# hkapp/cniic

Measured on AMD Instinct MI355X. Metric: Mpixels/sec encode (cluster-colors K=256), higher is better.
Workload: dtype u8/u64; 1 GPU; configs[1]: cluster-colors(256) encode of one 4096x4096 photo-like synthetic RGB image per GPU (seed 0x636E696963+2+rank), to convergence; image and stream HBM-resident; pixels_per_gpu=16777216, parallelism=1 GPU

## Files before the change

cniic_amd/csrc/codec.cpp:

```cpp
#include "codec.hpp"

#include <algorithm>
#include <cctype>
#include <cstring>
#include <memory>

#include "huff_host.hpp"

namespace cniic {

HostTrace &host_trace() { static thread_local HostTrace t; return t; }

static bool match_fun_u32(const std::string &s, const char *const *names, uint32_t *arg) {
    for (size_t p = 0; p < s.size(); p++)
        for (int i = 0; names[i]; i++) {
            const size_t l = strlen(names[i]);
            if (s.compare(p, l, names[i]) != 0 || p + l >= s.size() || s[p + l] != '(') continue;
            size_t q = p + l + 1;
            if (q >= s.size() || !isdigit((unsigned char)s[q])) continue;
            unsigned long long v = 0;
            bool ok = true;
            while (q < s.size() && isdigit((unsigned char)s[q])) {
                v = v * 10 + (unsigned)(s[q] - '0');
                if (v > 0xffffffffull) { ok = false; break; }
// ... 421 lines not shown
    put_u32(header, w);
    put_u32(header, h);
    huff_serialize_tree(tree, CNIIC_SYM_RGB, skeys.data(), header);
    *nbits = 0;
    for (size_t i = 0; i < scounts.size(); i++) *nbits += scounts[i] * slen[i];
    for (uint32_t k = 0; k < K; k++) {
        const size_t si = std::lower_bound(skeys.begin(), skeys.end(), colour(k)) - skeys.begin();
        clen[k] = pixels[k] ? slen[si] : 0;
        ccode[k] = pixels[k] ? scode[si] : 0;
    }
    return true;
}

int cc_finish(CcSession *s, const uint8_t *rgb_d, uint32_t w, uint32_t h, const uint32_t *local_counts_d, uint8_t *out,
              uint64_t cap, uint64_t *len, cniic_kmeans_stats *stats) {
    Ctx *c = s->c;
    const uint32_t K = s->K;
    const uint64_t U = s->U, n = (uint64_t)w * h;
    KmRgbwState *km = s->km;
    std::vector<uint8_t> cent(3 * (size_t)K);
    std::vector<uint64_t> members(K), wsum(K);
    cniic_kmeans_stats st{};
    const bool wide = km_rgbw_is_wide(km);
    DevBuf lab_d, key2label, pixlab;
    CNIIC_HIP_TRY(c, pixlab.alloc(n * (wide ? 2 : 1) + 16));
    DevBuf lw;
    bool lw_early = false;
    for (int attempt = 0;; attempt++) {
    CNIIC_TRY(km_rgbw_result_begin(km));
    if (s->sp_mode) {
        uint32_t *cell_start, *ckeys, *cweight;
        km_rgbw_cell_arrays(km, &cell_start, &ckeys, &cweight);
        if (s->local_points && K <= kPuPaletteWeights.words) {
            CNIIC_HIP_TRY(c, ctx_pinned_u(c));
            CNIIC_HIP_TRY(c, lw.alloc((uint64_t)K * 8));
            CNIIC_HIP_TRY(c, hipMemsetAsync(lw.p, 0, (uint64_t)K * 8, c->stream));
            CNIIC_TRY(local_cluster_weights(c, ckeys, km_rgbw_labels_internal(km, nullptr), wide, U, nullptr, K, lw.as<uint64_t>(), cweight));
            CNIIC_HIP_TRY(c, hipMemcpyAsync(c->pinned_u + kPuPaletteWeights.at, lw.p, (size_t)K * 8, hipMemcpyDeviceToHost, c->stream));
            if (!c->u_ev) CNIIC_HIP_TRY(c, hipEventCreateWithFlags(&c->u_ev, hipEventDisableTiming));
            CNIIC_HIP_TRY(c, hipEventRecord(c->u_ev, c->stream));
            lw_early = true;
        }
        CNIIC_TRY(sp_pixel_labels(c, &s->sp, rgb_d, cell_start, ckeys, km_rgbw_labels_internal(km, nullptr), wide, pixlab.p));
    } else {
        CNIIC_HIP_TRY(c, lab_d.alloc(U * (wide ? 2 : 1)));
        CNIIC_TRY(km_rgbw_labels_canonical(km, lab_d.p));
        CNIIC_HIP_TRY(c, key2label.alloc((1ull << 24) * (wide ? 2 : 1)));
        CNIIC_TRY(scatter_labels_by_key(c, s->keys_d.as<uint32_t>(), lab_d.p, wide, U, key2label.p));
        CNIIC_TRY(pixel_labels(c, rgb_d, n, key2label.p, wide, pixlab.p));
    }
    host_trace().mark("labels + pixel labels enq");
    const int rc_res = km_rgbw_result_end(km, cent.data(), members.data(), wsum.data(), &st);
    if (rc_res == kKmRetry && attempt == 0) continue;
    CNIIC_TRY(rc_res);
    break;
    }
    host_trace().mark("km_result");
    if (stats) *stats = st;
    CNIIC_TRY(check_enough_active(c, K, U, st.active));
    if (lw_early) {
        CNIIC_HIP_TRY(c, hipEventSynchronize(c->u_ev));
        for (uint32_t k = 0; k < K; k++) wsum[k] = c->pinned_u[kPuPaletteWeights.at + k];
    } else if (local_counts_d || s->local_points) {
        CNIIC_HIP_TRY(c, lw.alloc((uint64_t)K * 8));
        CNIIC_HIP_TRY(c, hipMemsetAsync(lw.p, 0, (uint64_t)K * 8, c->stream));
        if (s->sp_mode) {
            uint32_t *cell_start, *ckeys, *cweight;
            km_rgbw_cell_arrays(km, &cell_start, &ckeys, &cweight);
            CNIIC_TRY(local_cluster_weights(c, ckeys, km_rgbw_labels_internal(km, nullptr), wide, U, nullptr, K, lw.as<uint64_t>(), cweight));
        } else {
            CNIIC_TRY(local_cluster_weights(c, s->keys_d.as<uint32_t>(), lab_d.p, wide, U, local_counts_d, K, lw.as<uint64_t>(),
                                            s->weight_d.as<uint32_t>()));
        }
        CNIIC_HIP_TRY(c, hipMemcpyAsync(wsum.data(), lw.p, (size_t)K * 8, hipMemcpyDeviceToHost, c->stream));
        CNIIC_HIP_TRY(c, hipStreamSynchronize(c->stream));
    }
    std::vector<uint8_t> header, clen(K);
    std::vector<uint64_t> ccode(K);
    uint64_t nbits = 0;
    if (!palette_code(cent.data(), wsum.data(), K, w, h, header, clen.data(), ccode.data(), &nbits))
        return c->fail(CNIIC_ERR_BAD_ARG, "huffman: cannot build code");
    host_trace().mark("tree+codes (host)");
    StreamOut so(c, out, cap, len);
    CNIIC_TRY(so.begin(header, (nbits + 7) / 8));
    host_trace().mark("so.begin");
    DevBuf clen_d, ccode_d;
    CNIIC_HIP_TRY(c, clen_d.alloc(K));
    CNIIC_HIP_TRY(c, ccode_d.alloc((uint64_t)K * 8));
    CNIIC_HIP_TRY(c, hipMemcpyAsync(clen_d.p, clen.data(), K, hipMemcpyHostToDevice, c->stream));
    CNIIC_HIP_TRY(c, hipMemcpyAsync(ccode_d.p, ccode.data(), (size_t)K * 8, hipMemcpyHostToDevice, c->stream));
    uint64_t packed_bits = 0;
    {
        ScopedKernelTimer t(c, "huff_pack");
        CNIIC_TRY(huff_pack_labels(c, pixlab.p, n, wide, K, clen_d.as<uint8_t>(), ccode_d.as<uint64_t>(), so.dev,
                                   (uint64_t)header.size() * 8, &packed_bits));
        t.stop(1);
    }
    host_trace().mark("pack (+sync)");
    if (packed_bits != nbits)
        return c->fail(CNIIC_ERR_HIP, "cluster-colors: packed %llu bits, histogram predicts %llu",
                       (unsigned long long)packed_bits, (unsigned long long)nbits);
    const int rc_fin = so.finish();
    host_trace().mark("so.finish");
    return rc_fin;
}

int cc_finish_frames(CcSession *s, const uint8_t *rgb_d, uint32_t w, uint32_t h, uint32_t F, uint8_t *out, uint64_t stride, uint64_t *lens,
                     cniic_kmeans_stats *stats) {
    Ctx *c = s->c;
    const uint32_t K = s->K;
    const uint64_t U = s->U, npf = (uint64_t)w * h, n = npf * F;
    KmRgbwState *km = s->km;
    host_trace().mark("frames: enter");
    if (!F || !npf) return c->fail(CNIIC_ERR_BAD_ARG, "cc_finish_frames: empty batch");
    if (stride & 3) return c->fail(CNIIC_ERR_BAD_ARG, "cc_finish_frames: the stride between streams must be a multiple of 4");
    if (s->sp_mode && s->sp.npx != n) return c->fail(CNIIC_ERR_BAD_ARG, "cc_finish_frames: the session was opened on %llu pixels, the batch has %llu",
                                                     (unsigned long long)s->sp.npx, (unsigned long long)n);
    std::vector<uint8_t> cent(3 * (size_t)K);
    std::vector<uint64_t> members(K), wsum(K);
    cniic_kmeans_stats st{};
    CNIIC_TRY(km_rgbw_result_begin(km));
    const bool wide = km_rgbw_is_wide(km);
    const uint64_t lb = wide ? 2 : 1;
    DevBuf lab_d, key2label, pixlab, pixlab_al, cnt_d;
    host_trace().mark("frames: result_begin");
    CNIIC_HIP_TRY(c, pixlab.alloc(n * lb + 16));
    host_trace().mark("frames: alloc pixel labels");
    if (s->sp_mode) {
        uint32_t *cell_start, *ckeys, *cweight;
        km_rgbw_cell_arrays(km, &cell_start, &ckeys, &cweight);
        CNIIC_TRY(sp_pixel_labels(c, &s->sp, rgb_d, cell_start, ckeys, km_rgbw_labels_internal(km, nullptr), wide, pixlab.p));
        host_trace().mark("frames: pixel labels enqueued");
    } else {
        CNIIC_HIP_TRY(c, lab_d.alloc(U * lb));
        CNIIC_TRY(km_rgbw_labels_canonical(km, lab_d.p));
        CNIIC_HIP_TRY(c, key2label.alloc((1ull << 24) * lb));
        CNIIC_TRY(scatter_labels_by_key(c, s->keys_d.as<uint32_t>(), lab_d.p, wide, U, key2label.p));
        CNIIC_TRY(pixel_labels(c, rgb_d, n, key2label.p, wide, pixlab.p));
    }
    const void *labs = pixlab.p;
    uint64_t lab_stride = npf;
    if ((npf * lb) & 15) {
        lab_stride = (npf + 15) & ~15ull;
        CNIIC_HIP_TRY(c, pixlab_al.alloc(lab_stride * lb * F + 16));
        CNIIC_HIP_TRY(c, hipMemcpy2DAsync(pixlab_al.p, lab_stride * lb, pixlab.p, npf * lb, npf * lb, F, hipMemcpyDeviceToDevice, c->stream));
        labs = pixlab_al.p;
    }
    CNIIC_HIP_TRY(c, cnt_d.alloc((uint64_t)F * K * 4));
    CNIIC_TRY(frame_label_hist(c, labs, npf, lab_stride, F, wide, K, cnt_d.as<uint32_t>()));
    const bool gpu_trees = !wide && K <= 256 && c->opt(CNIIC_OPT_FRAME_TREES_HOST, "CNIIC_FRAME_TREES_HOST", 0) == 0;
    std::vector<uint32_t> cnt(gpu_trees ? 0 : (size_t)F * K);
    if (!gpu_trees) CNIIC_HIP_TRY(c, hipMemcpyAsync(cnt.data(), cnt_d.p, cnt.size() * 4, hipMemcpyDeviceToHost, c->stream));
    host_trace().mark("frames: hist enqueued");
    CNIIC_TRY(km_rgbw_result_end(km, cent.data(), members.data(), wsum.data(), &st));
    if (stats) *stats = st;
    CNIIC_TRY(check_enough_active(c, K, U, st.active));
    host_trace().mark("frames: result_end (sync)");
    CNIIC_HIP_TRY(c, hipStreamSynchronize(c->stream));
    host_trace().mark("frames: wait for the histograms");
    FramesOut fo(c, out, stride, F);
    DevBuf clen_d, ccode_d;
    CNIIC_HIP_TRY(c, clen_d.alloc((size_t)F * K));
    CNIIC_HIP_TRY(c, ccode_d.alloc((size_t)F * K * 8));
    std::vector<uint64_t> totals(F, 0);
    if (gpu_trees) {
        CNIIC_TRY(fo.begin());
        DevBuf meta_d;
        CNIIC_HIP_TRY(c, meta_d.alloc((size_t)F * 24 + 8));
        uint64_t *bb_d = meta_d.as<uint64_t>(), *nb_d = bb_d + F, *ln_d = nb_d + F;
        uint32_t *err_d = reinterpret_cast<uint32_t *>(ln_d + F);
        CNIIC_HIP_TRY(c, hipMemsetAsync(err_d, 0, 8, c->stream));
        CNIIC_TRY(frame_trees(c, cnt_d.as<uint32_t>(), km_rgbw_centroids_dev(km), F, K, w, h, fo.dev, stride, clen_d.as<uint8_t>(), ccode_d.as<uint64_t>(), bb_d, nb_d, ln_d, err_d));
        std::vector<uint64_t> meta((size_t)F * 3 + 1);
        CNIIC_HIP_TRY(c, hipMemcpyAsync(meta.data(), meta_d.p, (size_t)F * 24 + 8, hipMemcpyDeviceToHost, c->stream));
        CNIIC_HIP_TRY(c, hipStreamSynchronize(c->stream));
        host_trace().mark("frames: trees, codes, headers (GPU) + lengths back");
        const uint32_t err = (uint32_t)meta[(size_t)F * 3];
        if (err & 3u) return c->fail(CNIIC_ERR_BAD_ARG, "huffman: cannot build code");
// ... 589 lines not shown
```

cniic_amd/csrc/common.hpp:

```cpp
#pragma once
#include <hip/hip_runtime.h>

#include <algorithm>
#include <cstdarg>
#include <cstdint>
#include <cstdio>
#include <cstring>
#include <atomic>
#include <chrono>
#include <map>
#include <memory>
#include <mutex>
#include <string>
#include <thread>
#include <vector>

#include "../../include/cniic_hip.h"

namespace cniic {

constexpr uint64_t kDefaultSeed = 0x636E696963ULL;

struct KernelTime {
    double   ms = 0.0;
// ... 90 lines not shown
    bool        own_stream = false;
    std::mutex  mu;
    std::string err;
    std::map<std::string, KernelTime> ktimes;
    hipEvent_t  ev0 = nullptr, ev1 = nullptr;
    bool    timers = getenv("CNIIC_KERNEL_TIMERS") != nullptr;
    uint64_t opt_val[CNIIC_OPT_COUNT] = {};
    uint32_t opt_set = 0;
    uint64_t opt(int id, const char *env, uint64_t dflt) const {
        if (id > 0 && id < CNIIC_OPT_COUNT && ((opt_set >> id) & 1u)) return opt_val[id];
        const char *e = env ? getenv(env) : nullptr;
        return e ? strtoull(e, nullptr, 10) : dflt;
    }
    DevPool pool;
    DevBuf dense;
    DevBuf dense27, dense27_pages;
    bool   dense27_clean = false;
    DevBuf hilbert_lut;
    void  *pinned = nullptr;
    void  *pinned_ps = nullptr;
    uint32_t ps_div = 1;
    uint32_t ps_backoff = 0, ps_backoff_left = 0;
    hipEvent_t poll_ev[2] = {nullptr, nullptr};
    void  *pinned_res = nullptr;
    uint64_t pinned_res_bytes = 0;
    hipEvent_t res_ev = nullptr;
    uint64_t *pinned_u = nullptr;
    hipEvent_t u_ev = nullptr;
    std::shared_ptr<void> trie_scratch;
    std::shared_ptr<void> huf_scratch;
    void  *pinned_huf = nullptr;
    uint64_t pinned_huf_bytes = 0;
    hipEvent_t huf_ev = nullptr;
    std::shared_ptr<void> scan_leaves;
    DevBuf scan_xy;
    uint32_t scan_w = 0, scan_h = 0;
    std::vector<void *> batch_workers;
    DevBuf batch_stage;
    const void *poll_owner = nullptr;

    int fail(int code, const char *fmt, ...) {
        char buf[512];
        va_list ap;
        va_start(ap, fmt);
        vsnprintf(buf, sizeof buf, fmt, ap);
        va_end(ap);
        err = buf;
        return code;
    }
};

#define CNIIC_HIP_TRY(ctx, expr)                                                          \
    do {                                                                                  \
        hipError_t _e = (expr);                                                           \
        if (_e != hipSuccess)                                                             \
            return (ctx)->fail(CNIIC_ERR_HIP, "%s:%d %s -> %s", __FILE__, __LINE__, #expr, \
                               hipGetErrorString(_e));                                    \
    } while (0)

inline hipError_t ctx_spin_sync(Ctx *c) {
    hipError_t e;
    while ((e = hipStreamQuery(c->stream)) == hipErrorNotReady) {}
    return e;
}

inline hipError_t ctx_pinned_huf(Ctx *c, uint64_t bytes) {
    if (c->pinned_huf_bytes >= bytes) return hipSuccess;
    if (c->pinned_huf) (void)hipHostFree(c->pinned_huf);
    c->pinned_huf = nullptr; c->pinned_huf_bytes = 0;
    const uint64_t want = bytes + bytes / 4 + 65536;
    const hipError_t e = hipHostMalloc(&c->pinned_huf, want, hipHostMallocDefault);
    if (e == hipSuccess) c->pinned_huf_bytes = want;
    return e;
}

struct PuSlot { uint32_t at, words; };
constexpr uint32_t kPinnedUWords = 64 * 1024 / 8;
constexpr PuSlot kPuSpCount{0, 1};
constexpr PuSlot kPuPointCount{1, 1};
constexpr PuSlot kPuImageCount{2, 1};
constexpr PuSlot kPuHufTotals{3, 2};
constexpr PuSlot kPuDeltaOverflow{5, 1};
constexpr PuSlot kPuDeltaPacked{6, 1};
constexpr PuSlot kPuPaletteWeights{8, 4096};
constexpr PuSlot kPuHdecode{4104, 3};
constexpr PuSlot kPuTrieTotals{4108, 6};
constexpr PuSlot kPuLeafRuns{4114, 3};
constexpr PuSlot kPuSlots[] = {kPuSpCount, kPuPointCount, kPuImageCount, kPuHufTotals, kPuDeltaOverflow, kPuDeltaPacked,
                               kPuPaletteWeights, kPuHdecode, kPuTrieTotals, kPuLeafRuns};
constexpr bool pu_slots_disjoint() {
    uint32_t end = 0;
    for (const PuSlot &s : kPuSlots) {
        if (s.at < end || s.words == 0) return false;
        end = s.at + s.words;
    }
    return end <= kPinnedUWords;
}
static_assert(pu_slots_disjoint(), "Ctx::pinned_u: two slots overlap, or the last one ends behind the 64 KiB block");
static_assert(kPuPaletteWeights.words >= 4096, "Ctx::pinned_u: the shared-palette weights need room for K = 4096");

inline hipError_t ctx_pinned_u(Ctx *c) {
    if (c->pinned_u) return hipSuccess;
    return hipHostMalloc(reinterpret_cast<void **>(&c->pinned_u), kPinnedUWords * 8, hipHostMallocDefault);
}

#define CNIIC_TRY(expr)              \
    do {                             \
        int _rc = (expr);            \
        if (_rc != CNIIC_OK) return _rc; \
    } while (0)

inline bool is_device_ptr(const void *p) {
    if (!p) return false;
    hipPointerAttribute_t a;
    hipError_t e = hipPointerGetAttributes(&a, p);
    if (e != hipSuccess) { (void)hipGetLastError(); return false; }
    return a.type == hipMemoryTypeDevice || a.type == hipMemoryTypeManaged;
}

template <class T> struct In {
    const T *d = nullptr;
    DevBuf   own;
    int bind(Ctx *c, const T *p, uint64_t n) {
        if (n == 0 || !p) { d = nullptr; return CNIIC_OK; }
        if (is_device_ptr(p)) { d = p; return CNIIC_OK; }
        CNIIC_HIP_TRY(c, own.alloc(n * sizeof(T)));
        CNIIC_HIP_TRY(c, hipMemcpyAsync(own.p, p, n * sizeof(T), hipMemcpyHostToDevice, c->stream));
        d = own.as<T>();
        return CNIIC_OK;
    }
};

template <class T> struct Out {
    T       *d = nullptr;
    T       *host = nullptr;
    uint64_t n = 0;
    DevBuf   own;
    int bind(Ctx *c, T *p, uint64_t count) {
        n = count;
        if (!p || count == 0) { d = nullptr; host = nullptr; return CNIIC_OK; }
        if (is_device_ptr(p)) { d = p; host = nullptr; return CNIIC_OK; }
        CNIIC_HIP_TRY(c, own.alloc(count * sizeof(T)));
        d = own.as<T>();
        host = p;
        return CNIIC_OK;
    }
    int finish(Ctx *c, uint64_t count) {
        if (host && count) CNIIC_HIP_TRY(c, hipMemcpyAsync(host, d, count * sizeof(T), hipMemcpyDeviceToHost, c->stream));
        return CNIIC_OK;
    }
    int finish(Ctx *c) { return finish(c, n); }
};

inline uint64_t ceil_div(uint64_t a, uint64_t b) { return (a + b - 1) / b; }

inline int check_enough_active(Ctx *c, uint32_t K, uint64_t npoints, uint64_t active) {
    const uint64_t min_cc = std::min<uint64_t>((uint64_t)(0.99 * (double)K), npoints);
    if (active < min_cc)
        return c->fail(CNIIC_ERR_FEW_ACTIVE, "Not enough active clusters: requested %u, got %llu (min allowed: %llu)", K,
                       (unsigned long long)active, (unsigned long long)min_cc);
    return CNIIC_OK;
}

template <class Body> void parallel_for(uint32_t count, uint32_t threads, Body body) {
    std::atomic<uint32_t> next{0};
    auto work = [&](uint32_t t) { for (uint32_t i; (i = next.fetch_add(1)) < count;) body(i, t); };
    std::vector<std::thread> pool;
    for (uint32_t t = 1; t < threads; t++) pool.emplace_back(work, t);
    work(0);
    for (auto &th : pool) th.join();
}

// ... 82 lines not shown
                                       (unsigned long long)limit_ms);
                    std::this_thread::sleep_for(std::chrono::microseconds(20));
                }
            }
            CNIIC_HIP_TRY(c, hipEventSynchronize(c->poll_ev[slot ^ 1]));
            if (ring) {
                const volatile PollRec *r = reinterpret_cast<const volatile PollRec *>(static_cast<uint8_t *>(c->pinned) + ring_offset()) + last_prev % kPollRing;
                if (r->seq != last_prev) return c->fail(CNIIC_ERR_HIP, "kmeans: launch %u left no state record (found %u)", last_prev, r->seq);
                KmDevState t{};
                t.done = r->done; t.iter = r->iter; t.moved_last = r->moved_last; t.reseeds = r->reseeds; t.active = r->active; t.pair_evals = r->pair_evals;
                *h = t;
            } else if (mapped) {
                volatile KmDevState *m = &slots[2];
                KmDevState t{};
                t.done = m->done;
                std::atomic_thread_fence(std::memory_order_acquire);
                t.iter = m->iter; t.moved_last = m->moved_last; t.reseeds = m->reseeds; t.active = m->active; t.pair_evals = m->pair_evals;
                *h = t;
            } else {
                *h = slots[slot ^ 1];
            }
        }
        slot ^= 1;
        pending = 1;
        last_prev = last_launch;
        return CNIIC_OK;
    }
    int drain(KmDevState *h) {
        KmDevState *slots = static_cast<KmDevState *>(c->pinned);
        CNIIC_HIP_TRY(c, hipEventSynchronize(c->poll_ev[slot ^ 1]));
        *h = slots[slot ^ 1];
        return CNIIC_OK;
    }
};

struct HostTrace {
    bool on;
    std::vector<std::pair<const char *, double>> marks;
    HostTrace() : on(test_env("CNIIC_TRACE_HOST") != nullptr) {}
    static double now() { return std::chrono::duration<double, std::micro>(std::chrono::steady_clock::now().time_since_epoch()).count(); }
    void mark(const char *what) { if (on) marks.emplace_back(what, now()); }
    void dump() {
        if (!on || marks.empty()) return;
        for (size_t i = 1; i < marks.size(); i++) fprintf(stderr, "[host] %-28s %8.1f us\n", marks[i].first, marks[i].second - marks[i - 1].second);
        fprintf(stderr, "[host] %-28s %8.1f us\n", "total", marks.back().second - marks.front().second);
        marks.clear();
    }
};
HostTrace &host_trace();

struct ScopedKernelTimer {
    Ctx        *c;
    const char *name;
    bool        on;
    ScopedKernelTimer(Ctx *ctx, const char *nm) : ScopedKernelTimer(ctx, nm, ctx->timers) {}
    ScopedKernelTimer(Ctx *ctx, const char *nm, bool enable) : c(ctx), name(nm), on(enable) {
        if (on) (void)hipEventRecord(c->ev0, c->stream);
    }
    void stop(uint64_t launches = 1) {
        if (!on) return;
        (void)hipEventRecord(c->ev1, c->stream);
        (void)hipEventSynchronize(c->ev1);
        float ms = 0.f;
        (void)hipEventElapsedTime(&ms, c->ev0, c->ev1);
        KernelTime &kt = c->ktimes[name];
        kt.ms += ms;
        kt.launches += launches;
        on = false;
    }
};


int hist_rgb_dense(Ctx *c, const uint8_t *rgb_d, uint64_t npx, uint32_t *table_d);
int hist_syms_dense(Ctx *c, const uint32_t *syms_d, uint64_t n, uint32_t *table_d, uint32_t bits);
struct CompactPlan {
    DevBuf   blockoff, blockmax;
    uint64_t n_unique = 0;
    uint64_t max_count = 0;
    uint32_t bits = 0;
    const uint8_t *pages = nullptr;
};
int occupancy_pack(Ctx *c, const uint32_t *table_d, uint32_t *occ_d);
int gidx_build(Ctx *c, const uint32_t *occ_d, DevBuf &bits, DevBuf &wprefix, uint64_t *U_h, DevBuf *total_keep = nullptr);
int gidx_finish(Ctx *c, uint32_t *wprefix_d, const uint32_t *blocktot_d, uint64_t *total_d);

struct SpPlan {
    uint64_t npx = 0, U = 0;
    uint32_t nchunks = 0;
    DevBuf cnt, pre, bstart;
    DevBuf part, prank;
    DevBuf cell_count;
    DevBuf sstart, sbin, scnt;
    DevBuf bits, wprefix;
    DevBuf total;
};
int sp_build(Ctx *c, const uint8_t *rgb_d, uint64_t npx, SpPlan *plan);
int sp_wait_count(Ctx *c, SpPlan *plan);
int sp_emit(Ctx *c, const SpPlan *plan, const uint32_t *cell_start_d, uint32_t *ckeys_d, uint32_t *cweight_d, void *labels_d, bool wide,
            uint32_t K, const void *gbits_d, const uint32_t *gprefix_d, uint64_t Ug, const uint64_t *Ug_dev );
int sp_occupancy(Ctx *c, const SpPlan *plan, uint32_t *occ_d);
int sp_pixel_labels(Ctx *c, const SpPlan *plan, const uint8_t *rgb_d, const uint32_t *cell_start_d, const uint32_t *ckeys_d,
                    const void *labels_d, bool wide, void *pixlab_d);
int hist_compact_count(Ctx *c, const uint32_t *table_d, uint32_t bits, CompactPlan *plan, uint32_t *cell_count_d = nullptr,
                       const uint8_t *pages_d = nullptr);
int hist_compact_write(Ctx *c, uint32_t *table_d, const CompactPlan *plan, uint32_t *keys_d, uint64_t *counts_d,
                       uint32_t *weights_d);
int dense_table(Ctx *c, uint32_t bits, uint32_t **table_d);

struct KmRgbwState;
int km_rgbw_create(Ctx *c, const uint32_t *keys_d, const uint32_t *weight_d, uint64_t U, uint32_t shard,
                   uint32_t nshards, uint32_t K, const cniic_kmeans_opts *opts, void *partials_dev,
                   const uint32_t *rank_table_d , KmRgbwState **out,
                   const uint32_t *cell_count_d = nullptr ,
                   const void *gbits_d = nullptr, const uint32_t *gprefix_d = nullptr, uint64_t Ug = 0
                   ,
                   bool points_follow = false ,
                   const uint64_t *points_dev = nullptr );
int km_rgbw_set_points(KmRgbwState *s, uint64_t U, uint64_t Ulist = 0 );
void km_rgbw_cell_arrays(KmRgbwState *s, uint32_t **cell_start_d, uint32_t **ckeys_d, uint32_t **cweight_d);
void km_rgbw_destroy(KmRgbwState *s);
int km_rgbw_set_state(KmRgbwState *s, const uint8_t *centroids_h, const uint32_t *labels_d_u32);
int km_rgbw_assign(KmRgbwState *s);
int km_rgbw_update(KmRgbwState *s);
struct Comm;
int comm_unique_id(uint8_t *id128);
int comm_create(Ctx *c, const uint8_t *id128, uint32_t rank, uint32_t nranks, Comm **out);
int comm_create_host(Ctx *c, uint32_t rank, uint32_t nranks, int32_t (*fn)(void *, void *, uint64_t, int32_t), void *user, Comm **out);
void comm_destroy(Comm *cm);
Ctx *comm_ctx(Comm *cm);
uint32_t comm_size(const Comm *cm);
int comm_all_reduce(Comm *cm, void *buf_d, uint64_t count, int kind);
void comm_abort(Comm *cm);
int comm_async_error(Comm *cm);
uint64_t comm_timeout_ms(const Comm *cm);
void comm_set_timeout_ms(Comm *cm, uint64_t ms);
int comm_create_mailbox(Ctx *c, uint32_t rank, uint32_t nranks, uint64_t max_bytes, uint8_t *handle64, Comm **out);
int comm_connect_mailbox(Comm *cm, const uint8_t *handles);

struct Mailbox;
int mailbox_create(Ctx *c, uint32_t rank, uint32_t nranks, uint64_t cap_bytes, uint8_t *handle64, Mailbox **out);
int mailbox_connect(Mailbox *m, const uint8_t *handles);
int mailbox_all_reduce(Mailbox *m, void *buf_d, uint64_t count, int kind, uint64_t timeout_ms);
int mailbox_status(const Mailbox *m);
void mailbox_abort(Mailbox *m);
void mailbox_destroy(Mailbox *m);

constexpr int kKmRetry = 1000;
int km_rgbw_run(KmRgbwState *s, Comm *cm = nullptr, bool may_defer = false);
int km_rgbw_poll_changed(KmRgbwState *s, uint64_t *changed);
int km_rgbw_poll(KmRgbwState *s, cniic_kmeans_stats *st, uint32_t *done);
bool km_rgbw_run_stats(KmRgbwState *s, cniic_kmeans_stats *st);
int km_rgbw_poll_lagged(KmRgbwState *s, cniic_kmeans_stats *st, uint32_t *done, uint32_t *have);
int km_rgbw_result(KmRgbwState *s, uint8_t *centroids_h, uint32_t *labels_d_u32, uint64_t *members_h,
                   uint64_t *wsum_h, cniic_kmeans_stats *stats);
int km_rgbw_result_begin(KmRgbwState *s);
int km_rgbw_result_end(KmRgbwState *s, uint8_t *centroids_h, uint64_t *members_h, uint64_t *wsum_h, cniic_kmeans_stats *stats);
int km_rgbw_time_assign(KmRgbwState *s, int reps, double *ms_per_launch);
int km_rgbw_partials(KmRgbwState *s, uint64_t *sums_h, uint64_t *wsum_h, uint64_t *members_h, uint64_t *changed_h);
void *km_rgbw_partials_dev(KmRgbwState *s);
const uint32_t *km_rgbw_centroids_dev(KmRgbwState *s);
bool km_rgbw_is_wide(KmRgbwState *s);
int km_rgbw_labels_canonical(KmRgbwState *s, void *dst_d);
void *km_rgbw_labels_internal(KmRgbwState *s, uint64_t *elem_bytes);
int km_rgbw_fold_initial(KmRgbwState *s);
int km_rgbw_export_labels(KmRgbwState *s, void *dst_d);
int km_rgbw_import_labels(KmRgbwState *s, const void *src_d);
uint64_t km_rgbw_points(KmRgbwState *s);
// ... 2 lines not shown
                 const cniic_kmeans_opts *opts, cniic_colorpos *centroids_h, uint32_t *labels_d_u32,
                 uint64_t *members_h, cniic_kmeans_stats *stats);
int km_xyrgb_run_wide(Ctx *c, const uint8_t *rgb_d, uint32_t w, uint32_t h, uint32_t K, const cniic_kmeans_opts *opts, cniic_colorpos *centroids_h,
                      uint32_t *labels_d_u32, uint64_t *members_h, cniic_kmeans_stats *stats);
int km_xyrgb_step(Ctx *c, const uint8_t *rgb_d, uint32_t w, uint32_t h, uint32_t K,
                  const cniic_colorpos *centroids_h, uint32_t *labels_d_u32, uint64_t *sums_h,
                  uint64_t *wsum_h, uint64_t *members_h, uint64_t *changed_h, const cniic_kmeans_opts *opts);

int remap_rgb(Ctx *c, const uint8_t *rgb_d, uint64_t npx, const uint32_t *rank_table_d,
              const uint32_t *lut_rgb_d , uint8_t *out_d);
int expand_codes_by_label(Ctx *c, const uint8_t *labels8_d, const uint16_t *labels16_d, uint64_t U, const uint8_t *clen_d,
                          const uint64_t *ccode_d, uint8_t *len_d, uint64_t *code_d);
int local_cluster_weights(Ctx *c, const uint32_t *keys_d, const void *labels_d, bool wide, uint64_t U,
                          const uint32_t *local_counts_d, uint32_t K, uint64_t *out_d, const uint32_t *weights_d = nullptr);
int label_lut(Ctx *c, const uint32_t *labels_d, uint64_t U, const uint32_t *cent_d, uint32_t *lut_d);
int rank_from_keys(Ctx *c, const uint32_t *keys_d, uint64_t U, uint32_t *table_d);
int voronoi_paint(Ctx *c, const cniic_colorpos *cent_d, uint32_t K, uint32_t w, uint32_t h, uint8_t *out_d, bool small_coords = false);
int mse_rgb(Ctx *c, const uint8_t *a_d, const uint8_t *b_d, uint64_t npx, double *mse_h);
int mse_rgb_batch(Ctx *c, const uint8_t *a_d, const uint8_t *b_d, uint64_t npx, uint32_t frames, double *mse_h);
int mse_rgb_batch_var(Ctx *c, const uint8_t *a_d, const uint8_t *b_d, const uint64_t *a_off, const uint64_t *b_off, const uint64_t *npx,
                      uint32_t frames, double *mse_h);
int synth_image(Ctx *c, int kind, uint64_t seed, uint32_t w, uint32_t h, uint8_t *out_d);
int rgb_to_keys(Ctx *c, const uint8_t *rgb_d, uint64_t npx, uint32_t *keys_d);

constexpr int kCellShift = 3;
constexpr uint32_t kCellsPerDim = 256 >> kCellShift;
constexpr uint32_t kNumCells = kCellsPerDim * kCellsPerDim * kCellsPerDim;

struct LeafTable;
struct UdSums { DevBuf buf; bool filled = false; };
int huff_decode_dev(Ctx *c, const LeafTable &lt, const uint8_t *payload, bool payload_dev, uint64_t payload_bytes, uint64_t nsyms,
                    int mode, void *out_d, int *status, UdSums *sums = nullptr);
struct HdBatchFrame {
    const LeafTable *lt = nullptr;
    const uint8_t *payload = nullptr;
    uint64_t payload_bytes = 0, nsyms = 0;
    uint8_t *out_d = nullptr;
    int status = 0;
};
int huff_decode_batch_dev(Ctx *c, std::vector<HdBatchFrame> &frames);
int huff_decode_tables_dev(Ctx *c, const uint8_t *tab_d, uint64_t n, uint64_t off_key, uint64_t off_len, uint32_t max_len, uint32_t first_key,
                           const uint8_t *payload, bool payload_dev, uint64_t payload_bytes, uint64_t nsyms, int mode, void *out_d, int *status, UdSums *sums = nullptr);
int huff_parse_leaves_dev(Ctx *c, int sym_kind, const uint8_t *stream_d, uint64_t nbytes, uint64_t pos0, DevBuf *tab, uint64_t *n_leaves,
                          uint64_t *off_key, uint64_t *off_len, uint32_t *max_len, uint64_t *payload_pos, int *status);
int keys_to_rgb(Ctx *c, const uint32_t *keys_d, uint64_t n, uint8_t *rgb_d);
int delta_undiff_dev(Ctx *c, const uint32_t *keys_d, uint64_t n, uint8_t *lin_d, uint32_t *bad_h);
int delta_undiff_scatter_dev(Ctx *c, const uint32_t *keys_d, uint32_t w, uint32_t h, uint8_t *rgb_out_d, uint32_t *bad_h, UdSums *sums = nullptr);

struct RlePlan { uint64_t n = 0, nruns = 0; uint32_t nchunks = 0; DevBuf flags, run_off; };
int rle_plan(Ctx *c, const uint8_t *lin_d, uint64_t n, RlePlan *plan);
int rle_emit(Ctx *c, const uint8_t *lin_d, const RlePlan *plan, uint32_t *out_words_d);
int rle_expand_dev(Ctx *c, const uint8_t *rec_d, uint64_t R, uint64_t tail_bytes, uint64_t n, uint8_t *lin_d, int *status);
int rle_offsets(Ctx *c, const uint32_t *chunk_runs_d, uint32_t nchunks, uint64_t *run_off_d, uint64_t *total_d);
double rla_threshold(double d);
int rle_approx_plan(Ctx *c, const uint8_t *lin_d, uint64_t n, double d, RlePlan *plan);
int rle_approx_emit(Ctx *c, const uint8_t *lin_d, const RlePlan *plan, uint32_t *out_words_d);

int hilbert_xy(Ctx *c, uint32_t w, uint32_t h, uint32_t *xy_d);
int hilbert_linearize(Ctx *c, const uint8_t *rgb_d, uint32_t w, uint32_t h, uint8_t *out_d);
int hilbert_delta(Ctx *c, const uint8_t *rgb_d, uint32_t w, uint32_t h, uint32_t *syms_d, uint32_t *table_d);
int hilbert_scatter(Ctx *c, const uint8_t *lin_d, uint32_t w, uint32_t h, uint8_t *rgb_out_d);
int scan_inject(Ctx *c, uint32_t w, uint32_t h, const uint32_t *xy, bool xy_dev);
int hilbert_undiff_scatter(Ctx *c, const uint32_t *keys_d, const int32_t *chunk_off_d, uint32_t w, uint32_t h, uint8_t *rgb_out_d, uint32_t *bad_d, bool *fused);

constexpr uint32_t kPageShift = 12;
int delta_table(Ctx *c, uint32_t **table_d, uint8_t **pages_d);
int delta_table_clean(Ctx *c);
uint64_t delta_stream_len(uint64_t n);
int delta_gather_hist(Ctx *c, const uint8_t *rgb_d, uint32_t w, uint32_t h, uint16_t *hot16_d, uint32_t *table_d, uint8_t *pages_d,
                      uint32_t *coldkeys_d, uint8_t *chunk_cold_d, uint32_t *overflow_d);
struct DeltaPackScratch { DevBuf cb, co, edge, hot, hotlen; };
int delta_pack16_count(Ctx *c, const uint16_t *hot16_d, uint64_t n, uint32_t *coldkeys_d, const uint8_t *chunk_cold_d, uint32_t *dense_d,
                       const uint32_t *keys_d, const uint8_t *len_d, const uint64_t *code_d, uint64_t U, uint64_t *total_d, DeltaPackScratch *keep);
int delta_pack16_write(Ctx *c, const uint16_t *hot16_d, uint64_t n, const uint32_t *coldkeys_d, const uint8_t *len_d, const uint64_t *code_d, uint8_t *out_d,
                       uint64_t bit_base, DeltaPackScratch *keep);

int huff_sort_leaves_dev(Ctx *c, const uint64_t *counts_d, uint32_t n, uint64_t max_count, uint64_t *buf_a, uint64_t *buf_b, uint64_t **out_d);
int huff_sort_u64(Ctx *c, uint64_t *buf_a, uint64_t *buf_b, uint32_t n, uint32_t lo_bit, uint64_t **out_d);
int huff_tree_from_runs(Ctx *c, const uint64_t *sorted_d, const uint64_t *counts_d, uint32_t n, int sym_kind, uint8_t *len_d, uint64_t *code_d,
                        uint64_t *off_d, uint64_t *nbits_h, bool *built);
int huff_tree_codes(Ctx *c, const uint32_t *left_d, const uint32_t *right_d, const uint32_t *nleaves_d, const uint64_t *counts_d, uint32_t n,
                    uint32_t root, int sym_kind, uint8_t *len_d, uint64_t *code_d, uint64_t *off_d, uint64_t *totals_d);
int huff_tree_serialize_dev(Ctx *c, const uint32_t *keys_d, const uint64_t *off_d, uint32_t n, int sym_kind, uint8_t *trie_d, uint64_t trie_bytes);
int pack_scan(Ctx *c, const uint32_t *chunk_bits_d, uint32_t nchunks, uint64_t *chunk_off_d, uint64_t *total_d);
uint32_t pack_img_cap();
int huff_pack_keys(Ctx *c, const uint32_t *keys_or_null_d, const uint8_t *rgb_or_null_d, uint64_t n,
                   const uint32_t *rank_table_d, const uint8_t *len_d, const uint64_t *code_d,
                   uint8_t *out_d, uint64_t bit_base, uint64_t *nbits_h);
int huff_rank_stream(Ctx *c, const uint32_t *keys_or_null_d, const uint8_t *rgb_or_null_d, uint64_t n, const uint32_t *rank_table_d,
                     uint32_t *ranks_d, bool one_based);
int huff_pack_ranks(Ctx *c, const uint32_t *ranks_d, uint64_t n, const uint8_t *len_d, const uint64_t *code_d, uint8_t *out_d,
                    uint64_t bit_base, uint64_t *nbits_h);
int huff_pack_code32(Ctx *c, const uint32_t *syms_or_null_d, const uint8_t *rgb_or_null_d, uint64_t n, uint32_t *table_d,
                     const uint32_t *keys_d, const uint8_t *len_d, const uint64_t *code_d, uint64_t U, uint32_t *packed_d,
                     uint8_t *out_d, uint64_t bit_base, uint64_t *nbits_h);
int huff_pack_code32_hot(Ctx *c, const uint32_t *syms_d, uint64_t n, uint32_t *dense_d, const uint32_t *keys_d, const uint8_t *len_d,
                         const uint64_t *code_d, uint64_t U, uint32_t *packed_d, uint8_t *out_d, uint64_t bit_base, uint64_t *nbits_h);
int pixel_labels(Ctx *c, const uint8_t *rgb_d, uint64_t n, const void *key2label_d, bool wide, void *pixlab_d);
int huff_pack_labels(Ctx *c, const void *pixlab_d, uint64_t n, bool wide, uint32_t K, const uint8_t *clen_d,
                     const uint64_t *ccode_d, uint8_t *out_d, uint64_t bit_base, uint64_t *nbits_h);
int scatter_labels_by_key(Ctx *c, const uint32_t *keys_d, const void *labels_d, bool wide, uint64_t U, void *key2label_d);
int frame_label_hist(Ctx *c, const void *pixlab_d, uint64_t npf, uint64_t lab_stride, uint32_t frames, bool wide, uint32_t K, uint32_t *out_d );
int huff_pack_labels_frames(Ctx *c, const void *pixlab_d, uint64_t npf, uint64_t lab_stride, uint32_t frames, bool wide, uint32_t K, const uint8_t *clen_d,
                            const uint64_t *ccode_d, uint8_t *out_d, uint64_t stride, const uint64_t *bit_base_h, uint64_t *totals_h, const uint64_t *bit_base_d = nullptr);
int frame_trees(Ctx *c, const uint32_t *cnt_d, const uint32_t *cent_d, uint32_t frames, uint32_t K, uint32_t w, uint32_t h, uint8_t *out_d, uint64_t stride,
                uint8_t *clen_d, uint64_t *ccode_d, uint64_t *bit_base_d, uint64_t *nbits_d, uint64_t *lens_d, uint32_t *err_d);

}
```

cniic_amd/csrc/k_hist.hip:

```cpp
#include <cstdlib>

#include "common.hpp"
#include "device_utils.hpp"

namespace cniic {

__global__ __launch_bounds__(256) void k_hist_rgb(const uint8_t *__restrict__ rgb, uint64_t npx,
                                                  uint32_t *__restrict__ table) {
    const uint64_t ngroups = npx / 16;
    const uint64_t stride = (uint64_t)gridDim.x * blockDim.x;
    const uint4 *v = reinterpret_cast<const uint4 *>(rgb);
    for (uint64_t g = (uint64_t)blockIdx.x * blockDim.x + threadIdx.x; g < ngroups; g += stride) {
        uint32_t key[16];
        load16px_keys(v + 3 * g, key);
#pragma unroll
        for (int i = 0; i < 16; i++) atomic_count(table, key[i]);
    }
    if (blockIdx.x == 0) {
        uint64_t i = ngroups * 16 + threadIdx.x;
        if (i < npx) atomic_count(table, rgb_key(rgb + 3 * i));
    }
}

constexpr int kPartBits = 12;
// ... 256 lines not shown
            val[i] = rank + 1;
            rank++;
            dirty = true;
        }
    }
    if (dirty) {
#pragma unroll
        for (int j = 0; j < kScanPerThread / 4; j++)
            v[j] = make_uint4(val[4 * j], val[4 * j + 1], val[4 * j + 2], val[4 * j + 3]);
    }
}

int hist_compact_count(Ctx *c, const uint32_t *table_d, uint32_t bits, CompactPlan *plan, uint32_t *cell_count_d, const uint8_t *pages_d) {
    static_assert(kScanChunk == (1 << kPageShift), "a page flag per block of the compaction");
    plan->pages = pages_d;
    const uint64_t entries = 1ull << bits;
    const uint32_t nblocks = (uint32_t)(entries / kScanChunk);
    DevBuf tot;
    CNIIC_HIP_TRY(c, plan->blockoff.alloc((uint64_t)nblocks * 4));
    CNIIC_HIP_TRY(c, plan->blockmax.alloc((uint64_t)nblocks * 4));
    CNIIC_HIP_TRY(c, tot.alloc(16));
    hipLaunchKernelGGL(k_compact_count, dim3(nblocks), dim3(kScanThreads), 0, c->stream, table_d, plan->blockoff.as<uint32_t>(), plan->blockmax.as<uint32_t>(),
                       bits == 24 ? cell_count_d : nullptr, pages_d, tot.as<uint64_t>());
    {
        const uint32_t nparts = (nblocks + 1023) / 1024;
        DevBuf parttot;
        CNIIC_HIP_TRY(c, parttot.alloc((uint64_t)nparts * 4));
        hipLaunchKernelGGL(k_compact_scan_local, dim3(nparts), dim3(1024), 0, c->stream, plan->blockoff.as<uint32_t>(), (const uint32_t *)plan->blockmax.as<uint32_t>(), nblocks,
                           parttot.as<uint32_t>(), tot.as<uint64_t>());
        if (nparts > 1)
            hipLaunchKernelGGL(k_compact_scan_add, dim3(nparts), dim3(1024), 0, c->stream, plan->blockoff.as<uint32_t>(), nblocks,
                               (const uint32_t *)parttot.as<uint32_t>(), tot.as<uint64_t>());
    }
    CNIIC_HIP_TRY(c, hipGetLastError());
    uint64_t total[2] = {0, 0};
    CNIIC_HIP_TRY(c, hipMemcpyAsync(total, tot.p, 16, hipMemcpyDeviceToHost, c->stream));
    CNIIC_HIP_TRY(c, pages_d ? ctx_spin_sync(c) : hipStreamSynchronize(c->stream));
    plan->n_unique = total[0];
    plan->max_count = total[1];
    plan->bits = bits;
    return CNIIC_OK;
}

int hist_compact_write(Ctx *c, uint32_t *table_d, const CompactPlan *plan, uint32_t *keys_d, uint64_t *counts_d,
                       uint32_t *weights_d) {
    const uint32_t nblocks = (uint32_t)((1ull << plan->bits) / kScanChunk);
    hipLaunchKernelGGL(k_compact_write, dim3(nblocks), dim3(kScanThreads), 0, c->stream, table_d,
                       plan->blockoff.as<uint32_t>(), keys_d, counts_d, weights_d, plan->pages);
    CNIIC_HIP_TRY(c, hipGetLastError());
    return CNIIC_OK;
}

__global__ __launch_bounds__(256) void k_occ_pack(const uint32_t *__restrict__ table, uint32_t *__restrict__ occ) {
    const uint32_t wd = blockIdx.x * 256 + threadIdx.x;
    const uint4 a = reinterpret_cast<const uint4 *>(table)[2 * (size_t)wd], b = reinterpret_cast<const uint4 *>(table)[2 * (size_t)wd + 1];
    occ[wd] = (a.x != 0) | ((a.y != 0) << 4) | ((a.z != 0) << 8) | ((a.w != 0) << 12) | ((b.x != 0) << 16) | ((b.y != 0) << 20) |
              ((b.z != 0) << 24) | ((uint32_t)(b.w != 0) << 28);
}
__global__ __launch_bounds__(256) void k_gidx_words(const uint32_t *__restrict__ occ, unsigned long long *__restrict__ bits,
                                                    uint32_t *__restrict__ wprefix, uint32_t *__restrict__ blocktot) {
    __shared__ uint32_t wsum[256 / 64];
    const uint32_t w0 = (blockIdx.x * 256 + threadIdx.x) * 4;
    uint32_t cnt[4], mine = 0;
#pragma unroll
    for (int q = 0; q < 4; q++) {
        unsigned long long m = 0;
#pragma unroll
        for (int j = 0; j < 8; j++) {
            const uint32_t v = occ[8 * (size_t)(w0 + q) + j];
#pragma unroll
            for (int i = 0; i < 8; i++)
                if ((v >> (4 * i)) & 15u) m |= 1ull << (8 * j + i);
        }
        bits[w0 + q] = m;
        cnt[q] = (uint32_t)__popcll(m);
        mine += cnt[q];
    }
    uint32_t run = block_exclusive_scan<256>(mine, wsum);
#pragma unroll
    for (int q = 0; q < 4; q++) { wprefix[w0 + q] = run; run += cnt[q]; }
    if (threadIdx.x == 255) blocktot[blockIdx.x] = run;
}
__global__ __launch_bounds__(256) void k_gidx_finish(uint32_t *__restrict__ wprefix, const uint32_t *__restrict__ blocktot,
                                                     uint64_t *__restrict__ total) {
    __shared__ uint32_t wsum[256 / 64];
    __shared__ uint32_t boff[256];
    const uint32_t t = blocktot[threadIdx.x];
    const uint32_t ex = block_exclusive_scan<256>(t, wsum);
    boff[threadIdx.x] = ex;
    if (blockIdx.x == 0 && threadIdx.x == 255) *total = (uint64_t)ex + t;
    __syncthreads();
    const uint32_t add = boff[blockIdx.x];
    for (uint32_t i = threadIdx.x; i < 1024; i += 256) wprefix[blockIdx.x * 1024 + i] += add;
}

int gidx_finish(Ctx *c, uint32_t *wprefix_d, const uint32_t *blocktot_d, uint64_t *total_d) {
    hipLaunchKernelGGL(k_gidx_finish, dim3(256), dim3(256), 0, c->stream, wprefix_d, blocktot_d, total_d);
    CNIIC_HIP_TRY(c, hipGetLastError());
    return CNIIC_OK;
}

int occupancy_pack(Ctx *c, const uint32_t *table_d, uint32_t *occ_d) {
    hipLaunchKernelGGL(k_occ_pack, dim3((1u << 21) / 256), dim3(256), 0, c->stream, table_d, occ_d);
    CNIIC_HIP_TRY(c, hipGetLastError());
    return CNIIC_OK;
}

int gidx_build(Ctx *c, const uint32_t *occ_d, DevBuf &bits, DevBuf &wprefix, uint64_t *U_h, DevBuf *total_keep) {
    DevBuf tot_own;
    DevBuf &tot = total_keep ? *total_keep : tot_own;
    CNIIC_HIP_TRY(c, bits.alloc((1ull << 18) * 8));
    CNIIC_HIP_TRY(c, wprefix.alloc((1ull << 18) * 4));
    CNIIC_HIP_TRY(c, tot.alloc(8));
    DevBuf blocktot;
    CNIIC_HIP_TRY(c, blocktot.alloc(256 * 4));
    hipLaunchKernelGGL(k_gidx_words, dim3(256), dim3(256), 0, c->stream, occ_d, bits.as<unsigned long long>(), wprefix.as<uint32_t>(),
                       blocktot.as<uint32_t>());
    hipLaunchKernelGGL(k_gidx_finish, dim3(256), dim3(256), 0, c->stream, wprefix.as<uint32_t>(), (const uint32_t *)blocktot.as<uint32_t>(),
                       tot.as<uint64_t>());
    CNIIC_HIP_TRY(c, hipGetLastError());
    CNIIC_HIP_TRY(c, hipMemcpyAsync(U_h, tot.p, 8, hipMemcpyDeviceToHost, c->stream));
    if (!total_keep) CNIIC_HIP_TRY(c, hipStreamSynchronize(c->stream));
    return CNIIC_OK;
}

int dense_table(Ctx *c, uint32_t bits, uint32_t **table_d) {
    const uint64_t bytes = (1ull << bits) * 4;
    if (c->dense.bytes < bytes) CNIIC_HIP_TRY(c, c->dense.alloc(bytes));
    CNIIC_HIP_TRY(c, hipMemsetAsync(c->dense.p, 0, bytes, c->stream));
    *table_d = c->dense.as<uint32_t>();
    return CNIIC_OK;
}

}
```

cniic_amd/csrc/k_huff.hip:

```cpp
#include <mutex>

#include <algorithm>
#include <vector>

#include "common.hpp"
#include "device_utils.hpp"

namespace cniic {

constexpr int kPackThreads = 256;
constexpr int kPackPer = 16;
constexpr int kPackChunk = kPackThreads * kPackPer;

enum { SRC_RGB = 0, SRC_KEYS = 1, SRC_SYM16 = 2, SRC_RANKS = 3 };

template <int SRC>
__device__ __forceinline__ void fetch_ranks(const void *__restrict__ src, uint64_t n, uint64_t first,
                                            const uint32_t *__restrict__ rank_table, uint32_t rank[kPackPer]) {
    if (SRC == SRC_RGB) {
        const uint8_t *rgb = reinterpret_cast<const uint8_t *>(src);
        if (first + kPackPer <= n && ((reinterpret_cast<uintptr_t>(rgb) & 15) == 0)) {
            uint32_t key[16];
            load16px_keys(reinterpret_cast<const uint4 *>(rgb + 3 * first), key);
#pragma unroll
            for (int i = 0; i < kPackPer; i++) rank[i] = rank_table[key[i]] - 1;
        } else {
#pragma unroll
            for (int i = 0; i < kPackPer; i++)
                rank[i] = (first + i < n) ? rank_table[rgb_key(rgb + 3 * (first + i))] - 1 : 0xffffffffu;
        }
    } else if (SRC == SRC_KEYS) {
        const uint32_t *keys = reinterpret_cast<const uint32_t *>(src);
#pragma unroll
        for (int i = 0; i < kPackPer; i++) rank[i] = (first + i < n) ? rank_table[keys[first + i]] - 1 : 0xffffffffu;
    } else if (SRC == SRC_RANKS) {
        const uint32_t *rk = reinterpret_cast<const uint32_t *>(src);
        if (first + kPackPer <= n && ((reinterpret_cast<uintptr_t>(rk) & 15) == 0)) {
            const uint4 *v = reinterpret_cast<const uint4 *>(rk + first);
#pragma unroll
            for (int j = 0; j < 4; j++) { const uint4 q = v[j]; rank[4 * j] = q.x - 1; rank[4 * j + 1] = q.y - 1; rank[4 * j + 2] = q.z - 1; rank[4 * j + 3] = q.w - 1; }
        } else {
#pragma unroll
            for (int i = 0; i < kPackPer; i++) rank[i] = (first + i < n) ? rk[first + i] - 1 : 0xffffffffu;
        }
    } else {
        const uint16_t *sym = reinterpret_cast<const uint16_t *>(src);
#pragma unroll
        for (int i = 0; i < kPackPer; i++) rank[i] = (first + i < n) ? (uint32_t)sym[first + i] : 0xffffffffu;
    }
}

template <int SRC>
__global__ __launch_bounds__(kPackThreads) void k_rank_stream(const void *__restrict__ src, uint64_t n,
                                                              const uint32_t *__restrict__ rank_table, uint32_t *__restrict__ out,
                                                              uint32_t plus) {
    const uint64_t first = (uint64_t)blockIdx.x * kPackChunk + (uint64_t)threadIdx.x * kPackPer;
    uint32_t rank[kPackPer];
    fetch_ranks<SRC>(src, n, first, rank_table, rank);
    if (first + kPackPer <= n && ((reinterpret_cast<uintptr_t>(out) & 15) == 0)) {
        uint4 *o = reinterpret_cast<uint4 *>(out + first);
#pragma unroll
        for (int j = 0; j < 4; j++) o[j] = make_uint4(rank[4 * j] + plus, rank[4 * j + 1] + plus, rank[4 * j + 2] + plus, rank[4 * j + 3] + plus);
    } else {
        for (int i = 0; i < kPackPer; i++)
            if (first + i < n) out[first + i] = rank[i] + plus;
    }
}

template <int SRC>
__global__ __launch_bounds__(kPackThreads) void k_pack_count(const void *__restrict__ src, uint64_t n,
                                                             const uint32_t *__restrict__ rank_table,
                                                             const uint8_t *__restrict__ len,
                                                             uint32_t *__restrict__ chunk_bits) {
    const uint64_t first = (uint64_t)blockIdx.x * kPackChunk + (uint64_t)threadIdx.x * kPackPer;
    uint32_t rank[kPackPer];
    fetch_ranks<SRC>(src, n, first, rank_table, rank);
    uint32_t bits = 0;
#pragma unroll
    for (int i = 0; i < kPackPer; i++)
        if (rank[i] != 0xffffffffu) bits += len[rank[i]];
    bits = block_reduce_sum<kPackThreads>(bits);
    if (threadIdx.x == 0) chunk_bits[blockIdx.x] = bits;
}

__global__ __launch_bounds__(1024) void k_pack_scan_local(const uint32_t *__restrict__ chunk_bits, uint32_t nchunks,
                                                          uint64_t *__restrict__ chunk_off, uint64_t *__restrict__ blocktot,
                                                          uint64_t *__restrict__ total_bits) {
    __shared__ uint32_t wsum[1024 / 64];
    const uint32_t i = blockIdx.x * 1024 + threadIdx.x;
    const uint32_t v = i < nchunks ? chunk_bits[i] : 0u;
    const uint32_t ex = block_exclusive_scan<1024>(v, wsum);
    if (i < nchunks) chunk_off[i] = ex;
    if (threadIdx.x == 1023) {
        blocktot[blockIdx.x] = (uint64_t)ex + v;
        if (gridDim.x == 1) *total_bits = (uint64_t)ex + v;
    }
}
__global__ __launch_bounds__(1024) void k_pack_scan_add(uint32_t nchunks, uint64_t *__restrict__ chunk_off,
                                                        const uint64_t *__restrict__ blocktot, uint64_t *__restrict__ total_bits) {
    __shared__ unsigned long long s_before;
    unsigned long long mine = 0;
    for (uint32_t b = threadIdx.x; b < blockIdx.x; b += 1024) mine += blocktot[b];
    if (threadIdx.x == 0) s_before = 0;
    __syncthreads();
    mine = wave_reduce_sum64(mine);
    if ((threadIdx.x & 63) == 0 && mine) atomicAdd(&s_before, mine);
    __syncthreads();
    const unsigned long long before = s_before;
    const uint32_t i = blockIdx.x * 1024 + threadIdx.x;
    if (i < nchunks) chunk_off[i] += before;
    if (blockIdx.x == gridDim.x - 1 && threadIdx.x == 0) *total_bits = before + blocktot[blockIdx.x];
}
__global__ __launch_bounds__(1024) void k_pack_scan_small(const uint32_t *__restrict__ chunk_bits, uint32_t nchunks,
                                                          uint64_t *__restrict__ chunk_off, uint64_t *__restrict__ total_bits) {
    __shared__ uint32_t wsum[1024 / 64];
    const uint32_t i0 = threadIdx.x * 8;
    uint32_t v[8], sum = 0;
#pragma unroll
    for (int j = 0; j < 8; j++) { v[j] = i0 + j < nchunks ? chunk_bits[i0 + j] : 0u; sum += v[j]; }
    uint32_t run = block_exclusive_scan<1024>(sum, wsum);
#pragma unroll
    for (int j = 0; j < 8; j++) {
        if (i0 + j < nchunks) chunk_off[i0 + j] = run;
        run += v[j];
    }
    if (threadIdx.x == 1023) *total_bits = run;
}
static int pack_scan_counts(Ctx *c, const uint32_t *counts_d, uint32_t n, uint64_t *off_d, uint64_t *total_d) {
    if (n > 1024 && n <= 8192) {
        hipLaunchKernelGGL(k_pack_scan_small, dim3(1), dim3(1024), 0, c->stream, counts_d, n, off_d, total_d);
        CNIIC_HIP_TRY(c, hipGetLastError());
        return CNIIC_OK;
    }
    return pack_scan(c, counts_d, n, off_d, total_d);
}
int pack_scan(Ctx *c, const uint32_t *chunk_bits_d, uint32_t nchunks, uint64_t *chunk_off_d, uint64_t *total_d) {
    const uint32_t nb = (nchunks + 1023) / 1024;
    DevBuf blocktot;
    CNIIC_HIP_TRY(c, blocktot.alloc((uint64_t)nb * 8));
    hipLaunchKernelGGL(k_pack_scan_local, dim3(nb), dim3(1024), 0, c->stream, chunk_bits_d, nchunks, chunk_off_d, blocktot.as<uint64_t>(), total_d);
    if (nb > 1)
        hipLaunchKernelGGL(k_pack_scan_add, dim3(nb), dim3(1024), 0, c->stream, nchunks, chunk_off_d, (const uint64_t *)blocktot.as<uint64_t>(), total_d);
    CNIIC_HIP_TRY(c, hipGetLastError());
    return CNIIC_OK;
}

uint32_t pack_img_cap() {
    const char *e = test_env("CNIIC_TEST_PACK_IMG_WORDS");
    return e ? (uint32_t)atoi(e) : 0xffffffffu;
}

template <int SRC>
__global__ __launch_bounds__(kPackThreads) void k_pack_write(const void *__restrict__ src, uint64_t n,
                                                             const uint32_t *__restrict__ rank_table,
                                                             const uint8_t *__restrict__ len,
                                                             const uint64_t *__restrict__ code,
                                                             const uint64_t *__restrict__ chunk_off,
                                                             uint32_t *__restrict__ out_words, uint64_t bit_base, uint32_t img_cap) {
    constexpr uint32_t kImgWords = kPackChunk + 2;
    __shared__ uint32_t img[kImgWords];
    __shared__ uint32_t wsum[kPackThreads / 64];
    __shared__ uint32_t s_total;
    const uint64_t first = (uint64_t)blockIdx.x * kPackChunk + (uint64_t)threadIdx.x * kPackPer;
    uint32_t rank[kPackPer];
    fetch_ranks<SRC>(src, n, first, rank_table, rank);
    uint32_t l[kPackPer];
    uint32_t bits = 0;
#pragma unroll
    for (int i = 0; i < kPackPer; i++) {
        l[i] = rank[i] != 0xffffffffu ? len[rank[i]] : 0;
        bits += l[i];
    }
    uint32_t excl = block_exclusive_scan<kPackThreads>(bits, wsum);
    const uint64_t g0 = bit_base + chunk_off[blockIdx.x];
    const uint32_t skew = (uint32_t)(g0 & 31);
    uint32_t pos = skew + excl;
    if (threadIdx.x == kPackThreads - 1) s_total = excl + bits;
    __syncthreads();
    const uint32_t total = s_total;
    if (total == 0) return;
    const uint32_t nwords = (skew + total + 31) >> 5;
    const uint64_t w0 = g0 >> 5;
    if (nwords + 2 > min(kImgWords, img_cap)) {
#pragma unroll 1
        for (int i = 0; i < kPackPer; i++) {
            if (l[i]) pack_put<true>(out_words + w0, pos, l[i], code[rank[i]]);
            pos += l[i];
        }
        return;
    }
    for (uint32_t i = threadIdx.x; i < nwords + 2; i += kPackThreads) img[i] = 0;
    __syncthreads();
#pragma unroll
    for (int i = 0; i < kPackPer; i++) {
        if (l[i]) pack_put<false>(img, pos, l[i], code[rank[i]]);
        pos += l[i];
    }
    __syncthreads();
    for (uint32_t i = threadIdx.x; i < nwords; i += kPackThreads) {
        uint32_t v = __builtin_bswap32(img[i]);
        if (v == 0) continue;
        if (i == 0 || i == nwords - 1) atomicOr(&out_words[w0 + i], v);
        else out_words[w0 + i] = v;
    }
}

template <typename LabelT>
__global__ __launch_bounds__(kPackThreads) void k_pixel_labels(const uint8_t *__restrict__ rgb, uint64_t n,
                                                               const LabelT *__restrict__ key2label, LabelT *__restrict__ pixlab) {
    const uint64_t first = (uint64_t)blockIdx.x * kPackChunk + (uint64_t)threadIdx.x * kPackPer;
    if (first + kPackPer <= n && ((reinterpret_cast<uintptr_t>(rgb) & 15) == 0)) {
        uint32_t key[16];
        load16px_keys(reinterpret_cast<const uint4 *>(rgb + 3 * first), key);
        LabelT lab[16];
#pragma unroll
        for (int i = 0; i < 16; i++) lab[i] = key2label[key[i]];
        if (sizeof(LabelT) == 1) {
            uint32_t w[4];
#pragma unroll
            for (int j = 0; j < 4; j++) w[j] = (uint32_t)lab[4 * j] | ((uint32_t)lab[4 * j + 1] << 8) | ((uint32_t)lab[4 * j + 2] << 16) | ((uint32_t)lab[4 * j + 3] << 24);
            *reinterpret_cast<uint4 *>(pixlab + first) = make_uint4(w[0], w[1], w[2], w[3]);
        } else {
#pragma unroll
            for (int i = 0; i < 16; i++) pixlab[first + i] = lab[i];
        }
    } else {
        for (int i = 0; i < kPackPer; i++)
            if (first + i < n) pixlab[first + i] = key2label[rgb_key(rgb + 3 * (first + i))];
    }
}

template <typename LabelT>
__global__ __launch_bounds__(kPackThreads) void k_pack_count_lab(const LabelT *__restrict__ pixlab, uint64_t n, uint32_t K,
                                                                 const uint8_t *__restrict__ clen,
                                                                 uint32_t *__restrict__ chunk_bits, uint64_t lab_stride = 0) {
    extern __shared__ uint8_t s_len[];
    pixlab += (size_t)blockIdx.y * lab_stride;
    clen += (size_t)blockIdx.y * K;
    chunk_bits += (size_t)blockIdx.y * gridDim.x;
    for (uint32_t i = threadIdx.x; i < K; i += kPackThreads) s_len[i] = clen[i];
    __syncthreads();
    const uint64_t first = (uint64_t)blockIdx.x * kPackChunk + (uint64_t)threadIdx.x * kPackPer;
    uint32_t bits = 0;
    if (sizeof(LabelT) == 1 && first + kPackPer <= n) {
        const uint4 v = *reinterpret_cast<const uint4 *>(pixlab + first);
        const uint32_t w[4] = {v.x, v.y, v.z, v.w};
#pragma unroll
        for (int i = 0; i < 16; i++) bits += s_len[(w[i >> 2] >> (8 * (i & 3))) & 255];
    } else {
        for (int i = 0; i < kPackPer; i++)
            if (first + i < n) bits += s_len[pixlab[first + i]];
    }
    bits = block_reduce_sum<kPackThreads>(bits);
    if (threadIdx.x == 0) chunk_bits[blockIdx.x] = bits;
}

template <typename LabelT>
__global__ __launch_bounds__(kPackThreads) void k_pack_write_lab(const LabelT *__restrict__ pixlab, uint64_t n, uint32_t K,
                                                                 const uint8_t *__restrict__ clen,
                                                                 const uint64_t *__restrict__ ccode,
                                                                 const uint64_t *__restrict__ chunk_off,
                                                                 uint32_t *__restrict__ out_words, uint64_t bit_base, uint64_t lab_stride = 0,
                                                                 uint64_t out_stride_words = 0, const uint64_t *__restrict__ bit_base_frames = nullptr,
                                                                 uint32_t img_cap = 0xffffffffu ) {
    extern __shared__ __align__(8) unsigned long long s_tab[];
    pixlab += (size_t)blockIdx.y * lab_stride;
    clen += (size_t)blockIdx.y * K;
    ccode += (size_t)blockIdx.y * K;
    chunk_off += (size_t)blockIdx.y * gridDim.x;
    out_words += (size_t)blockIdx.y * out_stride_words;
    if (bit_base_frames) bit_base = bit_base_frames[blockIdx.y];
    constexpr uint32_t kImgWords = kPackChunk / 2 + 2;
    __shared__ uint32_t img[kImgWords];
    __shared__ uint32_t wsum[kPackThreads / 64];
    __shared__ uint32_t s_total;
    uint8_t *s_len = reinterpret_cast<uint8_t *>(s_tab + K);
    for (uint32_t i = threadIdx.x; i < K; i += kPackThreads) { s_tab[i] = ccode[i]; s_len[i] = clen[i]; }
    __syncthreads();
    const uint64_t first = (uint64_t)blockIdx.x * kPackChunk + (uint64_t)threadIdx.x * kPackPer;
    uint32_t lab[kPackPer], l[kPackPer];
    uint32_t bits = 0;
    if (sizeof(LabelT) == 1 && first + kPackPer <= n) {
        const uint4 v = *reinterpret_cast<const uint4 *>(pixlab + first);
        const uint32_t w[4] = {v.x, v.y, v.z, v.w};
#pragma unroll
        for (int i = 0; i < 16; i++) lab[i] = (w[i >> 2] >> (8 * (i & 3))) & 255;
    } else {
#pragma unroll
        for (int i = 0; i < kPackPer; i++) lab[i] = first + i < n ? (uint32_t)pixlab[first + i] : 0xffffffffu;
    }
#pragma unroll
    for (int i = 0; i < kPackPer; i++) { l[i] = lab[i] != 0xffffffffu ? s_len[lab[i]] : 0; bits += l[i]; }
    uint32_t excl = block_exclusive_scan<kPackThreads>(bits, wsum);
    const uint64_t g0 = bit_base + chunk_off[blockIdx.x];
    const uint32_t skew = (uint32_t)(g0 & 31);
    uint32_t pos = skew + excl;
    if (threadIdx.x == kPackThreads - 1) s_total = excl + bits;
    __syncthreads();
    const uint32_t nw_all = (skew + s_total + 31) >> 5;
    if (nw_all + 2 > min(kImgWords, img_cap)) {
        const uint64_t w0 = g0 >> 5;
#pragma unroll 1
        for (int i = 0; i < kPackPer; i++) {
            const uint32_t L = l[i];
            if (L == 0) continue;
            const uint64_t cd = s_tab[lab[i]];
            const uint32_t w = pos >> 5, b = pos & 31, room = 32 - b;
            if (L <= room) {
                atomicOr(&out_words[w0 + w], __builtin_bswap32((uint32_t)(cd << (room - L))));
            } else {
                const uint32_t rem = L - room;
                atomicOr(&out_words[w0 + w], __builtin_bswap32((uint32_t)(cd >> rem)));
                if (rem <= 32) atomicOr(&out_words[w0 + w + 1], __builtin_bswap32((uint32_t)(cd << (32 - rem))));
                else { atomicOr(&out_words[w0 + w + 1], __builtin_bswap32((uint32_t)(cd >> (rem - 32)))); atomicOr(&out_words[w0 + w + 2], __builtin_bswap32((uint32_t)(cd << (64 - rem)))); }
            }
            pos += L;
        }
        return;
    }
    for (uint32_t i = threadIdx.x; i < nw_all + 2; i += kPackThreads) img[i] = 0;
    __syncthreads();
#pragma unroll
    for (int i = 0; i < kPackPer; i++) {
        const uint32_t L = l[i];
        if (L == 0) continue;
        const uint64_t cd = s_tab[lab[i]];
        const uint32_t w = pos >> 5, b = pos & 31, room = 32 - b;
        if (L <= room) {
            atomicOr(&img[w], (uint32_t)(cd << (room - L)));
        } else {
            const uint32_t rem = L - room;
            atomicOr(&img[w], (uint32_t)(cd >> rem));
            if (rem <= 32) atomicOr(&img[w + 1], (uint32_t)(cd << (32 - rem)));
            else { atomicOr(&img[w + 1], (uint32_t)(cd >> (rem - 32))); atomicOr(&img[w + 2], (uint32_t)(cd << (64 - rem))); }
        }
        pos += L;
    }
    __syncthreads();
    const uint32_t total = s_total;
    if (total == 0) return;
    const uint32_t nwords = (skew + total + 31) >> 5;
    const uint64_t w0 = g0 >> 5;
    for (uint32_t i = threadIdx.x; i < nwords; i += kPackThreads) {
        const uint32_t v = __builtin_bswap32(img[i]);
        if (v == 0) continue;
        if (i == 0 || i == nwords - 1) atomicOr(&out_words[w0 + i], v);
        else out_words[w0 + i] = v;
    }
}

int pixel_labels(Ctx *c, const uint8_t *rgb_d, uint64_t n, const void *key2label_d, bool wide, void *pixlab_d) {
    if (n == 0) return CNIIC_OK;
    const uint32_t nchunks = (uint32_t)ceil_div(n, kPackChunk);
    if (wide)
        hipLaunchKernelGGL(k_pixel_labels<uint16_t>, dim3(nchunks), dim3(kPackThreads), 0, c->stream, rgb_d, n,
                           reinterpret_cast<const uint16_t *>(key2label_d), reinterpret_cast<uint16_t *>(pixlab_d));
    else
        hipLaunchKernelGGL(k_pixel_labels<uint8_t>, dim3(nchunks), dim3(kPackThreads), 0, c->stream, rgb_d, n,
                           reinterpret_cast<const uint8_t *>(key2label_d), reinterpret_cast<uint8_t *>(pixlab_d));
    CNIIC_HIP_TRY(c, hipGetLastError());
    return CNIIC_OK;
}

int huff_pack_labels(Ctx *c, const void *pixlab_d, uint64_t n, bool wide, uint32_t K,
                     const uint8_t *clen_d, const uint64_t *ccode_d, uint8_t *out_d, uint64_t bit_base, uint64_t *nbits_h) {
    *nbits_h = 0;
    if (n == 0) return CNIIC_OK;
    if (reinterpret_cast<uintptr_t>(out_d) & 3) return c->fail(CNIIC_ERR_BAD_ARG, "huff_pack: output must be 4-byte aligned");
    const uint32_t nchunks = (uint32_t)ceil_div(n, kPackChunk);
    DevBuf cb, co, tot;
    CNIIC_HIP_TRY(c, cb.alloc((uint64_t)nchunks * 4));
    CNIIC_HIP_TRY(c, co.alloc((uint64_t)nchunks * 8));
    CNIIC_HIP_TRY(c, tot.alloc(8));
    if (wide)
        hipLaunchKernelGGL(k_pack_count_lab<uint16_t>, dim3(nchunks), dim3(kPackThreads), K, c->stream,
                           reinterpret_cast<const uint16_t *>(pixlab_d), n, K, clen_d, cb.as<uint32_t>());
    else
        hipLaunchKernelGGL(k_pack_count_lab<uint8_t>, dim3(nchunks), dim3(kPackThreads), K, c->stream,
                           reinterpret_cast<const uint8_t *>(pixlab_d), n, K, clen_d, cb.as<uint32_t>());
    CNIIC_TRY(pack_scan(c, cb.as<uint32_t>(), nchunks, co.as<uint64_t>(), tot.as<uint64_t>()));
    if (wide)
        hipLaunchKernelGGL(k_pack_write_lab<uint16_t>, dim3(nchunks), dim3(kPackThreads), (size_t)K * 9 + 8, c->stream,
                           reinterpret_cast<const uint16_t *>(pixlab_d), n, K, clen_d, ccode_d, co.as<uint64_t>(),
                           reinterpret_cast<uint32_t *>(out_d), bit_base, (uint64_t)0, (uint64_t)0, (const uint64_t *)nullptr, pack_img_cap());
    else
        hipLaunchKernelGGL(k_pack_write_lab<uint8_t>, dim3(nchunks), dim3(kPackThreads), (size_t)K * 9 + 8, c->stream,
                           reinterpret_cast<const uint8_t *>(pixlab_d), n, K, clen_d, ccode_d, co.as<uint64_t>(),
                           reinterpret_cast<uint32_t *>(out_d), bit_base, (uint64_t)0, (uint64_t)0, (const uint64_t *)nullptr, pack_img_cap());
    CNIIC_HIP_TRY(c, hipGetLastError());
    uint64_t total = 0;
    CNIIC_HIP_TRY(c, hipMemcpyAsync(&total, tot.p, 8, hipMemcpyDeviceToHost, c->stream));
    CNIIC_HIP_TRY(c, hipStreamSynchronize(c->stream));
    *nbits_h = total;
    return CNIIC_OK;
}

template <typename LabelT>
__global__ __launch_bounds__(256) void k_frame_label_hist(const LabelT *__restrict__ pixlab, uint64_t npf, uint64_t lab_stride, uint32_t K,
                                                          uint32_t *__restrict__ out ) {
    extern __shared__ uint32_t s_hist[];
    for (uint32_t i = threadIdx.x; i < 4 * K; i += 256) s_hist[i] = 0;
    __syncthreads();
    const LabelT *base = pixlab + (size_t)blockIdx.y * lab_stride;
    uint32_t *hw = s_hist + (threadIdx.x >> 6) * K;
    const uint64_t per = ((npf + gridDim.x - 1) / gridDim.x + 15) & ~15ull;
    const uint64_t lo = (uint64_t)blockIdx.x * per, hi = lo + per < npf ? lo + per : npf;
    if (sizeof(LabelT) == 1 && (reinterpret_cast<uintptr_t>(base) & 15) == 0) {
        for (uint64_t i = lo + (uint64_t)threadIdx.x * 16; i < hi; i += 256 * 16) {
            if (i + 16 <= hi) {
                const uint4 v = *reinterpret_cast<const uint4 *>(base + i);
                const uint32_t w[4] = {v.x, v.y, v.z, v.w};
#pragma unroll
                for (int j = 0; j < 16; j++) atomicAdd(&hw[(w[j >> 2] >> (8 * (j & 3))) & 255], 1u);
            } else {
                for (uint64_t q = i; q < hi; q++) atomicAdd(&hw[base[q]], 1u);
            }
        }
    } else {
        for (uint64_t i = lo + threadIdx.x; i < hi; i += 256) atomicAdd(&hw[base[i]], 1u);
    }
    __syncthreads();
    for (uint32_t i = threadIdx.x; i < K; i += 256) {
        const uint32_t v = s_hist[i] + s_hist[K + i] + s_hist[2 * K + i] + s_hist[3 * K + i];
        if (v) atomicAdd(&out[(size_t)blockIdx.y * K + i], v);
    }
}

int frame_label_hist(Ctx *c, const void *pixlab_d, uint64_t npf, uint64_t lab_stride, uint32_t frames, bool wide, uint32_t K, uint32_t *out_d) {
    if (!frames || !npf) return CNIIC_OK;
    CNIIC_HIP_TRY(c, hipMemsetAsync(out_d, 0, (uint64_t)frames * K * 4, c->stream));
    const uint32_t bx = (uint32_t)std::min<uint64_t>(std::max<uint64_t>(ceil_div(npf, 1u << 16), 1), 64);
    if (wide)
        hipLaunchKernelGGL(k_frame_label_hist<uint16_t>, dim3(bx, frames), dim3(256), (size_t)K * 16, c->stream,
                           reinterpret_cast<const uint16_t *>(pixlab_d), npf, lab_stride, K, out_d);
    else
        hipLaunchKernelGGL(k_frame_label_hist<uint8_t>, dim3(bx, frames), dim3(256), (size_t)K * 16, c->stream,
                           reinterpret_cast<const uint8_t *>(pixlab_d), npf, lab_stride, K, out_d);
    CNIIC_HIP_TRY(c, hipGetLastError());
    return CNIIC_OK;
}

__device__ __forceinline__ void bitonic_sort_256(unsigned long long *a, uint32_t tid) {
    for (uint32_t k = 2; k <= 256; k <<= 1)
        for (uint32_t j = k >> 1; j > 0; j >>= 1) {
            __syncthreads();
            const uint32_t x = tid ^ j;
            if (x > tid) {
                const unsigned long long u = a[tid], v = a[x];
                const bool up = (tid & k) == 0;
                if ((u > v) == up) { a[tid] = v; a[x] = u; }
            }
        }
    __syncthreads();
}

__global__ __launch_bounds__(256) void k_frame_trees(const uint32_t *__restrict__ cnt , const uint32_t *__restrict__ cent ,
                                                     uint32_t K, uint32_t w, uint32_t h, uint8_t *__restrict__ out, uint64_t stride,
                                                     uint8_t *__restrict__ clen , unsigned long long *__restrict__ ccode ,
                                                     unsigned long long *__restrict__ bit_base , unsigned long long *__restrict__ nbits ,
                                                     unsigned long long *__restrict__ lens , uint32_t *__restrict__ err) {
    __shared__ unsigned long long s_sort[256];
    __shared__ uint32_t s_key[256], s_cnt[256], s_bfreq[256];
    __shared__ unsigned short s_symk[256], s_left[256], s_right[256], s_parent[512], s_size[512];
    __shared__ unsigned char s_side[512], s_len[256];
    __shared__ unsigned long long s_code[256], s_bits;
    __shared__ uint32_t s_wsum[4], s_n;
    const uint32_t tid = threadIdx.x, f = blockIdx.x;
    const uint32_t *fc = cnt + (size_t)f * K;
    const uint32_t myc = tid < K ? fc[tid] : 0u;
    s_sort[tid] = myc ? (((unsigned long long)(cent[tid] & 0xffffffu) << 32) | tid) : ~0ull;
    s_cnt[tid] = 0;
    if (tid == 0) s_bits = 0;
    bitonic_sort_256(s_sort, tid);
    const unsigned long long me = s_sort[tid];
    const bool valid = me != ~0ull;
    const uint32_t key = (uint32_t)(me >> 32), k = (uint32_t)me & 0xffffu;
// ... 813 lines not shown
```

cniic_amd/csrc/k_kmeans_persist.hip:

```cpp
#include <atomic>

#include <hip/hip_ext.h>

#include "kmeans_rgbw.hpp"

namespace cniic {

constexpr int kPsThreads = 1024, kPsWaves = kPsThreads / 64;
constexpr uint32_t kPsAccWords = 5 * 256;
constexpr uint32_t kPsOffTab = kPsAccWords * 8, kPsOffS = kPsOffTab + 256 * 8;
static_assert(kPsOffCell == kPsOffS + kPsSlotsMax * kPsScap * 4, "ps_cell_bytes / kPsOffCell (kmeans_rgbw.hpp) describe this layout");

__device__ __forceinline__ uint32_t ps_xcc_id() {
    uint32_t v;
    asm volatile("s_getreg_b32 %0, hwreg(HW_REG_XCC_ID)" : "=s"(v));
    return v & 7u;
}
__device__ __forceinline__ unsigned long long ps_aread(unsigned long long *p) {
    return __hip_atomic_fetch_add(p, 0ull, __ATOMIC_RELAXED, __HIP_MEMORY_SCOPE_AGENT);
}
__device__ __forceinline__ uint32_t ps_ld(const uint32_t *p) { return __hip_atomic_load(p, __ATOMIC_RELAXED, __HIP_MEMORY_SCOPE_AGENT); }
__device__ __forceinline__ void ps_st(uint32_t *p, uint32_t v) { __hip_atomic_store(p, v, __ATOMIC_RELAXED, __HIP_MEMORY_SCOPE_AGENT); }

__device__ __forceinline__ bool ps_spin(uint32_t *word, uint32_t old, PsBar *b, unsigned long long ticks) {
// ... 809 lines not shown
                atomicOr(&s_mm[(k >> 6) & 3], 1ull << (k & 63));
            }
        } else if (tid == kPsThreads - 1) {
            s_changed = ps_aread(&Pcur[5 * (size_t)K]);
            s_pev = ps_aread(&Pcur[5 * (size_t)K + 1]);
        }
        __syncthreads();
        const unsigned long long changed = s_changed;
        nS = s_nmoved;
        reseeds_total += s_reseed;
        evals_total += s_pev;
        const bool fin = changed == 0 || (a.max_iters && j >= a.max_iters);
        if (blockIdx.x == 0 && tid == 0) {
            KmDevState *sw = a.st_rw;
            sw->changed_ring[(j - 1) % kHistRing] = changed;
            sw->nmoved_ring[(j - 1) % kHistRing] = nS;
            if (fin) {
                sw->moved_last = changed; sw->reseeds = reseeds_total; sw->active = s_active; sw->pair_evals = evals_total; sw->iter = j; sw->done = 1;
                PsExit *x = &a.cold->exit;
                x->iter = j; x->moved_last = changed; x->reseeds = reseeds_total; x->active = s_active; x->pair_evals = evals_total;
            }
        }
        if (fin) break;
    }
    if (blockIdx.x == 0 && tid < K) {
        const PsCold *cd = a.cold;
        const uint2 cc = tab[tid];
        cd->cent_g[tid] = cc.x;
        cd->cconst_g[tid] = cc;
        cd->members_out[tid] = run[4];
        cd->wsum_out[tid] = run[3];
    }
    for (uint32_t i = wid; i < C; i += kPsWaves) {
        const uint32_t s = cstart[i], n = cstart[i + 1] - s, gs = gstart[i];
        if (i < Cres) { for (uint32_t t = lane; t < n; t += 64) a.labels[gs + t] = (uint8_t)(255u - (pts[s + t] >> 24)); }
        else { for (uint32_t t = lane; t < n; t += 64) a.labels[gs + t] = (uint8_t)(255u - (a.pk[gs + t] >> 24)); }
    }
    if (blockIdx.x == 0) {
        __syncthreads();
        if (tid == 0) { __threadfence_system(); a.cold->exit.status = kPsStatusDone; __threadfence_system(); }
    }
}

static std::atomic<int> g_ps_cus_in_use[16];

static int ps_cu_count(int device) {
    static std::atomic<int> cached[16];
    const int d = device >= 0 && device < 16 ? device : 0;
    int n = cached[d].load();
    if (n) return n;
    hipDeviceProp_t prop;
    if (hipGetDeviceProperties(&prop, device) != hipSuccess) { (void)hipGetLastError(); return 0; }
    cached[d].store(prop.multiProcessorCount);
    return prop.multiProcessorCount;
}

uint32_t ps_grid_for(Ctx *c, uint64_t Umax) {
    uint32_t G = (uint32_t)ps_cu_count(c->device);
    if (!G) return 0;
    G = std::max(1u, G / std::max(1u, c->ps_div));
    if (const uint64_t mb = c->opt(CNIIC_OPT_KM_MAX_BLOCKS, "CNIIC_KM_MAX_BLOCKS", 0)) G = std::max<uint32_t>(1u, (uint32_t)((uint64_t)G * std::min<uint64_t>(mb, 768) / 768));
    if (const char *e = test_env("CNIIC_KM_PS_BLOCKS")) G = std::max(1, atoi(e));
    G = (uint32_t)std::min<uint64_t>(G, std::max<uint64_t>(1, ceil_div(Umax, 512)));
    return std::min<uint32_t>(G, 1024u);
}

static void ps_learn(Ctx *c, uint32_t status, bool injected) {
    if (status == kPsStatusDone) { c->ps_backoff = 0; c->ps_backoff_left = 0; return; }
    if (status != kPsStatusAborted || injected) return;
    c->ps_backoff = std::min<uint32_t>(256u, std::max<uint32_t>(4u, 2u * c->ps_backoff));
    c->ps_backoff_left = c->ps_backoff;
}

int ps_prepare(KmRgbwState *s) {
    Ctx *c = s->c;
    if (c->ps_backoff_left && !test_env("CNIIC_KM_PS_REQUIRE")) { c->ps_backoff_left--; return CNIIC_OK; }
    const uint32_t G = ps_grid_for(c, s->U);
    if (!G) return CNIIC_OK;
    static bool attr_set[16] = {};
    if (c->device >= 0 && c->device < 16 && !attr_set[c->device]) {
        CNIIC_HIP_TRY(c, hipFuncSetAttribute(reinterpret_cast<const void *>(k_rgbw_persist), hipFuncAttributeMaxDynamicSharedMemorySize, (int)kPsDynBytes));
        attr_set[c->device] = true;
    }
    const uint64_t o_bar = 0, o_part = (sizeof(PsBar) + 255) & ~255ull, o_fail = o_part + ((3 * (uint64_t)kPsPartWords * 8 + 255) & ~255ull);
    const uint64_t o_rng = o_fail + 256, total = o_rng + ((uint64_t)G * kPsChunks + 1) * 4;
    CNIIC_HIP_TRY(c, s->ps_arena.alloc(total));
    CNIIC_HIP_TRY(c, hipMemsetAsync(s->ps_arena.p, 0, o_rng, c->stream));
    CNIIC_HIP_TRY(c, s->ps_pk.alloc(std::max<uint64_t>(s->U, 1) * 4));
    s->ps_blocks = G;
    s->ps_o_part = o_part; s->ps_o_fail = o_fail; s->ps_o_rng = o_rng;
    (void)o_bar;
    uint8_t *a = s->ps_arena.as<uint8_t>();
    uint32_t budget = kPsDynBytes;
    if (const char *e = test_env("CNIIC_TEST_PS_LDS_BYTES")) budget = std::min<uint32_t>(kPsDynBytes, (uint32_t)atoi(e));
    s->ps_budget = budget;
    hipLaunchKernelGGL(k_ps_ranges, dim3(1), dim3(1024), 0, c->stream, (const uint32_t *)s->ne_cost.as<uint32_t>(), (const uint32_t *)s->ne_count.as<uint32_t>(), G, budget,
                       reinterpret_cast<uint32_t *>(a + o_rng), reinterpret_cast<uint32_t *>(a + o_fail));
    CNIIC_HIP_TRY(c, hipGetLastError());
    s->ps = true;
    return CNIIC_OK;
}

int km_rgbw_run_persistent(KmRgbwState *s, bool *ran, bool may_defer) {
    Ctx *c = s->c;
    *ran = false;
    if (!s->ps || s->ps_tried) return CNIIC_OK;
    s->ps_tried = true;
    const int dev = c->device >= 0 && c->device < 16 ? c->device : 0, G = (int)s->ps_blocks;
    if (g_ps_cus_in_use[dev].fetch_add(G) + G > ps_cu_count(c->device)) { g_ps_cus_in_use[dev].fetch_sub(G); return CNIIC_OK; }
    std::shared_ptr<void> release(nullptr, [dev, G](void *) { g_ps_cus_in_use[dev].fetch_sub(G); });
    if (!c->pinned_ps) CNIIC_HIP_TRY(c, hipHostMalloc(&c->pinned_ps, 1024, hipHostMallocDefault));
    static_assert(sizeof(PsCold) <= 1024, "the pinned block holds a PsCold");
    PsCold *cold = static_cast<PsCold *>(c->pinned_ps);
    memset(cold, 0, sizeof *cold);
    PsExit *xh = &cold->exit;
    uint8_t *ar = s->ps_arena.as<uint8_t>();
    PsArgs a{};
    a.ckeys = s->ckeys.as<uint32_t>(); a.cweight = s->cweight.as<uint32_t>(); a.labels = s->labels.as<uint8_t>();
    a.ne_cell = s->ne_cell.as<uint32_t>(); a.ne_start = s->ne_start.as<uint32_t>();
    a.cb = reinterpret_cast<const uint32_t *>(ar + s->ps_o_rng); a.ranges_fail = reinterpret_cast<const uint32_t *>(ar + s->ps_o_fail);
    a.lds_budget = s->ps_budget;
    a.pk = s->ps_pk.as<uint32_t>(); a.cconst0 = s->cconst.as<uint2>();
    a.partials = reinterpret_cast<unsigned long long *>(ar + s->ps_o_part); a.bar = reinterpret_cast<PsBar *>(ar);
    cold->cconst_g = s->cconst.as<uint2>(); cold->cent_g = s->cent.as<uint32_t>(); cold->members_out = s->members_last.as<uint64_t>(); cold->wsum_out = s->wsum_last.as<uint64_t>();
    cold->keys = s->keys; cold->gx = s->gidx; cold->seed = s->seed; cold->U = s->gidx.bits ? s->gidx.U : s->U;
    a.st_rw = s->dstate.as<KmDevState>(); a.cold = cold; a.max_iters = s->max_iters;
    a.K = s->K; a.max_skip = s->no_skip ? 0u : s->max_skip; a.agg_iters = kAggLaunches;
    a.test_abort_at = 0;
    if (const char *e = test_env("CNIIC_TEST_PS_ABORT_AT")) a.test_abort_at = (uint32_t)atoi(e);
    a.clean_skip = 1;
    if (const char *e = test_env("CNIIC_KM_PS_CLEANSKIP")) a.clean_skip = atoi(e) ? 1u : 0u;
    uint64_t tmo_ms = 2000;
    if (const char *e = test_env("CNIIC_KM_PS_TIMEOUT_MS")) tmo_ms = (uint64_t)atoll(e);
    a.timeout_ticks = tmo_ms * 100000ull;
    hipEvent_t e0 = nullptr, e1 = nullptr;
    if (s->profile) { CNIIC_HIP_TRY(c, hipEventCreate(&e0)); CNIIC_HIP_TRY(c, hipEventCreate(&e1)); }
    hipExtLaunchKernelGGL(k_rgbw_persist, dim3((uint32_t)G), dim3(kPsThreads), kPsDynBytes, c->stream, e0, e1, 0, a);
    CNIIC_HIP_TRY(c, hipGetLastError());
    if (may_defer && !s->profile) {
        s->ps_pending = true;
        s->ps_hold = release;
        *ran = true;
        return CNIIC_OK;
    }
    CNIIC_HIP_TRY(c, ctx_spin_sync(c));
    const uint32_t status = xh->status;
    ps_learn(c, status, a.test_abort_at != 0);
    if (status != kPsStatusDone) {
        if (e0) { (void)hipEventDestroy(e0); (void)hipEventDestroy(e1); }
        if (test_env("CNIIC_KM_PS_REQUIRE")) return c->fail(CNIIC_ERR_HIP, "kmeans_rgbw: the persistent launch ended with status %u (CNIIC_KM_PS_REQUIRE)", status);
        return CNIIC_OK;
    }
    s->run_stats.iterations = xh->iter; s->run_stats.moved_last = xh->moved_last; s->run_stats.empty_reseeds = xh->reseeds;
    s->run_stats.active = xh->active; s->run_stats.pair_evals = xh->pair_evals;
    s->run_stats_valid = true;
    if (s->profile) {
        float ms = 0.f;
        (void)hipEventElapsedTime(&ms, e0, e1);
        (void)hipEventDestroy(e0); (void)hipEventDestroy(e1);
        KernelTime &kt = c->ktimes["kmeans_rgbw_persist"];
        kt.ms += ms; kt.launches += 1;
        KernelTime &ki = c->ktimes["kmeans_rgbw_persist_iters"];
        ki.ms += ms; ki.launches += xh->iter;
    }
    *ran = true;
    return CNIIC_OK;
}

int km_rgbw_persistent_verdict(KmRgbwState *s, bool *retry) {
    Ctx *c = s->c;
    *retry = false;
    s->ps_pending = false;
    s->ps_hold.reset();
    const PsExit *xh = &static_cast<const PsCold *>(c->pinned_ps)->exit;
    ps_learn(c, xh->status, test_env("CNIIC_TEST_PS_ABORT_AT") != nullptr);
    if (xh->status == kPsStatusDone) {
        s->run_stats.iterations = xh->iter; s->run_stats.moved_last = xh->moved_last; s->run_stats.empty_reseeds = xh->reseeds;
        s->run_stats.active = xh->active; s->run_stats.pair_evals = xh->pair_evals;
        s->run_stats_valid = true;
        return CNIIC_OK;
    }
    if (test_env("CNIIC_KM_PS_REQUIRE")) return c->fail(CNIIC_ERR_HIP, "kmeans_rgbw: the persistent launch ended with status %u (CNIIC_KM_PS_REQUIRE)", xh->status);
    CNIIC_TRY(km_rgbw_run(s, nullptr, false));
    *retry = true;
    return CNIIC_OK;
}

}
```

cniic_amd/csrc/k_kmeans_rgbw.hip:

```cpp
#include <cstdlib>
#include <memory>
#include <vector>


#include <hip/hip_ext.h>

#include "kmeans_rgbw.hpp"

namespace cniic {


__global__ void k_rgbw_init_cent(const uint32_t *__restrict__ keys, uint64_t U, uint32_t K, uint32_t Kpad, uint32_t idbits,
                                 uint2 *__restrict__ cconst, uint32_t *__restrict__ cent, GIdx gx, uint32_t *__restrict__ cent_copy,
                                 uint32_t *__restrict__ moved_list, const uint64_t *__restrict__ U_dev) {
    uint32_t k = blockIdx.x * blockDim.x + threadIdx.x;
    if (U_dev) U = max(*U_dev, (uint64_t)K);
    if (k == 0 && moved_list) moved_list[0] = K;
    if (k < K) {
        uint64_t ppc = U / K;
        uint64_t first = (k < K - 1) ? U - ((uint64_t)k + 1) * ppc : 0;
        uint32_t ck = gx.bits ? gidx_select(gx, first) : keys[first];
        cent[k] = ck;
        if (cent_copy) cent_copy[k] = ck;
        cconst[k] = make_cconst(ck, k, idbits);
// ... 40 lines not shown
#pragma unroll 4
        for (uint32_t k = 0; k < Kpad; k++) {
            const uint2 cc = cconst[k];
#pragma unroll
            for (int j = 0; j < kPPT; j++) {
                uint32_t key = (dot4u8(p[j], cc.x, 0) << (IDBITS + 1)) + cc.y;
                best[j] = max(best[j], key);
            }
        }
#pragma unroll
        for (int j = 0; j < kPPT; j++) {
            if (!valid[j]) continue;
            uint64_t i = base + (uint64_t)j * kAssignThreads + threadIdx.x;
            uint32_t cur = labels[i];
            uint2 cc = tab[cur];
            uint32_t kcur = (dot4u8(p[j], cc.x, 0) << (IDBITS + 1)) + cc.y;
            uint32_t nl = cur;
            if ((best[j] >> IDBITS) > (kcur >> IDBITS)) {
                nl = IDMASK - (best[j] & IDMASK);
                labels[i] = (LabelT)nl;
                moved++;
            }
            uint64_t w = weight[lo + i];
            uint32_t r = (p[j] >> 16) & 255, g = (p[j] >> 8) & 255, b = p[j] & 255;
            atomicAdd(&acc[3 * nl + 0], (unsigned long long)(r * w));
            atomicAdd(&acc[3 * nl + 1], (unsigned long long)(g * w));
            atomicAdd(&acc[3 * nl + 2], (unsigned long long)(b * w));
            atomicAdd(&acc[3 * K + nl], (unsigned long long)w);
            atomicAdd(&acc[4 * K + nl], 1ull);
        }
    }
    moved = block_reduce_sum<kAssignThreads>(moved);
    __syncthreads();
    uint64_t *row = slabs + (size_t)blockIdx.x * (5 * (size_t)K + 2);
    for (uint32_t i = threadIdx.x; i < 5 * K; i += kAssignThreads) row[i] = acc[i];
    if (threadIdx.x == 0) {
        row[5 * (size_t)K] = moved;
        uint64_t per_block = 0;
        for (uint64_t base = (uint64_t)blockIdx.x * kAssignThreads * kPPT; base < n; base += sweep)
            per_block += min((uint64_t)kAssignThreads * kPPT, n - base);
        row[5 * (size_t)K + 1] = per_block * K;
    }
}

__global__ __launch_bounds__(256) void k_slab_reduce(const uint64_t *__restrict__ slabs, uint32_t nrows, uint32_t W,
                                                     uint64_t *__restrict__ partials,
                                                     const KmDevState *__restrict__ st) {
    if (st->done) return;
    __shared__ unsigned long long sh[4][64];
    const uint32_t col = blockIdx.x * 64 + (threadIdx.x & 63);
    const uint32_t rl = threadIdx.x >> 6;
    unsigned long long s = 0;
    if (col < W)
        for (uint32_t r = blockIdx.y * 4 + rl; r < nrows; r += gridDim.y * 4) s += slabs[(size_t)r * W + col];
    sh[rl][threadIdx.x & 63] = s;
    __syncthreads();
    if (rl == 0 && col < W) {
        s = sh[0][threadIdx.x] + sh[1][threadIdx.x] + sh[2][threadIdx.x] + sh[3][threadIdx.x];
        if (s) atomicAdd(reinterpret_cast<unsigned long long *>(partials) + col, s);
    }
}

__global__ __launch_bounds__(256) void k_cell_count(const uint32_t *__restrict__ keys, uint64_t U,
                                                    uint32_t *__restrict__ cell_count) {
    const uint64_t stride = (uint64_t)gridDim.x * blockDim.x;
    const int lane = threadIdx.x & 63;
    for (uint64_t base = (uint64_t)blockIdx.x * blockDim.x; base < U; base += stride) {
        const uint64_t i = base + threadIdx.x;
        bool active = i < U;
        const uint32_t cell = active ? cell_of(keys[i]) : 0;
        for (;;) {
            unsigned long long m = __ballot(active);
            if (!m) break;
            const int leader = __ffsll((long long)m) - 1;
            const uint32_t lc = (uint32_t)__builtin_amdgcn_readlane((int)cell, leader);
            const bool same = active && cell == lc;
            const unsigned long long ms = __ballot(same);
            if (lane == leader) atomicAdd(&cell_count[lc], (uint32_t)__popcll(ms));
            active = active && !same;
        }
    }
}

constexpr uint32_t kCellGroups = kNumCells / 64;
__global__ __launch_bounds__(64) void k_cell_totals(const uint32_t *__restrict__ cell_count, uint2 *__restrict__ tot) {
    const uint32_t v = cell_count[blockIdx.x * 64 + threadIdx.x];
    const uint32_t sum = wave_reduce_sum(v), sweeps = wave_reduce_sum((v + 64 * kSweep - 1) / (64 * kSweep));
    const uint32_t ne = (uint32_t)__popcll(__ballot(v != 0));
    if (threadIdx.x == 0) { tot[blockIdx.x] = make_uint2(sum, ne); tot[kCellGroups + blockIdx.x] = make_uint2(sweeps, 0u); }
}
__global__ __launch_bounds__(64) void k_cell_scan(const uint32_t *__restrict__ cell_count, const uint2 *__restrict__ tot,
                                                  uint32_t *__restrict__ cell_start, uint32_t *__restrict__ cursor,
                                                  uint32_t *__restrict__ ne_cell, uint32_t *__restrict__ ne_start,
                                                  uint32_t *__restrict__ ne_cost, uint32_t *__restrict__ ne_count, uint32_t fixed_cost,
                                                  uint32_t sweep_cost) {
    const uint32_t lane = threadIdx.x, grp = blockIdx.x;
    uint32_t ps = 0, pn = 0, pw = 0;
    for (uint32_t g = lane; g < grp; g += 64) { const uint2 t = tot[g]; ps += t.x; pn += t.y; pw += tot[kCellGroups + g].x; }
    const uint32_t base = wave_reduce_sum(ps), nbase = wave_reduce_sum(pn), wbase = wave_reduce_sum(pw);
    const uint32_t cell = grp * 64 + lane, v = cell_count[cell], sw = (v + 64 * kSweep - 1) / (64 * kSweep);
    const uint32_t start = base + wave_inclusive_scan(v) - v, swb = wbase + wave_inclusive_scan(sw) - sw;
    cell_start[cell] = start;
    if (cursor) cursor[cell] = start;
    const unsigned long long nzm = __ballot(v != 0);
    if (v) {
        const uint32_t m = nbase + (uint32_t)__popcll(nzm & ((1ull << lane) - 1ull));
        ne_cell[m] = cell; ne_start[m] = start; ne_cost[m] = (sweep_cost ? swb * sweep_cost : start) + m * fixed_cost;
    }
    if (grp == kCellGroups - 1 && lane == 63) {
        const uint32_t U = start + v, M = nbase + (uint32_t)__popcll(nzm);
        cell_start[kNumCells] = U;
        ne_start[M] = U;
        ne_cost[M] = (sweep_cost ? (swb + sw) * sweep_cost : U) + M * fixed_cost;
        *ne_count = M;
    }
}

constexpr uint32_t kCellColours = 1u << (3 * kCellShift);
__device__ __forceinline__ uint32_t cell_key(uint32_t cell, uint32_t t) {
    constexpr uint32_t lm = (1u << kCellShift) - 1;
    const CellBox bx = cell_box(cell);
    const uint32_t r = (uint32_t)bx.r0 | (t >> (2 * kCellShift));
    const uint32_t g = (uint32_t)bx.g0 | ((t >> kCellShift) & lm);
    const uint32_t b = (uint32_t)bx.b0 | (t & lm);
    return (r << 16) | (g << 8) | b;
}
__global__ __launch_bounds__(512) void k_cells_count_tbl(const uint32_t *__restrict__ table, uint32_t *__restrict__ cell_count) {
    uint32_t mine = 0;
    for (uint32_t t = threadIdx.x; t < kCellColours; t += 512) mine += table[cell_key(blockIdx.x, t)] != 0;
    const uint32_t n = block_reduce_sum<512>(mine);
    if (threadIdx.x == 0) cell_count[blockIdx.x] = n;
}
template <typename LabelT>
__global__ __launch_bounds__(512) void k_cells_write_tbl(const uint32_t *__restrict__ table, const uint32_t *__restrict__ weight,
                                                         const uint32_t *__restrict__ cell_start, uint64_t U, uint32_t K,
                                                         uint32_t *__restrict__ ckeys, uint32_t *__restrict__ cweight,
                                                         uint32_t *__restrict__ crank, LabelT *__restrict__ labels, GIdx gx) {
    __shared__ uint32_t wsum[512 / 64];
    __shared__ uint32_t s_run;
    const uint32_t s = cell_start[blockIdx.x], e = cell_start[blockIdx.x + 1];
    if (s == e) return;
    if (threadIdx.x == 0) s_run = s;
    __syncthreads();
    for (uint32_t t0 = 0; t0 < kCellColours; t0 += 512) {
        const uint32_t key = cell_key(blockIdx.x, t0 + threadIdx.x);
        const uint32_t v = table[key];
        const uint32_t run = s_run;
        const uint32_t pos = run + block_exclusive_scan<512>(v != 0, wsum);
        if (v) {
            const uint32_t rank = v - 1;
            ckeys[pos] = key;
            cweight[pos] = weight[rank];
            crank[pos] = rank;
            labels[pos] = (LabelT)init_label(gx.bits ? gidx_rank(gx, key) : rank, U, K);
        }
        if (threadIdx.x == 511) s_run = pos + (v != 0);
        __syncthreads();
    }
}

__global__ __launch_bounds__(256) void k_cell_scatter(const uint32_t *__restrict__ keys, const uint32_t *__restrict__ weight,
                                                      uint64_t U, uint32_t *__restrict__ cursor,
                                                      uint32_t *__restrict__ ckeys, uint32_t *__restrict__ cweight,
                                                      uint32_t *__restrict__ crank) {
    const uint64_t stride = (uint64_t)gridDim.x * blockDim.x;
    const int lane = threadIdx.x & 63;
    for (uint64_t base = (uint64_t)blockIdx.x * blockDim.x; base < U; base += stride) {
        const uint64_t i = base + threadIdx.x;
        bool active = i < U;
        const uint32_t key = active ? keys[i] : 0;
        const uint32_t cell = cell_of(key);
        uint32_t pos = 0;
        for (;;) {
            unsigned long long m = __ballot(active);
            if (!m) break;
            const int leader = __ffsll((long long)m) - 1;
            const uint32_t lc = (uint32_t)__builtin_amdgcn_readlane((int)cell, leader);
            const bool same = active && cell == lc;
            const unsigned long long ms = __ballot(same);
            uint32_t b = 0;
            if (lane == leader) b = atomicAdd(&cursor[lc], (uint32_t)__popcll(ms));
            b = (uint32_t)__builtin_amdgcn_readlane((int)b, leader);
            if (same) pos = b + (uint32_t)__popcll(ms & ((1ull << lane) - 1));
            active = active && !same;
        }
        if (i < U) {
            ckeys[pos] = key;
            cweight[pos] = weight[i];
            crank[pos] = (uint32_t)i;
        }
    }
}

// ... 789 lines not shown
__global__ void k_widen_labels(const LabelT *__restrict__ in, const uint32_t *__restrict__ rank, uint32_t *__restrict__ out,
                               uint64_t lo, uint64_t hi) {
    const uint64_t stride = (uint64_t)gridDim.x * blockDim.x;
    for (uint64_t i = lo + (uint64_t)blockIdx.x * blockDim.x + threadIdx.x; i < hi; i += stride) {
        if (rank) out[rank[i]] = in[i];
        else out[i - lo] = in[i - lo];
    }
}
template <typename LabelT>
__global__ void k_narrow_labels(const uint32_t *__restrict__ in, LabelT *__restrict__ out, uint64_t n) {
    const uint64_t stride = (uint64_t)gridDim.x * blockDim.x;
    for (uint64_t i = (uint64_t)blockIdx.x * blockDim.x + threadIdx.x; i < n; i += stride) out[i] = (LabelT)in[i];
}
template <typename LabelT>
__global__ void k_labels_to_canonical(const LabelT *__restrict__ in, const uint32_t *__restrict__ rank, LabelT *__restrict__ out,
                                      uint64_t U) {
    const uint64_t stride = (uint64_t)gridDim.x * blockDim.x;
    for (uint64_t i = (uint64_t)blockIdx.x * blockDim.x + threadIdx.x; i < U; i += stride) out[rank[i]] = in[i];
}
__global__ void k_set_cconst(const uint32_t *__restrict__ cent, uint32_t K, uint32_t Kpad, uint32_t idbits,
                             uint2 *__restrict__ cconst) {
    uint32_t k = blockIdx.x * blockDim.x + threadIdx.x;
    if (k < K) cconst[k] = make_cconst(cent[k], k, idbits);
    else if (k < Kpad) cconst[k] = make_uint2(0u, 0u);
}

static inline uint32_t grid_1d(uint64_t n, uint32_t cap = 2048) {
    return (uint32_t)std::min<uint64_t>(std::max<uint64_t>(ceil_div(n, 256), 1), cap);
}

#define KM_ALLOC(buf, bytes)                                                                       \
    do {                                                                                           \
        hipError_t _e = (buf).alloc(bytes);                                                        \
        if (_e != hipSuccess) { delete s; return c->fail(CNIIC_ERR_HIP, "kmeans_rgbw: hipMalloc(%llu) failed: %s", \
                                                        (unsigned long long)(bytes), hipGetErrorString(_e)); } \
    } while (0)

int km_rgbw_create(Ctx *c, const uint32_t *keys_d, const uint32_t *weight_d, uint64_t U, uint32_t shard,
                   uint32_t nshards, uint32_t K, const cniic_kmeans_opts *opts, void *partials_dev,
                   const uint32_t *rank_table_d, KmRgbwState **out, const uint32_t *cell_count_d, const void *gbits_d,
                   const uint32_t *gprefix_d, uint64_t Ug, bool points_follow, const uint64_t *points_dev) {
    if (K == 0 || U == 0 || nshards == 0 || shard >= nshards) return c->fail(CNIIC_ERR_BAD_ARG, "kmeans_rgbw: bad sizes");
    if (points_follow && (!gbits_d || !cell_count_d || nshards != 1 || (opts && (opts->flags & CNIIC_KM_BRUTE_FORCE))))
        return c->fail(CNIIC_ERR_BAD_ARG, "kmeans_rgbw: points written by the caller need the cell counts and the colour index");
    if (!points_follow && gbits_d && (!rank_table_d || nshards != 1 || (opts && (opts->flags & CNIIC_KM_BRUTE_FORCE))))
        return c->fail(CNIIC_ERR_BAD_ARG, "kmeans_rgbw: a share of a larger point list needs the table-driven cells path, unsharded");
    const uint64_t lo = U * shard / nshards, hi = U * (shard + 1) / nshards;
    const uint64_t Ulist = gbits_d ? Ug : U;
    if (points_dev && !points_follow) return c->fail(CNIIC_ERR_BAD_ARG, "kmeans_rgbw: a device-side point count needs points_follow");
    if (!points_dev && Ulist / K == 0) return c->fail(CNIIC_ERR_TOO_FEW_POINTS, "kmeans: %llu points for %u clusters (src/kmeans.rs:68)",
                                       (unsigned long long)Ulist, K);
    if (K > 65535) return c->fail(CNIIC_ERR_UNSUPPORTED, "kmeans_rgbw: K=%u > 65535 not supported", K);
    if (K > 2048 && (nshards != 1 || (opts && (opts->flags & CNIIC_KM_BRUTE_FORCE))))
        return c->fail(CNIIC_ERR_UNSUPPORTED, "kmeans_rgbw: K=%u > 2048 runs unsharded on the cell-major arrays only", K);
    if (U >= (1ull << 32)) return c->fail(CNIIC_ERR_BAD_ARG, "kmeans_rgbw: too many points");
    auto *s = new KmRgbwState();
    s->c = c; s->U = U; s->lo = lo; s->hi = hi; s->K = K; s->shard = shard; s->nshards = nshards;
    s->Kpad = (K + 3) & ~3u;
    s->wide = K > 256;
    s->big = K > 2048;
    s->idbits = s->wide ? 12 : 8;
    s->seed = (opts && opts->seed) ? opts->seed : kDefaultSeed;
    s->max_iters = opts ? opts->max_iters : 0;
    s->cells = !(opts && (opts->flags & CNIIC_KM_BRUTE_FORCE));
    s->profile = opts && (opts->flags & CNIIC_KM_PROFILE);
    s->no_skip = opts && (opts->flags & CNIIC_KM_NO_SKIP);
    if (const char *ms = test_env("CNIIC_KM_MAXSKIP")) s->max_skip = std::min<uint32_t>((uint32_t)atoi(ms), kMaxMovedSkip);
    if (const char *fa = test_env("CNIIC_TEST_FAIL_AT_LAUNCH")) s->fail_at = atol(fa);
    s->keys = keys_d; s->weight = weight_d;
    s->gidx = GIdx{static_cast<const unsigned long long *>(gbits_d), gprefix_d, Ug};
    const uint64_t n = hi - lo;
    const uint64_t W = 5 * (uint64_t)K + 2;
    const uint64_t lab_bytes = s->wide ? 2 : 1;
    KM_ALLOC(s->cconst, (uint64_t)s->Kpad * 8);
    s->res_cent = (sizeof(KmDevState) + 255) & ~255ull;
    s->res_members = s->res_cent + (((uint64_t)K * 4 + 7) & ~7ull);
    s->res_wsum = s->res_members + (uint64_t)K * 8;
    s->res_bytes = s->res_wsum + (uint64_t)K * 8;
    s->fused = s->cells && !s->wide && !(test_env("CNIIC_KM_UNFUSED") && atoi(test_env("CNIIC_KM_UNFUSED")));
    {
        auto up = [](uint64_t x) { return (x + 255) & ~255ull; };
        const uint64_t o_part = up(s->res_bytes), o_run = o_part + up(partials_dev ? 0 : W * 8), o_fp = o_run + up(s->cells ? W * 8 : 0);
        const uint64_t o_fr = o_fp + up(s->fused ? 3 * W * 8 : 0), o_fc = o_fr + up(s->fused ? 2 * W * 8 : 0);
        const uint64_t o_mv = o_fc + up(s->fused ? 2 * (uint64_t)K * 4 : 0), total = o_mv + up(s->cells ? ((uint64_t)K + 1) * 4 : 0);
        KM_ALLOC(s->arena, total);
        (void)hipMemsetAsync(s->arena.p, 0, total, c->stream);
        uint8_t *a = s->arena.as<uint8_t>();
        s->resblk.view(a, s->res_bytes);
        if (partials_dev) {
            s->partials = reinterpret_cast<uint64_t *>(partials_dev);
            (void)hipMemsetAsync(s->partials, 0, W * 8, c->stream);
        } else {
            s->partials_own.view(a + o_part, W * 8);
            s->partials = s->partials_own.as<uint64_t>();
        }
        if (s->cells) {
            s->running.view(a + o_run, W * 8);
            s->moved_list.view(a + o_mv, ((uint64_t)K + 1) * 4);
        }
        if (s->fused) {
            s->fused_partials.view(a + o_fp, 3 * W * 8);
            s->fused_running.view(a + o_fr, 2 * W * 8);
            s->fused_cent.view(a + o_fc, 2 * (uint64_t)K * 4);
        }
    }
    s->dstate.view(s->resblk.p, sizeof(KmDevState));
    s->cent.view(static_cast<uint8_t *>(s->resblk.p) + s->res_cent, (uint64_t)K * 4);
    s->members_last.view(static_cast<uint8_t *>(s->resblk.p) + s->res_members, (uint64_t)K * 8);
    s->wsum_last.view(static_cast<uint8_t *>(s->resblk.p) + s->res_wsum, (uint64_t)K * 8);
    hipLaunchKernelGGL(k_rgbw_init_cent, dim3(ceil_div(s->Kpad, 256)), dim3(256), 0, c->stream, keys_d, Ulist, K, s->Kpad, s->idbits,
                       s->cconst.as<uint2>(), s->cent.as<uint32_t>(), s->gidx, s->fused ? s->fused_cent.as<uint32_t>() : (uint32_t *)nullptr,
                       s->cells ? s->moved_list.as<uint32_t>() : (uint32_t *)nullptr, points_dev);
    if (s->cells) {
        s->nblocks = (uint32_t)std::min<uint64_t>(std::max<uint64_t>(ceil_div(U / nshards, s->wide ? 1024 : 64), 1), s->wide ? 4096u : kCellBlocks);
        if (const uint64_t mb = c->opt(CNIIC_OPT_KM_MAX_BLOCKS, "CNIIC_KM_MAX_BLOCKS", 0)) {
            const uint32_t cap = std::max(3u, (uint32_t)std::min<uint64_t>(mb, kCellBlocks) / 3 * 3);
            if (!s->wide && nshards == 1 && s->nblocks > cap) s->nblocks = cap;
        }
        if (s->wide) s->nblocks = (s->nblocks + 7) & ~7u;
        KM_ALLOC(s->labels, std::max<uint64_t>(U, 1) * lab_bytes);
        KM_ALLOC(s->ckeys, U * 4);
        KM_ALLOC(s->cweight, U * 4);
        if (!points_follow) KM_ALLOC(s->crank, U * 4);
        KM_ALLOC(s->cell_start, ((uint64_t)kNumCells + 1) * 4);
        KM_ALLOC(s->ne_cell, (uint64_t)kNumCells * 4);
        KM_ALLOC(s->ne_start, ((uint64_t)kNumCells + 1) * 4);
        KM_ALLOC(s->ne_cost, ((uint64_t)kNumCells + 1) * 4);
        KM_ALLOC(s->ne_count, 4);
        const uint32_t G = s->nblocks * (s->wide ? 1u : (uint32_t)kCellWaves) * nshards;
        KM_ALLOC(s->wfirst, ((uint64_t)G + 1) * 4);
        if (!s->big) KM_ALLOC(s->cell_rec, (uint64_t)kNumCells * cell_rec_words((K + 63) / 64) * 4);
        DevBuf count, cursor, cell_tot;
        KM_ALLOC(count, (uint64_t)kNumCells * 4);
        KM_ALLOC(cell_tot, (uint64_t)kCellGroups * 8 * 2);
        if (points_follow) {
            hipLaunchKernelGGL(k_cell_totals, dim3(kCellGroups), dim3(64), 0, c->stream, cell_count_d, cell_tot.as<uint2>());
            hipLaunchKernelGGL(k_cell_scan, dim3(kCellGroups), dim3(64), 0, c->stream, cell_count_d, (const uint2 *)cell_tot.as<uint2>(), s->cell_start.as<uint32_t>(),
                               (uint32_t *)nullptr, s->ne_cell.as<uint32_t>(), s->ne_start.as<uint32_t>(), s->ne_cost.as<uint32_t>(),
                               s->ne_count.as<uint32_t>(), kCellFixedCost, kCellSweepCost);
        } else if (rank_table_d) {
            const uint32_t *cnt = cell_count_d;
            if (!cnt) {
                hipLaunchKernelGGL(k_cells_count_tbl, dim3(kNumCells), dim3(512), 0, c->stream, rank_table_d, count.as<uint32_t>());
                cnt = count.as<uint32_t>();
            }
            hipLaunchKernelGGL(k_cell_totals, dim3(kCellGroups), dim3(64), 0, c->stream, cnt, cell_tot.as<uint2>());
            hipLaunchKernelGGL(k_cell_scan, dim3(kCellGroups), dim3(64), 0, c->stream, cnt, (const uint2 *)cell_tot.as<uint2>(), s->cell_start.as<uint32_t>(),
                               (uint32_t *)nullptr, s->ne_cell.as<uint32_t>(), s->ne_start.as<uint32_t>(), s->ne_cost.as<uint32_t>(),
                               s->ne_count.as<uint32_t>(), kCellFixedCost, kCellSweepCost);
            if (s->wide)
                hipLaunchKernelGGL(k_cells_write_tbl<uint16_t>, dim3(kNumCells), dim3(512), 0, c->stream, rank_table_d, weight_d,
                                   s->cell_start.as<uint32_t>(), Ulist, K, s->ckeys.as<uint32_t>(), s->cweight.as<uint32_t>(),
                                   s->crank.as<uint32_t>(), s->labels.as<uint16_t>(), s->gidx);
            else
                hipLaunchKernelGGL(k_cells_write_tbl<uint8_t>, dim3(kNumCells), dim3(512), 0, c->stream, rank_table_d, weight_d,
                                   s->cell_start.as<uint32_t>(), Ulist, K, s->ckeys.as<uint32_t>(), s->cweight.as<uint32_t>(),
                                   s->crank.as<uint32_t>(), s->labels.as<uint8_t>(), s->gidx);
        } else {
            KM_ALLOC(cursor, (uint64_t)kNumCells * 4);
            (void)hipMemsetAsync(count.p, 0, (uint64_t)kNumCells * 4, c->stream);
            const uint32_t g = grid_1d(U);
            hipLaunchKernelGGL(k_cell_count, dim3(g), dim3(256), 0, c->stream, keys_d, U, count.as<uint32_t>());
            hipLaunchKernelGGL(k_cell_totals, dim3(kCellGroups), dim3(64), 0, c->stream, count.as<uint32_t>(), cell_tot.as<uint2>());
            hipLaunchKernelGGL(k_cell_scan, dim3(kCellGroups), dim3(64), 0, c->stream, count.as<uint32_t>(), (const uint2 *)cell_tot.as<uint2>(), s->cell_start.as<uint32_t>(),
                               cursor.as<uint32_t>(), s->ne_cell.as<uint32_t>(), s->ne_start.as<uint32_t>(), s->ne_cost.as<uint32_t>(),
                               s->ne_count.as<uint32_t>(), kCellFixedCost, kCellSweepCost);
            hipLaunchKernelGGL(k_cell_scatter, dim3(g), dim3(256), 0, c->stream, keys_d, weight_d, U, cursor.as<uint32_t>(),
                               s->ckeys.as<uint32_t>(), s->cweight.as<uint32_t>(), s->crank.as<uint32_t>());
            if (s->wide)
                hipLaunchKernelGGL(k_rgbw_init_labels<uint16_t>, dim3(grid_1d(U)), dim3(256), 0, c->stream, s->crank.as<uint32_t>(), U,
                                   (uint64_t)0, U, K, s->labels.as<uint16_t>());
            else
                hipLaunchKernelGGL(k_rgbw_init_labels<uint8_t>, dim3(grid_1d(U)), dim3(256), 0, c->stream, s->crank.as<uint32_t>(), U,
                                   (uint64_t)0, U, K, s->labels.as<uint8_t>());
        }
        s->wfirst_waves = G;
        if (s->fused && nshards == 1 && c->ps_div <= 1 && c->opt(CNIIC_OPT_KM_LOOP, "CNIIC_KM_LOOP", 0) == 0) {
            const int rc_ps = ps_prepare(s);
            if (rc_ps != CNIIC_OK) { delete s; return rc_ps; }
        }
        hipError_t e = hipGetLastError();
        if (e != hipSuccess) { delete s; return c->fail(CNIIC_ERR_HIP, "kmeans_rgbw setup: %s", hipGetErrorString(e)); }
    } else {
        s->nblocks = (uint32_t)std::min<uint64_t>(std::max<uint64_t>(ceil_div(n, (uint64_t)kAssignThreads * kPPT), 1), kMaxBlocks);
        KM_ALLOC(s->labels, std::max<uint64_t>(n, 1) * lab_bytes);
        KM_ALLOC(s->slabs, (uint64_t)s->nblocks * W * 8);
        if (s->wide)
            hipLaunchKernelGGL(k_rgbw_init_labels<uint16_t>, dim3(grid_1d(n)), dim3(256), 0, c->stream, (const uint32_t *)nullptr, U, lo,
                               hi, K, s->labels.as<uint16_t>());
        else
            hipLaunchKernelGGL(k_rgbw_init_labels<uint8_t>, dim3(grid_1d(n)), dim3(256), 0, c->stream, (const uint32_t *)nullptr, U, lo,
                               hi, K, s->labels.as<uint8_t>());
    }
    hipError_t e = hipGetLastError();
    if (e != hipSuccess) { delete s; return c->fail(CNIIC_ERR_HIP, "kmeans_rgbw init launch: %s", hipGetErrorString(e)); }
    *out = s;
    return CNIIC_OK;
}

void km_rgbw_destroy(KmRgbwState *s) { delete s; }

static int launch_update(KmRgbwState *s, int mode) {
    Ctx *c = s->c;
    hipLaunchKernelGGL(k_rgbw_update, dim3(1), dim3(256), 0, c->stream, s->partials, s->running.as<uint64_t>(), mode, s->keys,
                       s->gidx.bits ? s->gidx.U : s->U,
                       s->K, s->idbits, s->seed, s->max_iters, s->cconst.as<uint2>(), s->cent.as<uint32_t>(),
                       s->members_last.as<uint64_t>(), s->wsum_last.as<uint64_t>(), s->cells ? s->moved_list.as<uint32_t>() : nullptr,
                       s->dstate.as<KmDevState>(), s->gidx);
    CNIIC_HIP_TRY(c, hipGetLastError());
    return CNIIC_OK;
}

int km_rgbw_fold_initial(KmRgbwState *) { return CNIIC_OK; }

int km_rgbw_set_state(KmRgbwState *s, const uint8_t *centroids_h, const uint32_t *labels_d_u32) {
    Ctx *c = s->c;
    if (s->cells) return c->fail(CNIIC_ERR_BAD_ARG, "km_rgbw_set_state needs the brute-force state");
    std::vector<uint32_t> ck(s->K);
    for (uint32_t k = 0; k < s->K; k++)
        ck[k] = ((uint32_t)centroids_h[3 * k] << 16) | ((uint32_t)centroids_h[3 * k + 1] << 8) | centroids_h[3 * k + 2];
    CNIIC_HIP_TRY(c, hipMemcpyAsync(s->cent.p, ck.data(), (size_t)s->K * 4, hipMemcpyHostToDevice, c->stream));
    hipLaunchKernelGGL(k_set_cconst, dim3(ceil_div(s->Kpad, 256)), dim3(256), 0, c->stream, s->cent.as<uint32_t>(), s->K,
                       s->Kpad, s->idbits, s->cconst.as<uint2>());
    const uint64_t n = s->hi - s->lo;
    if (n) {
        if (s->wide)
            hipLaunchKernelGGL(k_narrow_labels<uint16_t>, dim3(grid_1d(n)), dim3(256), 0, c->stream, labels_d_u32, s->labels.as<uint16_t>(), n);
        else
            hipLaunchKernelGGL(k_narrow_labels<uint8_t>, dim3(grid_1d(n)), dim3(256), 0, c->stream, labels_d_u32, s->labels.as<uint8_t>(), n);
    }
    CNIIC_HIP_TRY(c, hipGetLastError());
    CNIIC_HIP_TRY(c, hipStreamSynchronize(c->stream));
    return CNIIC_OK;
}

static void ensure_wave_ranges(KmRgbwState *s) {
    if (!s->wfirst_waves) return;
    hipLaunchKernelGGL(k_wave_ranges, dim3(ceil_div((uint64_t)s->wfirst_waves + 1, 256)), dim3(256), 0, s->c->stream, s->ne_cost.as<uint32_t>(),
                       s->ne_count.as<uint32_t>(), s->wfirst_waves, s->wfirst.as<uint32_t>());
    s->wfirst_waves = 0;
}

static void launch_assign(KmRgbwState *s, hipEvent_t ev_start = nullptr, hipEvent_t ev_stop = nullptr, const FusedUpdate *fused = nullptr,
                          unsigned long long *part_fused = nullptr) {
    Ctx *c = s->c;
    if (s->cells) ensure_wave_ranges(s);
    FusedUpdate fz{};
// ... 412 lines not shown
```

cniic_amd/csrc/k_points.hip:

```cpp
#include "common.hpp"
#include "device_utils.hpp"

namespace cniic {

constexpr uint32_t kSpBuckets = 512;
constexpr uint32_t kSpBins = 1u << 15;
constexpr uint32_t kSpChunk = 1u << 16;
constexpr int kSpThreads = 1024;
constexpr uint32_t kSpSliceMin = 1u << 17;
constexpr uint32_t kSpSlices = 8;
constexpr uint32_t kSpWaves = kSpThreads / 64;

__device__ __forceinline__ uint32_t sp_bucket(uint32_t key) {
    return (((key >> 21) & 7u) << 6) | (((key >> 13) & 7u) << 3) | ((key >> 5) & 7u);
}
__device__ __forceinline__ uint32_t sp_bin(uint32_t key) {
    const uint32_t r = (key >> 16) & 31u, g = (key >> 8) & 31u, b = key & 31u;
    return ((r >> 3) << 13) | ((g >> 3) << 11) | ((b >> 3) << 9) | ((r & 7u) << 6) | ((g & 7u) << 3) | (b & 7u);
}
__device__ __forceinline__ uint32_t sp_key(uint32_t bucket, uint32_t bin) {
    const uint32_t r = (((bucket >> 6) & 7u) << 5) | (((bin >> 13) & 3u) << 3) | ((bin >> 6) & 7u);
    const uint32_t g = (((bucket >> 3) & 7u) << 5) | (((bin >> 11) & 3u) << 3) | ((bin >> 3) & 7u);
    const uint32_t b = ((bucket & 7u) << 5) | (((bin >> 9) & 3u) << 3) | (bin & 7u);
    return (r << 16) | (g << 8) | b;
}

__device__ __forceinline__ uint32_t scan512(uint32_t v, uint32_t *wsum) { return block_exclusive_scan<kSpThreads>(v, wsum); }

template <typename F> __device__ __forceinline__ void sp_for_pixels(const uint8_t *__restrict__ rgb, uint64_t npx, F &&f) {
    const uint64_t p0 = (uint64_t)blockIdx.x * kSpChunk, p1 = min(npx, p0 + kSpChunk);
    const uint4 *v = reinterpret_cast<const uint4 *>(rgb);
    for (uint64_t g = p0 / 16 + threadIdx.x; g * 16 < p1; g += kSpThreads) {
        uint32_t key[16];
        if (g * 16 + 16 <= p1) {
            load16px_keys(v + 3 * g, key);
            f(g * 16, key, 16u);
        } else {
            const uint32_t m = (uint32_t)(p1 - g * 16);
            for (uint32_t i = 0; i < 16; i++) key[i] = i < m ? rgb_key(rgb + 3 * (g * 16 + i)) : 0u;
            f(g * 16, key, m);
        }
    }
}

__global__ __launch_bounds__(kSpThreads) void k_sp_count(const uint8_t *__restrict__ rgb, uint64_t npx, uint32_t *__restrict__ cnt) {
    __shared__ uint32_t h[kSpBuckets];
    if (threadIdx.x < kSpBuckets) h[threadIdx.x] = 0;
    __syncthreads();
    sp_for_pixels(rgb, npx, [&](uint64_t, const uint32_t (&key)[16], uint32_t m) {
#pragma unroll
        for (uint32_t i = 0; i < 16; i++)
            if (i < m) atomicAdd(&h[sp_bucket(key[i])], 1u);
    });
    __syncthreads();
    if (threadIdx.x < kSpBuckets) cnt[(size_t)blockIdx.x * kSpBuckets + threadIdx.x] = h[threadIdx.x];
}

__global__ __launch_bounds__(256) void k_sp_colscan(const uint32_t *__restrict__ cnt, uint32_t nchunks, uint32_t *__restrict__ pre,
                                                    uint32_t *__restrict__ total) {
    __shared__ uint32_t wsum[256 / 64];
    const uint32_t b = blockIdx.x, per = (nchunks + 255) / 256;
    const uint32_t c0 = threadIdx.x * per, c1 = min(c0 + per, nchunks);
    uint32_t s = 0;
    for (uint32_t c = c0; c < c1; c++) s += cnt[(size_t)c * kSpBuckets + b];
    uint32_t run = block_exclusive_scan<256>(s, wsum);
    for (uint32_t c = c0; c < c1; c++) {
        pre[(size_t)c * kSpBuckets + b] = run;
        run += cnt[(size_t)c * kSpBuckets + b];
    }
    if (threadIdx.x == 255) total[b] = run;
}

__global__ __launch_bounds__(kSpBuckets) void k_sp_bstart(const uint32_t *__restrict__ total, uint32_t *__restrict__ bstart,
                                                          uint32_t *__restrict__ sstart) {
    __shared__ uint32_t wsum[kSpBuckets / 64];
    const uint32_t t = total[threadIdx.x];
    const uint32_t ex = block_exclusive_scan<kSpBuckets>(t, wsum);
    bstart[threadIdx.x] = ex;
    if (threadIdx.x == kSpBuckets - 1) bstart[kSpBuckets] = ex + t;
    sstart[threadIdx.x] = block_exclusive_scan<kSpBuckets>(min(t, kSpBins), wsum);
}

template <int STEPS, typename F> __device__ __forceinline__ void sp_walk_sorted(const uint32_t *off, uint32_t n, F &&f) {
    const uint32_t lane = threadIdx.x & 63, wv = threadIdx.x >> 6;
    const uint32_t per = (n + kSpThreads - 1) / kSpThreads * 64;
    const uint32_t j0 = wv * per, j1 = min(n, j0 + per);
    if (j0 >= j1) return;
    const uint32_t jj = min(j0 + lane, j1 - 1);
    uint32_t lo = 0, hi = kSpBuckets;
    while (hi - lo > 1) {
        const uint32_t mid = (lo + hi) >> 1;
        if (off[mid] <= jj) lo = mid; else hi = mid;
    }
    uint32_t b = lo, end = off[b + 1];
    for (uint32_t j = j0 + lane; j < j1; j += 64 * STEPS) {
        uint32_t jb[STEPS];
#pragma unroll
        for (int t = 0; t < STEPS; t++) {
            const uint32_t q = j + 64 * t;
            jb[t] = 0xffffffffu;
            if (q < j1) {
                while (q >= end) { b++; end = off[b + 1]; }
                jb[t] = b;
            }
        }
        f(j, jb);
    }
}

__global__ __launch_bounds__(kSpThreads) void k_sp_scatter(const uint8_t *__restrict__ rgb, uint64_t npx, const uint32_t *__restrict__ cnt,
                                                           const uint32_t *__restrict__ pre, const uint32_t *__restrict__ bstart,
                                                           uint16_t *__restrict__ part, uint16_t *__restrict__ prank) {
    extern __shared__ __align__(16) uint8_t sp_lds[];
    uint16_t *stage = reinterpret_cast<uint16_t *>(sp_lds);
    uint32_t *off = reinterpret_cast<uint32_t *>(sp_lds + (size_t)kSpChunk * 2);
    uint32_t *cur = off + kSpBuckets + 1;
    __shared__ uint32_t wsum[kSpWaves];
    const uint32_t *mycnt = cnt + (size_t)blockIdx.x * kSpBuckets;
    const uint32_t n_b = threadIdx.x < kSpBuckets ? mycnt[threadIdx.x] : 0u;
    const uint32_t ex = scan512(n_b, wsum);
    if (threadIdx.x < kSpBuckets) { off[threadIdx.x] = ex; cur[threadIdx.x] = 0; }
    if (threadIdx.x == kSpBuckets - 1) off[kSpBuckets] = ex + n_b;
    __syncthreads();
    sp_for_pixels(rgb, npx, [&](uint64_t first, const uint32_t (&key)[16], uint32_t m) {
        uint32_t rk[16];
#pragma unroll
        for (uint32_t i = 0; i < 16; i++) {
            rk[i] = 0;
            if (i < m) {
                const uint32_t b = sp_bucket(key[i]);
                rk[i] = off[b] + atomicAdd(&cur[b], 1u);
                stage[rk[i]] = (uint16_t)sp_bin(key[i]);
            }
        }
        if (m == 16) {
            uint4 *d = reinterpret_cast<uint4 *>(prank + first);
            d[0] = make_uint4(rk[0] | (rk[1] << 16), rk[2] | (rk[3] << 16), rk[4] | (rk[5] << 16), rk[6] | (rk[7] << 16));
            d[1] = make_uint4(rk[8] | (rk[9] << 16), rk[10] | (rk[11] << 16), rk[12] | (rk[13] << 16), rk[14] | (rk[15] << 16));
        } else {
            for (uint32_t i = 0; i < m; i++) prank[first + i] = (uint16_t)rk[i];
        }
    });
    __syncthreads();
    const uint32_t lane = threadIdx.x & 63, wv = threadIdx.x >> 6;
    const uint32_t *mypre = pre + (size_t)blockIdx.x * kSpBuckets;
    const uint32_t mb = wv + kSpWaves * (lane & 31);
    const uint32_t m_n = mycnt[mb], m_dst = bstart[mb] + mypre[mb], m_off = off[mb];
    for (uint32_t k = 0; k < kSpBuckets / kSpWaves; k++) {
        const uint32_t n = __shfl(m_n, k, 64), d0 = __shfl(m_dst, k, 64), o = __shfl(m_off, k, 64);
        for (uint32_t i = lane; i < n; i += 64) part[(size_t)d0 + i] = stage[o + i];
    }
}

template <typename F> __device__ __forceinline__ void sp_for_entries(const uint16_t *__restrict__ part, uint64_t s, uint64_t e, F &&f) {
    const uint64_t a = min(e, (s + 3) & ~3ull), z = a + ((e - a) & ~3ull);
    for (uint64_t i = s + threadIdx.x; i < a; i += kSpThreads) { const uint32_t v = part[i]; f(i, v, v, v, v, 1u); }
    constexpr uint64_t kStep = 4 * (uint64_t)kSpThreads;
    for (uint64_t i = a + 4 * (uint64_t)threadIdx.x; i < z; i += 4 * kStep) {
        uint2 q[4];
#pragma unroll
        for (int t = 0; t < 4; t++) q[t] = i + t * kStep < z ? *reinterpret_cast<const uint2 *>(part + i + t * kStep) : make_uint2(0u, 0u);
#pragma unroll
        for (int t = 0; t < 4; t++)
            if (i + t * kStep < z) f(i + t * kStep, q[t].x & 0xffffu, q[t].x >> 16, q[t].y & 0xffffu, q[t].y >> 16, 4u);
    }
    for (uint64_t i = z + threadIdx.x; i < e; i += kSpThreads) { const uint32_t v = part[i]; f(i, v, v, v, v, 1u); }
}

__device__ __forceinline__ void sp_bucket_hist(const uint16_t *__restrict__ part, uint64_t s, uint64_t e, uint32_t *hist) {
    for (uint32_t i = threadIdx.x; i < kSpBins; i += kSpThreads) hist[i] = 0;
    __syncthreads();
    sp_for_entries(part, s, e, [&](uint64_t, uint32_t a, uint32_t b, uint32_t c, uint32_t d, uint32_t m) {
        if (m == 1) { atomicAdd(&hist[a], 1u); return; }
        const bool same = a == b && b == c && c == d;
        const uint32_t first = __builtin_amdgcn_readfirstlane(a);
        if (__all(same && a == first) && __popcll(__ballot(1)) == 64) {
            if ((threadIdx.x & 63) == 0) atomicAdd(&hist[a], 256u);
        } else if (same) {
            atomicAdd(&hist[a], 4u);
        } else {
            atomicAdd(&hist[a], 1u); atomicAdd(&hist[b], 1u); atomicAdd(&hist[c], 1u); atomicAdd(&hist[d], 1u);
        }
    });
    __syncthreads();
}


__global__ __launch_bounds__(kSpThreads) void k_sp_hist(const uint16_t *__restrict__ part, const uint32_t *__restrict__ bstart,
                                                        const uint32_t *__restrict__ sstart, uint32_t *__restrict__ cell_count,
                                                        uint32_t *__restrict__ bits32, uint16_t *__restrict__ sbin,
                                                        uint32_t *__restrict__ scnt) {
    extern __shared__ __align__(16) uint8_t sp_lds[];
    uint32_t *hist = reinterpret_cast<uint32_t *>(sp_lds);
    __shared__ uint32_t wsum[kSpWaves];
    const uint32_t bucket = blockIdx.x;
    const uint64_t s = bstart[bucket], e = bstart[bucket + 1];
    const uint32_t r5 = threadIdx.x >> 5, g5 = threadIdx.x & 31;
    const uint32_t word_at = ((((bucket >> 6) & 7u) << 5 | r5) << 11) | ((((bucket >> 3) & 7u) << 5 | g5) << 3) | (bucket & 7u);
    if (s == e) {
        if (threadIdx.x < 64) cell_count[bucket * 64 + threadIdx.x] = 0;
        bits32[word_at] = 0;
        return;
    }
    sp_bucket_hist(part, s, e, hist);
    uint32_t word = 0;
#pragma unroll
    for (uint32_t bq = 0; bq < 4; bq++) {
        const uint32_t base = ((r5 >> 3) << 13) | ((g5 >> 3) << 11) | (bq << 9) | ((r5 & 7u) << 6) | ((g5 & 7u) << 3);
#pragma unroll
        for (uint32_t j = 0; j < 8; j++) word |= (hist[base + j] != 0 ? 1u : 0u) << (bq * 8 + j);
    }
    bits32[word_at] = word;
    const uint32_t lane = threadIdx.x & 63, wv = threadIdx.x >> 6;
    const unsigned long long lt_mask = (1ull << lane) - 1ull;
    uint32_t mine = 0;
    for (uint32_t c4 = 0; c4 < 4; c4++) {
        uint32_t in_cell = 0;
        for (uint32_t st = 0; st < 8; st++) in_cell += (uint32_t)__popcll(__ballot(hist[wv * 2048 + c4 * 512 + st * 64 + lane] != 0));
        if (lane == 0) cell_count[bucket * 64 + wv * 4 + c4] = in_cell;
        mine += in_cell;
    }
    if (lane == 0) wsum[wv] = mine;
    __syncthreads();
    uint32_t pos0 = sstart[bucket];
    for (uint32_t i = 0; i < wv; i++) pos0 += wsum[i];
    for (uint32_t st = 0; st < 32; st++) {
        const uint32_t bin = wv * 2048 + st * 64 + lane, v = hist[bin];
        const unsigned long long bm = __ballot(v != 0);
        if (v) {
            const uint32_t pos = pos0 + (uint32_t)__popcll(bm & lt_mask);
// ... 104 lines not shown
    const uint32_t ex = scan512(n_b, wsum);
    if (threadIdx.x < kSpBuckets) off[threadIdx.x] = ex;
    if (threadIdx.x == kSpBuckets - 1) off[kSpBuckets] = ex + n_b;
    __syncthreads();
    if (threadIdx.x < kSpBuckets) gsrc[threadIdx.x] = bstart[threadIdx.x] + mypre[threadIdx.x] - off[threadIdx.x];
    __syncthreads();
    sp_walk_sorted<8>(off, off[kSpBuckets], [&](uint32_t j, const uint32_t (&jb)[8]) {
        LabelT got[8];
#pragma unroll
        for (int t = 0; t < 8; t++) got[t] = jb[t] != 0xffffffffu ? partlab[(size_t)(gsrc[jb[t]] + (j + 64 * t))] : (LabelT)0;
#pragma unroll
        for (int t = 0; t < 8; t++)
            if (jb[t] != 0xffffffffu) stage[j + 64 * t] = got[t];
    });
    __syncthreads();
    const uint64_t p0 = (uint64_t)blockIdx.x * kSpChunk, p1 = min(npx, p0 + kSpChunk);
    for (uint64_t g = p0 / 16 + threadIdx.x; g * 16 < p1; g += kSpThreads) {
        const uint64_t first = g * 16;
        const uint32_t m = (uint32_t)min<uint64_t>(16, p1 - first);
        uint32_t lab[16];
        if (m == 16) {
            const uint4 *rp = reinterpret_cast<const uint4 *>(prank + first);
            const uint4 r0 = rp[0], r1 = rp[1];
            const uint32_t rw[8] = {r0.x, r0.y, r0.z, r0.w, r1.x, r1.y, r1.z, r1.w};
#pragma unroll
            for (uint32_t i = 0; i < 16; i++) lab[i] = stage[(rw[i >> 1] >> (16 * (i & 1))) & 0xffffu];
            if (sizeof(LabelT) == 1) {
                uint32_t w[4];
#pragma unroll
                for (int j = 0; j < 4; j++) w[j] = lab[4 * j] | (lab[4 * j + 1] << 8) | (lab[4 * j + 2] << 16) | (lab[4 * j + 3] << 24);
                *reinterpret_cast<uint4 *>(pixlab + first) = make_uint4(w[0], w[1], w[2], w[3]);
            } else {
                uint4 *d = reinterpret_cast<uint4 *>(pixlab + first);
                d[0] = make_uint4(lab[0] | (lab[1] << 16), lab[2] | (lab[3] << 16), lab[4] | (lab[5] << 16), lab[6] | (lab[7] << 16));
                d[1] = make_uint4(lab[8] | (lab[9] << 16), lab[10] | (lab[11] << 16), lab[12] | (lab[13] << 16), lab[14] | (lab[15] << 16));
            }
        } else {
            for (uint32_t i = 0; i < m; i++) pixlab[first + i] = stage[prank[first + i]];
        }
    }
}

static int sp_set_lds(Ctx *c) {
    static bool done = false;
    if (done) return CNIIC_OK;
    const int big = 140 * 1024;
    CNIIC_HIP_TRY(c, hipFuncSetAttribute(reinterpret_cast<const void *>(k_sp_scatter), hipFuncAttributeMaxDynamicSharedMemorySize, big));
    CNIIC_HIP_TRY(c, hipFuncSetAttribute(reinterpret_cast<const void *>(k_sp_hist), hipFuncAttributeMaxDynamicSharedMemorySize, big));
    CNIIC_HIP_TRY(c, hipFuncSetAttribute(reinterpret_cast<const void *>(k_sp_partlab<uint8_t>), hipFuncAttributeMaxDynamicSharedMemorySize, big));
    CNIIC_HIP_TRY(c, hipFuncSetAttribute(reinterpret_cast<const void *>(k_sp_partlab<uint16_t>), hipFuncAttributeMaxDynamicSharedMemorySize, big));
    CNIIC_HIP_TRY(c, hipFuncSetAttribute(reinterpret_cast<const void *>(k_sp_pixlab<uint8_t>), hipFuncAttributeMaxDynamicSharedMemorySize, big));
    CNIIC_HIP_TRY(c, hipFuncSetAttribute(reinterpret_cast<const void *>(k_sp_pixlab<uint16_t>), hipFuncAttributeMaxDynamicSharedMemorySize, big));
    done = true;
    return CNIIC_OK;
}

int sp_build(Ctx *c, const uint8_t *rgb_d, uint64_t npx, SpPlan *plan) {
    if (npx == 0 || (reinterpret_cast<uintptr_t>(rgb_d) & 15)) return c->fail(CNIIC_ERR_BAD_ARG, "sp_build: empty or unaligned image");
    CNIIC_TRY(sp_set_lds(c));
    plan->npx = npx;
    plan->nchunks = (uint32_t)ceil_div(npx, kSpChunk);
    const uint64_t nc = plan->nchunks;
    CNIIC_HIP_TRY(c, plan->cnt.alloc(nc * kSpBuckets * 4));
    CNIIC_HIP_TRY(c, plan->pre.alloc(nc * kSpBuckets * 4));
    CNIIC_HIP_TRY(c, plan->bstart.alloc(((uint64_t)kSpBuckets + 1) * 4));
    CNIIC_HIP_TRY(c, plan->part.alloc(npx * 2 + 16));
    CNIIC_HIP_TRY(c, plan->prank.alloc((npx + 16) * 2));
    CNIIC_HIP_TRY(c, plan->cell_count.alloc((uint64_t)kNumCells * 4));
    const uint64_t smax = std::min<uint64_t>(npx, 1ull << 24);
    CNIIC_HIP_TRY(c, plan->sstart.alloc((uint64_t)kSpBuckets * 4));
    CNIIC_HIP_TRY(c, plan->sbin.alloc(smax * 2));
    CNIIC_HIP_TRY(c, plan->scnt.alloc(smax * 4));
    CNIIC_HIP_TRY(c, plan->bits.alloc((1ull << 18) * 8));
    CNIIC_HIP_TRY(c, plan->wprefix.alloc((1ull << 18) * 4));
    DevBuf total, blocktot;
    CNIIC_HIP_TRY(c, total.alloc((uint64_t)kSpBuckets * 4));
    CNIIC_HIP_TRY(c, blocktot.alloc(256 * 4));
    CNIIC_HIP_TRY(c, plan->total.alloc(8));
    CNIIC_HIP_TRY(c, ctx_pinned_u(c));
    if (!c->u_ev) CNIIC_HIP_TRY(c, hipEventCreateWithFlags(&c->u_ev, hipEventDisableTiming));
    hipLaunchKernelGGL(k_sp_count, dim3(plan->nchunks), dim3(kSpThreads), 0, c->stream, rgb_d, npx, plan->cnt.as<uint32_t>());
    hipLaunchKernelGGL(k_sp_colscan, dim3(kSpBuckets), dim3(256), 0, c->stream, plan->cnt.as<uint32_t>(), plan->nchunks,
                       plan->pre.as<uint32_t>(), total.as<uint32_t>());
    hipLaunchKernelGGL(k_sp_bstart, dim3(1), dim3(kSpBuckets), 0, c->stream, total.as<uint32_t>(), plan->bstart.as<uint32_t>(),
                       plan->sstart.as<uint32_t>());
    hipLaunchKernelGGL(k_sp_scatter, dim3(plan->nchunks), dim3(kSpThreads), (size_t)kSpChunk * 2 + kSpBuckets * 8 + 16, c->stream, rgb_d, npx,
                       plan->cnt.as<uint32_t>(), plan->pre.as<uint32_t>(), plan->bstart.as<uint32_t>(), plan->part.as<uint16_t>(),
                       plan->prank.as<uint16_t>());
    hipLaunchKernelGGL(k_sp_hist, dim3(kSpBuckets), dim3(kSpThreads), (size_t)kSpBins * 4, c->stream, plan->part.as<uint16_t>(),
                       plan->bstart.as<uint32_t>(), plan->sstart.as<uint32_t>(), plan->cell_count.as<uint32_t>(), plan->bits.as<uint32_t>(),
                       plan->sbin.as<uint16_t>(), plan->scnt.as<uint32_t>());
    hipLaunchKernelGGL(k_bits_prefix, dim3(256), dim3(256), 0, c->stream, plan->bits.as<unsigned long long>(), plan->wprefix.as<uint32_t>(),
                       blocktot.as<uint32_t>());
    CNIIC_TRY(gidx_finish(c, plan->wprefix.as<uint32_t>(), blocktot.as<uint32_t>(), plan->total.as<uint64_t>()));
    CNIIC_HIP_TRY(c, hipGetLastError());
    CNIIC_HIP_TRY(c, hipMemcpyAsync(c->pinned_u + kPuSpCount.at, plan->total.p, 8, hipMemcpyDeviceToHost, c->stream));
    CNIIC_HIP_TRY(c, hipEventRecord(c->u_ev, c->stream));
    return CNIIC_OK;
}

int sp_wait_count(Ctx *c, SpPlan *plan) {
    CNIIC_HIP_TRY(c, hipEventSynchronize(c->u_ev));
    plan->U = c->pinned_u[kPuSpCount.at];
    return CNIIC_OK;
}

int sp_emit(Ctx *c, const SpPlan *plan, const uint32_t *cell_start_d, uint32_t *ckeys_d, uint32_t *cweight_d, void *labels_d, bool wide,
            uint32_t K, const void *gbits_d, const uint32_t *gprefix_d, uint64_t Ug, const uint64_t *Ug_dev) {
    const GIdx gx{static_cast<const unsigned long long *>(gbits_d), gprefix_d, Ug};
    hipLaunchKernelGGL(k_sp_emit, dim3(kSpBuckets * kSpEmitSplit), dim3(256), 0, c->stream, plan->sstart.as<uint32_t>(), plan->sbin.as<uint16_t>(),
                       plan->scnt.as<uint32_t>(), SpEmit{cell_start_d, ckeys_d, cweight_d, labels_d, K, wide ? 1u : 0u, gx, Ug_dev});
    CNIIC_HIP_TRY(c, hipGetLastError());
    return CNIIC_OK;
}

__global__ __launch_bounds__(256) void k_occ_from_bits(const uint32_t *__restrict__ bits32, uint32_t *__restrict__ occ) {
    const uint32_t i = blockIdx.x * 256 + threadIdx.x;
    const uint32_t byte = (bits32[i >> 2] >> (8 * (i & 3))) & 255u;
    uint32_t v = 0;
#pragma unroll
    for (int j = 0; j < 8; j++) v |= ((byte >> j) & 1u) << (4 * j);
    occ[i] = v;
}
int sp_occupancy(Ctx *c, const SpPlan *plan, uint32_t *occ_d) {
    hipLaunchKernelGGL(k_occ_from_bits, dim3((1u << 21) / 256), dim3(256), 0, c->stream, plan->bits.as<uint32_t>(), occ_d);
    CNIIC_HIP_TRY(c, hipGetLastError());
    return CNIIC_OK;
}

int sp_pixel_labels(Ctx *c, const SpPlan *plan, const uint8_t *rgb_d, const uint32_t *cell_start_d, const uint32_t *ckeys_d,
                    const void *labels_d, bool wide, void *pixlab_d) {
    DevBuf partlab;
    const uint64_t lb = wide ? 2 : 1;
    CNIIC_HIP_TRY(c, partlab.alloc(plan->npx * lb + 16));
    if (wide) {
        hipLaunchKernelGGL(k_sp_partlab<uint16_t>, dim3(kSpBuckets, plan->npx >= 2 * (uint64_t)kSpSliceMin ? kSpSlices : 1), dim3(kSpThreads), (size_t)kSpBins * 2, c->stream, plan->part.as<uint16_t>(),
                           plan->bstart.as<uint32_t>(), cell_start_d, ckeys_d, static_cast<const uint16_t *>(labels_d), partlab.as<uint16_t>());
        hipLaunchKernelGGL(k_sp_pixlab<uint16_t>, dim3(plan->nchunks), dim3(kSpThreads), (size_t)kSpChunk * 2 + kSpBuckets * 8 + 16, c->stream, rgb_d,
                           plan->npx, plan->cnt.as<uint32_t>(), plan->pre.as<uint32_t>(), plan->bstart.as<uint32_t>(), partlab.as<uint16_t>(),
                           plan->prank.as<uint16_t>(), static_cast<uint16_t *>(pixlab_d));
    } else {
        hipLaunchKernelGGL(k_sp_partlab<uint8_t>, dim3(kSpBuckets, plan->npx >= 2 * (uint64_t)kSpSliceMin ? kSpSlices : 1), dim3(kSpThreads), (size_t)kSpBins, c->stream, plan->part.as<uint16_t>(),
                           plan->bstart.as<uint32_t>(), cell_start_d, ckeys_d, static_cast<const uint8_t *>(labels_d), partlab.as<uint8_t>());
        hipLaunchKernelGGL(k_sp_pixlab<uint8_t>, dim3(plan->nchunks), dim3(kSpThreads), (size_t)kSpChunk + kSpBuckets * 8 + 16, c->stream, rgb_d,
                           plan->npx, plan->cnt.as<uint32_t>(), plan->pre.as<uint32_t>(), plan->bstart.as<uint32_t>(), partlab.as<uint8_t>(),
                           plan->prank.as<uint16_t>(), static_cast<uint8_t *>(pixlab_d));
    }
    CNIIC_HIP_TRY(c, hipGetLastError());
    return CNIIC_OK;
}

}
```

cniic_amd/csrc/kmeans_rgbw.hpp:

```cpp
#pragma once
#include <cstdlib>
#include <memory>
#include <vector>

#include "common.hpp"
#include "device_utils.hpp"

namespace cniic {

constexpr uint32_t kBias = 1u << 18;
constexpr int kPPT = 8;
constexpr int kAssignThreads = 256;
constexpr uint32_t kMaxBlocks = 512;
constexpr int kCellWaves = 8;
__host__ __device__ constexpr uint32_t km_scap(uint32_t K) { return K <= 256 ? (K + 1) / 2 : (K + 1) / 2 < 512u ? (K + 1) / 2 : 512u; }
__host__ __device__ constexpr uint32_t km_ccap(uint32_t K) { return K <= 256 ? K : 256u; }
constexpr uint32_t kCellWavesBig = 12;
constexpr uint32_t kBigBlocksFrom = 10;
constexpr uint32_t kAggLaunches = 3;
constexpr uint32_t kCellBlocks = 256 * 3;
constexpr int kSweep = 4;
constexpr uint32_t kCellFixedCost = 512;
constexpr uint32_t kCellSweepCost = 256;

struct KmRgbwState {
    Ctx *c = nullptr;
    uint64_t U = 0, lo = 0, hi = 0, seed = 0, max_iters = 0;
    uint32_t K = 0, Kpad = 0, idbits = 8, nblocks = 1;
    bool wide = false;
    bool big = false;
    bool cells = true;
    bool profile = false;
    bool no_skip = false;
    const uint32_t *keys = nullptr, *weight = nullptr;
    DevBuf labels;
    DevBuf cconst, slabs, partials_own, dstate, cent, members_last, wsum_last;
    DevBuf arena;
    DevBuf resblk;
    uint64_t res_cent = 0, res_members = 0, res_wsum = 0, res_bytes = 0;
    std::unique_ptr<LaggedPoll> lagged;
    DevBuf ckeys, cweight, crank, cell_start, running, ne_cell, ne_start, ne_cost, ne_count, wfirst;
    DevBuf cell_rec, moved_list;
    uint32_t wfirst_waves = 0;
    GIdx gidx{nullptr, nullptr, 0};
    DevBuf fused_partials, fused_running, fused_cent;
    bool fused = false;
    cniic_kmeans_stats run_stats{};
    bool run_stats_valid = false;
    uint32_t max_skip = 64;
    long fail_at = -1;
    uint32_t shard = 0, nshards = 1;
    uint64_t *partials = nullptr;
    bool ps = false, ps_tried = false;
    bool ps_pending = false;
    std::shared_ptr<void> ps_hold;
    uint32_t ps_blocks = 0;
    DevBuf ps_arena;
    DevBuf ps_pk;
    uint64_t ps_o_part = 0, ps_o_fail = 0, ps_o_rng = 0;
    uint32_t ps_budget = 0;
};

constexpr uint32_t kPsChunks = 24;
constexpr uint32_t kPsSlotsMax = 32;
constexpr uint32_t kPsScap = 96;
constexpr uint32_t kPsRecWords = 11;
constexpr uint32_t kPsMaxCells = 2048;
constexpr uint32_t kPsOffCell = 5 * 256 * 8 + 256 * 8 + kPsSlotsMax * kPsScap * 4;
constexpr uint32_t kPsDynBytes = 160 * 1024 - 3072;
constexpr uint32_t kPsPartWords = 5 * 256 + 8;
__host__ __device__ constexpr uint32_t ps_cell_bytes(uint32_t C) { return 16u + ((C + 3u) & ~3u) * (4u + 4u + kPsRecWords * 4u + 2u + 2u + 1u); }
struct alignas(128) PsLine { uint32_t v; uint32_t pad[31]; };
struct PsBar { PsLine xcount[8], xgen[8], xblocks[8], top, topgen, count, gen, abort_; };
constexpr uint32_t kPsStatusDone = 1, kPsStatusAborted = 2, kPsStatusRanges = 3;
struct PsExit { uint32_t status, pad; uint64_t iter, moved_last, reseeds, active, pair_evals; };
void launch_rgbw_assign_big(Ctx *c, const uint32_t *ckeys, const uint32_t *cweight, uint64_t U, uint32_t K, const uint32_t *cent, uint16_t *labels,
                            unsigned long long *partials, const KmDevState *st);
int ps_prepare(KmRgbwState *s);
int km_rgbw_run_persistent(KmRgbwState *s, bool *ran, bool may_defer);
int km_rgbw_persistent_verdict(KmRgbwState *s, bool *retry);
constexpr uint32_t kAggMin = 16;


__device__ __forceinline__ uint32_t dot4u8(uint32_t a, uint32_t b, uint32_t acc) {
    return __builtin_amdgcn_udot4(a, b, acc, false);
}

__device__ __forceinline__ uint2 make_cconst(uint32_t ckey, uint32_t k, uint32_t idbits) {
    uint32_t h = dot4u8(ckey, ckey, 0);
    uint32_t idmask = (1u << idbits) - 1;
    return make_uint2(ckey, ((kBias - h) << idbits) | (idmask - k));
}

struct CellBox { int32_t r0, g0, b0; };
__device__ __forceinline__ CellBox super_box(uint32_t sup) {
    return CellBox{(int32_t)((sup / (kSupersPerDim * kSupersPerDim)) << (kCellShift + 2)),
                   (int32_t)(((sup / kSupersPerDim) % kSupersPerDim) << (kCellShift + 2)),
                   (int32_t)((sup % kSupersPerDim) << (kCellShift + 2))};
}
__device__ __forceinline__ CellBox cell_box(uint32_t c) {
    const CellBox sb = super_box(c >> kSuperShift);
    return CellBox{sb.r0 + (int32_t)(((c >> 4) & 3) << kCellShift), sb.g0 + (int32_t)(((c >> 2) & 3) << kCellShift),
                   sb.b0 + (int32_t)((c & 3) << kCellShift)};
}

constexpr uint32_t kRecComplete = 0x80000000u;
__host__ __device__ constexpr uint32_t cell_rec_words(uint32_t MW) { return (2 + 2 * MW + 15) & ~15u; }
constexpr uint32_t kMaxMovedSkip = 64;

__device__ __forceinline__ uint32_t pack_rgb(int32_t r, int32_t g, int32_t b) { return ((uint32_t)r << 16) | ((uint32_t)g << 8) | (uint32_t)b; }

__device__ __forceinline__ uint32_t centre_dist(uint32_t ck, const CellBox &bx, int32_t ext) {
    const int32_t h = (ext + 1) >> 1;
    const uint32_t c = pack_rgb(bx.r0 + h, bx.g0 + h, bx.b0 + h);
    return dot4u8(ck, ck, dot4u8(c, c, 0)) - 2u * dot4u8(ck, c, 0);
}

struct Dominance {
    uint32_t ppk, lopk, hipk;
    int32_t cp, ext;
    __device__ __forceinline__ void set(const CellBox &bx, int32_t e, uint32_t pivot) {
        ppk = pivot & 0xffffffu;
        ext = e;
        lopk = pack_rgb(bx.r0, bx.g0, bx.b0);
        hipk = pack_rgb(bx.r0 + e, bx.g0 + e, bx.b0 + e);
        cp = (int32_t)dot4u8(ppk, ppk, 0) - 2 * (int32_t)dot4u8(ppk, lopk, 0) - e * (int32_t)dot4u8(ppk, 0x010101u, 0);
    }
    __device__ __forceinline__ int32_t worst(uint32_t ck) const {
        const uint32_t v = ck;
        return cp - (int32_t)dot4u8(v, v, 0) + (int32_t)dot4u8(v, hipk, dot4u8(v, lopk, 0)) + __mul24(ext, (int32_t)__builtin_amdgcn_sad_u8(ppk, v, 0u));
    }
};

__device__ __forceinline__ uint32_t wave_all_min(uint32_t v) { return wave_reduce_min(v); }

__device__ __forceinline__ uint32_t nearest_to_centre(const uint2 *list, uint32_t n, const CellBox &bx, int32_t ext, int lane) {
    uint32_t bd = 0xfffffu, be = 4095u;
    for (uint32_t e = lane; e < n; e += 64) {
        const uint32_t d = centre_dist(list[e].x, bx, ext);
        if (d < bd) { bd = d; be = e; }
    }
    return wave_all_min((bd << 12) | be) & 4095u;
}

__device__ __forceinline__ uint32_t lanes_below(unsigned long long bm) {
    return __builtin_amdgcn_mbcnt_hi((uint32_t)(bm >> 32), __builtin_amdgcn_mbcnt_lo((uint32_t)bm, 0u));
}

__device__ __forceinline__ uint32_t build_super(const uint2 *tab, uint32_t K, uint32_t sup, int lane, unsigned long long lt_mask,
                                                uint2 *S, uint32_t cap) {
    constexpr int32_t ext = (1 << (kCellShift + 2)) - 1;
    const CellBox bx = super_box(sup);
    Dominance dm;
    dm.set(bx, ext, tab[nearest_to_centre(tab, K, bx, ext, lane)].x);
    uint32_t n = 0;
    for (uint32_t k0 = 0; k0 < K; k0 += 64) {
// ... 26 lines not shown
```

Measured before the change: 10030 Mpixels/s.

## Batch palette uploads, fuse small scan kernels, and write totals straight to pinned memory

The Huffman code tables and header are packed into one pinned staging block and sent with a single host-to-device copy, and the first pack-count block writes the header into the output stream on the GPU. Scan kernels now store their totals directly into pinned host memory with a system fence, which removes the separate device-to-host copies. Several small kernels are merged: a single-block scan for mid-sized chunk counts, the bucket-start scan folded into the scatter kernel, and the cell totals folded into the cell scan. The intent is to cut launch count and per-call host/copy latency, at the cost of redundant per-block scans and reliance on fenced writes to pinned memory.

```diff
diff --git a/cniic_amd/csrc/codec.cpp b/cniic_amd/csrc/codec.cpp
--- a/cniic_amd/csrc/codec.cpp
+++ b/cniic_amd/csrc/codec.cpp
@@ -527,18 +527,30 @@
         return c->fail(CNIIC_ERR_BAD_ARG, "huffman: cannot build code");
     host_trace().mark("tree+codes (host)");
     StreamOut so(c, out, cap, len);
-    CNIIC_TRY(so.begin(header, (nbits + 7) / 8));
+    CNIIC_TRY(so.begin_sized(header.size(), (nbits + 7) / 8));
     host_trace().mark("so.begin");
-    DevBuf clen_d, ccode_d;
-    CNIIC_HIP_TRY(c, clen_d.alloc(K));
-    CNIIC_HIP_TRY(c, ccode_d.alloc((uint64_t)K * 8));
-    CNIIC_HIP_TRY(c, hipMemcpyAsync(clen_d.p, clen.data(), K, hipMemcpyHostToDevice, c->stream));
-    CNIIC_HIP_TRY(c, hipMemcpyAsync(ccode_d.p, ccode.data(), (size_t)K * 8, hipMemcpyHostToDevice, c->stream));
+    const uint64_t o_len = (uint64_t)K * 8, o_hdr = (o_len + K + 7) & ~7ull, up_bytes = o_hdr + header.size();
+    DevBuf up_d;
+    CNIIC_HIP_TRY(c, up_d.alloc(up_bytes));
+    const uint8_t *hdr_d = nullptr;
+    if (n && up_bytes <= (uint64_t)kPuPaletteUp.words * 8) {
+        CNIIC_HIP_TRY(c, ctx_pinned_u(c));
+        uint8_t *up = reinterpret_cast<uint8_t *>(c->pinned_u + kPuPaletteUp.at);
+        memcpy(up, ccode.data(), (size_t)K * 8);
+        memcpy(up + o_len, clen.data(), K);
+        memcpy(up + o_hdr, header.data(), header.size());
+        CNIIC_HIP_TRY(c, hipMemcpyAsync(up_d.p, up, up_bytes, hipMemcpyHostToDevice, c->stream));
+        hdr_d = up_d.as<uint8_t>() + o_hdr;
+    } else {
+        CNIIC_TRY(so.put_header(header));
+        CNIIC_HIP_TRY(c, hipMemcpyAsync(up_d.as<uint8_t>() + o_len, clen.data(), K, hipMemcpyHostToDevice, c->stream));
+        CNIIC_HIP_TRY(c, hipMemcpyAsync(up_d.p, ccode.data(), (size_t)K * 8, hipMemcpyHostToDevice, c->stream));
+    }
     uint64_t packed_bits = 0;
     {
         ScopedKernelTimer t(c, "huff_pack");
-        CNIIC_TRY(huff_pack_labels(c, pixlab.p, n, wide, K, clen_d.as<uint8_t>(), ccode_d.as<uint64_t>(), so.dev,
-                                   (uint64_t)header.size() * 8, &packed_bits));
+        CNIIC_TRY(huff_pack_labels(c, pixlab.p, n, wide, K, up_d.as<uint8_t>() + o_len, up_d.as<uint64_t>(), so.dev,
+                                   (uint64_t)header.size() * 8, &packed_bits, hdr_d));
         t.stop(1);
     }
     host_trace().mark("pack (+sync)");
diff --git a/cniic_amd/csrc/common.hpp b/cniic_amd/csrc/common.hpp
--- a/cniic_amd/csrc/common.hpp
+++ b/cniic_amd/csrc/common.hpp
@@ -196,12 +196,14 @@
 constexpr PuSlot kPuHufTotals{3, 2};
 constexpr PuSlot kPuDeltaOverflow{5, 1};
 constexpr PuSlot kPuDeltaPacked{6, 1};
+constexpr PuSlot kPuPackLabels{7, 1};
 constexpr PuSlot kPuPaletteWeights{8, 4096};
 constexpr PuSlot kPuHdecode{4104, 3};
 constexpr PuSlot kPuTrieTotals{4108, 6};
 constexpr PuSlot kPuLeafRuns{4114, 3};
-constexpr PuSlot kPuSlots[] = {kPuSpCount, kPuPointCount, kPuImageCount, kPuHufTotals, kPuDeltaOverflow, kPuDeltaPacked,
-                               kPuPaletteWeights, kPuHdecode, kPuTrieTotals, kPuLeafRuns};
+constexpr PuSlot kPuPaletteUp{4117, 2048};
+constexpr PuSlot kPuSlots[] = {kPuSpCount, kPuPointCount, kPuImageCount, kPuHufTotals, kPuDeltaOverflow, kPuDeltaPacked, kPuPackLabels,
+                               kPuPaletteWeights, kPuHdecode, kPuTrieTotals, kPuLeafRuns, kPuPaletteUp};
 constexpr bool pu_slots_disjoint() {
     uint32_t end = 0;
     for (const PuSlot &s : kPuSlots) {
@@ -450,7 +452,7 @@
 };
 int occupancy_pack(Ctx *c, const uint32_t *table_d, uint32_t *occ_d);
 int gidx_build(Ctx *c, const uint32_t *occ_d, DevBuf &bits, DevBuf &wprefix, uint64_t *U_h, DevBuf *total_keep = nullptr);
-int gidx_finish(Ctx *c, uint32_t *wprefix_d, const uint32_t *blocktot_d, uint64_t *total_d);
+int gidx_finish(Ctx *c, uint32_t *wprefix_d, const uint32_t *blocktot_d, uint64_t *total_d, uint64_t *total_pinned = nullptr);
 
 struct SpPlan {
     uint64_t npx = 0, U = 0;
@@ -619,7 +621,7 @@
 int huff_tree_codes(Ctx *c, const uint32_t *left_d, const uint32_t *right_d, const uint32_t *nleaves_d, const uint64_t *counts_d, uint32_t n,
                     uint32_t root, int sym_kind, uint8_t *len_d, uint64_t *code_d, uint64_t *off_d, uint64_t *totals_d);
 int huff_tree_serialize_dev(Ctx *c, const uint32_t *keys_d, const uint64_t *off_d, uint32_t n, int sym_kind, uint8_t *trie_d, uint64_t trie_bytes);
-int pack_scan(Ctx *c, const uint32_t *chunk_bits_d, uint32_t nchunks, uint64_t *chunk_off_d, uint64_t *total_d);
+int pack_scan(Ctx *c, const uint32_t *chunk_bits_d, uint32_t nchunks, uint64_t *chunk_off_d, uint64_t *total_d, uint64_t *total_pinned = nullptr);
 uint32_t pack_img_cap();
 int huff_pack_keys(Ctx *c, const uint32_t *keys_or_null_d, const uint8_t *rgb_or_null_d, uint64_t n,
                    const uint32_t *rank_table_d, const uint8_t *len_d, const uint64_t *code_d,
@@ -635,7 +637,7 @@
                          const uint64_t *code_d, uint64_t U, uint32_t *packed_d, uint8_t *out_d, uint64_t bit_base, uint64_t *nbits_h);
 int pixel_labels(Ctx *c, const uint8_t *rgb_d, uint64_t n, const void *key2label_d, bool wide, void *pixlab_d);
 int huff_pack_labels(Ctx *c, const void *pixlab_d, uint64_t n, bool wide, uint32_t K, const uint8_t *clen_d,
-                     const uint64_t *ccode_d, uint8_t *out_d, uint64_t bit_base, uint64_t *nbits_h);
+                     const uint64_t *ccode_d, uint8_t *out_d, uint64_t bit_base, uint64_t *nbits_h, const uint8_t *hdr_d = nullptr);
 int scatter_labels_by_key(Ctx *c, const uint32_t *keys_d, const void *labels_d, bool wide, uint64_t U, void *key2label_d);
 int frame_label_hist(Ctx *c, const void *pixlab_d, uint64_t npf, uint64_t lab_stride, uint32_t frames, bool wide, uint32_t K, uint32_t *out_d );
 int huff_pack_labels_frames(Ctx *c, const void *pixlab_d, uint64_t npf, uint64_t lab_stride, uint32_t frames, bool wide, uint32_t K, const uint8_t *clen_d,
diff --git a/cniic_amd/csrc/k_hist.hip b/cniic_amd/csrc/k_hist.hip
--- a/cniic_amd/csrc/k_hist.hip
+++ b/cniic_amd/csrc/k_hist.hip
@@ -362,20 +362,23 @@
     if (threadIdx.x == 255) blocktot[blockIdx.x] = run;
 }
 __global__ __launch_bounds__(256) void k_gidx_finish(uint32_t *__restrict__ wprefix, const uint32_t *__restrict__ blocktot,
-                                                     uint64_t *__restrict__ total) {
+                                                     uint64_t *__restrict__ total, uint64_t *__restrict__ total_host) {
     __shared__ uint32_t wsum[256 / 64];
     __shared__ uint32_t boff[256];
     const uint32_t t = blocktot[threadIdx.x];
     const uint32_t ex = block_exclusive_scan<256>(t, wsum);
     boff[threadIdx.x] = ex;
-    if (blockIdx.x == 0 && threadIdx.x == 255) *total = (uint64_t)ex + t;
+    if (blockIdx.x == 0 && threadIdx.x == 255) {
+        *total = (uint64_t)ex + t;
+        if (total_host) { *total_host = (uint64_t)ex + t; __threadfence_system(); }
+    }
     __syncthreads();
     const uint32_t add = boff[blockIdx.x];
     for (uint32_t i = threadIdx.x; i < 1024; i += 256) wprefix[blockIdx.x * 1024 + i] += add;
 }
 
-int gidx_finish(Ctx *c, uint32_t *wprefix_d, const uint32_t *blocktot_d, uint64_t *total_d) {
-    hipLaunchKernelGGL(k_gidx_finish, dim3(256), dim3(256), 0, c->stream, wprefix_d, blocktot_d, total_d);
+int gidx_finish(Ctx *c, uint32_t *wprefix_d, const uint32_t *blocktot_d, uint64_t *total_d, uint64_t *total_pinned) {
+    hipLaunchKernelGGL(k_gidx_finish, dim3(256), dim3(256), 0, c->stream, wprefix_d, blocktot_d, total_d, total_pinned);
     CNIIC_HIP_TRY(c, hipGetLastError());
     return CNIIC_OK;
 }
@@ -397,7 +400,7 @@
     hipLaunchKernelGGL(k_gidx_words, dim3(256), dim3(256), 0, c->stream, occ_d, bits.as<unsigned long long>(), wprefix.as<uint32_t>(),
                        blocktot.as<uint32_t>());
     hipLaunchKernelGGL(k_gidx_finish, dim3(256), dim3(256), 0, c->stream, wprefix.as<uint32_t>(), (const uint32_t *)blocktot.as<uint32_t>(),
-                       tot.as<uint64_t>());
+                       tot.as<uint64_t>(), (uint64_t *)nullptr);
     CNIIC_HIP_TRY(c, hipGetLastError());
     CNIIC_HIP_TRY(c, hipMemcpyAsync(U_h, tot.p, 8, hipMemcpyDeviceToHost, c->stream));
     if (!total_keep) CNIIC_HIP_TRY(c, hipStreamSynchronize(c->stream));
diff --git a/cniic_amd/csrc/k_huff.hip b/cniic_amd/csrc/k_huff.hip
--- a/cniic_amd/csrc/k_huff.hip
+++ b/cniic_amd/csrc/k_huff.hip
@@ -85,7 +85,7 @@
 
 __global__ __launch_bounds__(1024) void k_pack_scan_local(const uint32_t *__restrict__ chunk_bits, uint32_t nchunks,
                                                           uint64_t *__restrict__ chunk_off, uint64_t *__restrict__ blocktot,
-                                                          uint64_t *__restrict__ total_bits) {
+                                                          uint64_t *__restrict__ total_bits, uint64_t *__restrict__ total_host) {
     __shared__ uint32_t wsum[1024 / 64];
     const uint32_t i = blockIdx.x * 1024 + threadIdx.x;
     const uint32_t v = i < nchunks ? chunk_bits[i] : 0u;
@@ -93,11 +93,15 @@
     if (i < nchunks) chunk_off[i] = ex;
     if (threadIdx.x == 1023) {
         blocktot[blockIdx.x] = (uint64_t)ex + v;
-        if (gridDim.x == 1) *total_bits = (uint64_t)ex + v;
+        if (gridDim.x == 1) {
+            *total_bits = (uint64_t)ex + v;
+            if (total_host) { *total_host = (uint64_t)ex + v; __threadfence_system(); }
+        }
     }
 }
 __global__ __launch_bounds__(1024) void k_pack_scan_add(uint32_t nchunks, uint64_t *__restrict__ chunk_off,
-                                                        const uint64_t *__restrict__ blocktot, uint64_t *__restrict__ total_bits) {
+                                                        const uint64_t *__restrict__ blocktot, uint64_t *__restrict__ total_bits,
+                                                        uint64_t *__restrict__ total_host) {
     __shared__ unsigned long long s_before;
     unsigned long long mine = 0;
     for (uint32_t b = threadIdx.x; b < blockIdx.x; b += 1024) mine += blocktot[b];
@@ -109,7 +113,34 @@
     const unsigned long long before = s_before;
     const uint32_t i = blockIdx.x * 1024 + threadIdx.x;
     if (i < nchunks) chunk_off[i] += before;
-    if (blockIdx.x == gridDim.x - 1 && threadIdx.x == 0) *total_bits = before + blocktot[blockIdx.x];
+    if (blockIdx.x == gridDim.x - 1 && threadIdx.x == 0) {
+        *total_bits = before + blocktot[blockIdx.x];
+        if (total_host) { *total_host = before + blocktot[blockIdx.x]; __threadfence_system(); }
+    }
+}
+__global__ __launch_bounds__(1024) void k_pack_scan_one(const uint32_t *__restrict__ chunk_bits, uint32_t nchunks,
+                                                        uint64_t *__restrict__ chunk_off, uint64_t *__restrict__ total_bits,
+                                                        uint64_t *__restrict__ total_host) {
+    __shared__ unsigned long long wsum[1024 / 64];
+    const uint32_t i0 = threadIdx.x * 8, lane = threadIdx.x & 63, wid = threadIdx.x >> 6;
+    uint32_t v[8];
+    uint64_t sum = 0;
+#pragma unroll
+    for (int j = 0; j < 8; j++) { v[j] = i0 + j < nchunks ? chunk_bits[i0 + j] : 0u; sum += v[j]; }
+    const uint64_t inc = wave_inclusive_scan64<false>(sum);
+    if (lane == 63) wsum[wid] = inc;
+    __syncthreads();
+    uint64_t run = inc - sum;
+    for (uint32_t i = 0; i < wid; i++) run += wsum[i];
+#pragma unroll
+    for (int j = 0; j < 8; j++) {
+        if (i0 + j < nchunks) chunk_off[i0 + j] = run;
+        run += v[j];
+    }
+    if (threadIdx.x == 1023) {
+        *total_bits = run;
+        if (total_host) { *total_host = run; __threadfence_system(); }
+    }
 }
 __global__ __launch_bounds__(1024) void k_pack_scan_small(const uint32_t *__restrict__ chunk_bits, uint32_t nchunks,
                                                           uint64_t *__restrict__ chunk_off, uint64_t *__restrict__ total_bits) {
@@ -134,13 +165,18 @@
     }
     return pack_scan(c, counts_d, n, off_d, total_d);
 }
-int pack_scan(Ctx *c, const uint32_t *chunk_bits_d, uint32_t nchunks, uint64_t *chunk_off_d, uint64_t *total_d) {
+int pack_scan(Ctx *c, const uint32_t *chunk_bits_d, uint32_t nchunks, uint64_t *chunk_off_d, uint64_t *total_d, uint64_t *total_pinned) {
+    if (nchunks > 1024 && nchunks <= 8192) {
+        hipLaunchKernelGGL(k_pack_scan_one, dim3(1), dim3(1024), 0, c->stream, chunk_bits_d, nchunks, chunk_off_d, total_d, total_pinned);
+        CNIIC_HIP_TRY(c, hipGetLastError());
+        return CNIIC_OK;
+    }
     const uint32_t nb = (nchunks + 1023) / 1024;
     DevBuf blocktot;
     CNIIC_HIP_TRY(c, blocktot.alloc((uint64_t)nb * 8));
-    hipLaunchKernelGGL(k_pack_scan_local, dim3(nb), dim3(1024), 0, c->stream, chunk_bits_d, nchunks, chunk_off_d, blocktot.as<uint64_t>(), total_d);
+    hipLaunchKernelGGL(k_pack_scan_local, dim3(nb), dim3(1024), 0, c->stream, chunk_bits_d, nchunks, chunk_off_d, blocktot.as<uint64_t>(), total_d, total_pinned);
     if (nb > 1)
-        hipLaunchKernelGGL(k_pack_scan_add, dim3(nb), dim3(1024), 0, c->stream, nchunks, chunk_off_d, (const uint64_t *)blocktot.as<uint64_t>(), total_d);
+        hipLaunchKernelGGL(k_pack_scan_add, dim3(nb), dim3(1024), 0, c->stream, nchunks, chunk_off_d, (const uint64_t *)blocktot.as<uint64_t>(), total_d, total_pinned);
     CNIIC_HIP_TRY(c, hipGetLastError());
     return CNIIC_OK;
 }
@@ -233,8 +269,17 @@
 template <typename LabelT>
 __global__ __launch_bounds__(kPackThreads) void k_pack_count_lab(const LabelT *__restrict__ pixlab, uint64_t n, uint32_t K,
                                                                  const uint8_t *__restrict__ clen,
-                                                                 uint32_t *__restrict__ chunk_bits, uint64_t lab_stride = 0) {
+                                                                 uint32_t *__restrict__ chunk_bits, uint64_t lab_stride = 0,
+                                                                 const uint8_t *__restrict__ hdr = nullptr, uint32_t hdr_bytes = 0,
+                                                                 uint32_t *__restrict__ out_words = nullptr) {
     extern __shared__ uint8_t s_len[];
+    if (hdr_bytes && blockIdx.x == 0 && blockIdx.y == 0) {
+        for (uint32_t w = threadIdx.x; 4 * w < hdr_bytes; w += kPackThreads) {
+            uint32_t word = 0;
+            for (uint32_t j = 0; j < 4 && 4 * w + j < hdr_bytes; j++) word |= (uint32_t)hdr[4 * w + j] << (8 * j);
+            out_words[w] = word;
+        }
+    }
     pixlab += (size_t)blockIdx.y * lab_stride;
     clen += (size_t)blockIdx.y * K;
     chunk_bits += (size_t)blockIdx.y * gridDim.x;
@@ -363,7 +408,7 @@
 }
 
 int huff_pack_labels(Ctx *c, const void *pixlab_d, uint64_t n, bool wide, uint32_t K,
-                     const uint8_t *clen_d, const uint64_t *ccode_d, uint8_t *out_d, uint64_t bit_base, uint64_t *nbits_h) {
+                     const uint8_t *clen_d, const uint64_t *ccode_d, uint8_t *out_d, uint64_t bit_base, uint64_t *nbits_h, const uint8_t *hdr_d) {
     *nbits_h = 0;
     if (n == 0) return CNIIC_OK;
     if (reinterpret_cast<uintptr_t>(out_d) & 3) return c->fail(CNIIC_ERR_BAD_ARG, "huff_pack: output must be 4-byte aligned");
@@ -372,13 +417,17 @@
     CNIIC_HIP_TRY(c, cb.alloc((uint64_t)nchunks * 4));
     CNIIC_HIP_TRY(c, co.alloc((uint64_t)nchunks * 8));
     CNIIC_HIP_TRY(c, tot.alloc(8));
+    CNIIC_HIP_TRY(c, ctx_pinned_u(c));
+    const uint32_t hdr_bytes = hdr_d ? (uint32_t)(bit_base / 8) : 0u;
     if (wide)
         hipLaunchKernelGGL(k_pack_count_lab<uint16_t>, dim3(nchunks), dim3(kPackThreads), K, c->stream,
-                           reinterpret_cast<const uint16_t *>(pixlab_d), n, K, clen_d, cb.as<uint32_t>());
+                           reinterpret_cast<const uint16_t *>(pixlab_d), n, K, clen_d, cb.as<uint32_t>(), (uint64_t)0, hdr_d, hdr_bytes,
+                           reinterpret_cast<uint32_t *>(out_d));
     else
         hipLaunchKernelGGL(k_pack_count_lab<uint8_t>, dim3(nchunks), dim3(kPackThreads), K, c->stream,
-                           reinterpret_cast<const uint8_t *>(pixlab_d), n, K, clen_d, cb.as<uint32_t>());
-    CNIIC_TRY(pack_scan(c, cb.as<uint32_t>(), nchunks, co.as<uint64_t>(), tot.as<uint64_t>()));
+                           reinterpret_cast<const uint8_t *>(pixlab_d), n, K, clen_d, cb.as<uint32_t>(), (uint64_t)0, hdr_d, hdr_bytes,
+                           reinterpret_cast<uint32_t *>(out_d));
+    CNIIC_TRY(pack_scan(c, cb.as<uint32_t>(), nchunks, co.as<uint64_t>(), tot.as<uint64_t>(), c->pinned_u + kPuPackLabels.at));
     if (wide)
         hipLaunchKernelGGL(k_pack_write_lab<uint16_t>, dim3(nchunks), dim3(kPackThreads), (size_t)K * 9 + 8, c->stream,
                            reinterpret_cast<const uint16_t *>(pixlab_d), n, K, clen_d, ccode_d, co.as<uint64_t>(),
@@ -388,10 +437,8 @@
                            reinterpret_cast<const uint8_t *>(pixlab_d), n, K, clen_d, ccode_d, co.as<uint64_t>(),
                            reinterpret_cast<uint32_t *>(out_d), bit_base, (uint64_t)0, (uint64_t)0, (const uint64_t *)nullptr, pack_img_cap());
     CNIIC_HIP_TRY(c, hipGetLastError());
-    uint64_t total = 0;
-    CNIIC_HIP_TRY(c, hipMemcpyAsync(&total, tot.p, 8, hipMemcpyDeviceToHost, c->stream));
     CNIIC_HIP_TRY(c, hipStreamSynchronize(c->stream));
-    *nbits_h = total;
+    *nbits_h = c->pinned_u[kPuPackLabels.at];
     return CNIIC_OK;
 }
 
diff --git a/cniic_amd/csrc/k_kmeans_persist.hip b/cniic_amd/csrc/k_kmeans_persist.hip
--- a/cniic_amd/csrc/k_kmeans_persist.hip
+++ b/cniic_amd/csrc/k_kmeans_persist.hip
@@ -915,20 +915,15 @@
         CNIIC_HIP_TRY(c, hipFuncSetAttribute(reinterpret_cast<const void *>(k_rgbw_persist), hipFuncAttributeMaxDynamicSharedMemorySize, (int)kPsDynBytes));
         attr_set[c->device] = true;
     }
-    const uint64_t o_bar = 0, o_part = (sizeof(PsBar) + 255) & ~255ull, o_fail = o_part + ((3 * (uint64_t)kPsPartWords * 8 + 255) & ~255ull);
-    const uint64_t o_rng = o_fail + 256, total = o_rng + ((uint64_t)G * kPsChunks + 1) * 4;
-    CNIIC_HIP_TRY(c, s->ps_arena.alloc(total));
-    CNIIC_HIP_TRY(c, hipMemsetAsync(s->ps_arena.p, 0, o_rng, c->stream));
+    if (!s->ps_zero.p) return CNIIC_OK;
+    CNIIC_HIP_TRY(c, s->ps_ranges.alloc(((uint64_t)G * kPsChunks + 1) * 4));
     CNIIC_HIP_TRY(c, s->ps_pk.alloc(std::max<uint64_t>(s->U, 1) * 4));
     s->ps_blocks = G;
-    s->ps_o_part = o_part; s->ps_o_fail = o_fail; s->ps_o_rng = o_rng;
-    (void)o_bar;
-    uint8_t *a = s->ps_arena.as<uint8_t>();
     uint32_t budget = kPsDynBytes;
     if (const char *e = test_env("CNIIC_TEST_PS_LDS_BYTES")) budget = std::min<uint32_t>(kPsDynBytes, (uint32_t)atoi(e));
     s->ps_budget = budget;
     hipLaunchKernelGGL(k_ps_ranges, dim3(1), dim3(1024), 0, c->stream, (const uint32_t *)s->ne_cost.as<uint32_t>(), (const uint32_t *)s->ne_count.as<uint32_t>(), G, budget,
-                       reinterpret_cast<uint32_t *>(a + o_rng), reinterpret_cast<uint32_t *>(a + o_fail));
+                       s->ps_ranges.as<uint32_t>(), reinterpret_cast<uint32_t *>(s->ps_zero.as<uint8_t>() + kPsOffFail));
     CNIIC_HIP_TRY(c, hipGetLastError());
     s->ps = true;
     return CNIIC_OK;
@@ -947,14 +942,14 @@
     PsCold *cold = static_cast<PsCold *>(c->pinned_ps);
     memset(cold, 0, sizeof *cold);
     PsExit *xh = &cold->exit;
-    uint8_t *ar = s->ps_arena.as<uint8_t>();
+    uint8_t *ar = s->ps_zero.as<uint8_t>();
     PsArgs a{};
     a.ckeys = s->ckeys.as<uint32_t>(); a.cweight = s->cweight.as<uint32_t>(); a.labels = s->labels.as<uint8_t>();
     a.ne_cell = s->ne_cell.as<uint32_t>(); a.ne_start = s->ne_start.as<uint32_t>();
-    a.cb = reinterpret_cast<const uint32_t *>(ar + s->ps_o_rng); a.ranges_fail = reinterpret_cast<const uint32_t *>(ar + s->ps_o_fail);
+    a.cb = s->ps_ranges.as<uint32_t>(); a.ranges_fail = reinterpret_cast<const uint32_t *>(ar + kPsOffFail);
     a.lds_budget = s->ps_budget;
     a.pk = s->ps_pk.as<uint32_t>(); a.cconst0 = s->cconst.as<uint2>();
-    a.partials = reinterpret_cast<unsigned long long *>(ar + s->ps_o_part); a.bar = reinterpret_cast<PsBar *>(ar);
+    a.partials = reinterpret_cast<unsigned long long *>(ar + kPsOffPart); a.bar = reinterpret_cast<PsBar *>(ar);
     cold->cconst_g = s->cconst.as<uint2>(); cold->cent_g = s->cent.as<uint32_t>(); cold->members_out = s->members_last.as<uint64_t>(); cold->wsum_out = s->wsum_last.as<uint64_t>();
     cold->keys = s->keys; cold->gx = s->gidx; cold->seed = s->seed; cold->U = s->gidx.bits ? s->gidx.U : s->U;
     a.st_rw = s->dstate.as<KmDevState>(); a.cold = cold; a.max_iters = s->max_iters;
diff --git a/cniic_amd/csrc/k_kmeans_rgbw.hip b/cniic_amd/csrc/k_kmeans_rgbw.hip
--- a/cniic_amd/csrc/k_kmeans_rgbw.hip
+++ b/cniic_amd/csrc/k_kmeans_rgbw.hip
@@ -146,33 +146,27 @@
     }
 }
 
-constexpr uint32_t kCellGroups = kNumCells / 64;
-__global__ __launch_bounds__(64) void k_cell_totals(const uint32_t *__restrict__ cell_count, uint2 *__restrict__ tot) {
-    const uint32_t v = cell_count[blockIdx.x * 64 + threadIdx.x];
-    const uint32_t sum = wave_reduce_sum(v), sweeps = wave_reduce_sum((v + 64 * kSweep - 1) / (64 * kSweep));
-    const uint32_t ne = (uint32_t)__popcll(__ballot(v != 0));
-    if (threadIdx.x == 0) { tot[blockIdx.x] = make_uint2(sum, ne); tot[kCellGroups + blockIdx.x] = make_uint2(sweeps, 0u); }
-}
-__global__ __launch_bounds__(64) void k_cell_scan(const uint32_t *__restrict__ cell_count, const uint2 *__restrict__ tot,
+constexpr uint32_t kCellScanThreads = 1024;
+static_assert(kNumCells % kCellScanThreads == 0, "k_cell_scan: whole blocks of cells");
+__device__ __forceinline__ uint32_t cell_sweeps(uint32_t v) { return (v + 64 * kSweep - 1) / (64 * kSweep); }
+__global__ __launch_bounds__(kCellScanThreads) void k_cell_scan(const uint32_t *__restrict__ cell_count,
                                                   uint32_t *__restrict__ cell_start, uint32_t *__restrict__ cursor,
                                                   uint32_t *__restrict__ ne_cell, uint32_t *__restrict__ ne_start,
                                                   uint32_t *__restrict__ ne_cost, uint32_t *__restrict__ ne_count, uint32_t fixed_cost,
                                                   uint32_t sweep_cost) {
-    const uint32_t lane = threadIdx.x, grp = blockIdx.x;
+    __shared__ uint32_t wsum[kCellScanThreads / 64];
+    const uint32_t first = blockIdx.x * kCellScanThreads;
     uint32_t ps = 0, pn = 0, pw = 0;
-    for (uint32_t g = lane; g < grp; g += 64) { const uint2 t = tot[g]; ps += t.x; pn += t.y; pw += tot[kCellGroups + g].x; }
-    const uint32_t base = wave_reduce_sum(ps), nbase = wave_reduce_sum(pn), wbase = wave_reduce_sum(pw);
-    const uint32_t cell = grp * 64 + lane, v = cell_count[cell], sw = (v + 64 * kSweep - 1) / (64 * kSweep);
-    const uint32_t start = base + wave_inclusive_scan(v) - v, swb = wbase + wave_inclusive_scan(sw) - sw;
+    for (uint32_t i = threadIdx.x; i < first; i += kCellScanThreads) { const uint32_t t = cell_count[i]; ps += t; pn += t != 0; pw += cell_sweeps(t); }
+    const uint32_t base = block_reduce_sum<kCellScanThreads>(ps), nbase = block_reduce_sum<kCellScanThreads>(pn), wbase = block_reduce_sum<kCellScanThreads>(pw);
+    const uint32_t cell = first + threadIdx.x, v = cell_count[cell], sw = cell_sweeps(v), nz = v != 0;
+    const uint32_t start = base + block_exclusive_scan<kCellScanThreads>(v, wsum), swb = wbase + block_exclusive_scan<kCellScanThreads>(sw, wsum);
+    const uint32_t m = nbase + block_exclusive_scan<kCellScanThreads>(nz, wsum);
     cell_start[cell] = start;
     if (cursor) cursor[cell] = start;
-    const unsigned long long nzm = __ballot(v != 0);
-    if (v) {
-        const uint32_t m = nbase + (uint32_t)__popcll(nzm & ((1ull << lane) - 1ull));
-        ne_cell[m] = cell; ne_start[m] = start; ne_cost[m] = (sweep_cost ? swb * sweep_cost : start) + m * fixed_cost;
-    }
-    if (grp == kCellGroups - 1 && lane == 63) {
-        const uint32_t U = start + v, M = nbase + (uint32_t)__popcll(nzm);
+    if (v) { ne_cell[m] = cell; ne_start[m] = start; ne_cost[m] = (sweep_cost ? swb * sweep_cost : start) + m * fixed_cost; }
+    if (cell == kNumCells - 1) {
+        const uint32_t U = start + v, M = m + nz;
         cell_start[kNumCells] = U;
         ne_start[M] = U;
         ne_cost[M] = (sweep_cost ? (swb + sw) * sweep_cost : U) + M * fixed_cost;
@@ -1128,7 +1122,9 @@
         auto up = [](uint64_t x) { return (x + 255) & ~255ull; };
         const uint64_t o_part = up(s->res_bytes), o_run = o_part + up(partials_dev ? 0 : W * 8), o_fp = o_run + up(s->cells ? W * 8 : 0);
         const uint64_t o_fr = o_fp + up(s->fused ? 3 * W * 8 : 0), o_fc = o_fr + up(s->fused ? 2 * W * 8 : 0);
-        const uint64_t o_mv = o_fc + up(s->fused ? 2 * (uint64_t)K * 4 : 0), total = o_mv + up(s->cells ? ((uint64_t)K + 1) * 4 : 0);
+        const uint64_t o_mv = o_fc + up(s->fused ? 2 * (uint64_t)K * 4 : 0), o_ps = o_mv + up(s->cells ? ((uint64_t)K + 1) * 4 : 0);
+        const bool ps_may = s->fused && nshards == 1;
+        const uint64_t total = o_ps + up(ps_may ? kPsZeroBytes : 0);
         KM_ALLOC(s->arena, total);
         (void)hipMemsetAsync(s->arena.p, 0, total, c->stream);
         uint8_t *a = s->arena.as<uint8_t>();
@@ -1149,6 +1145,7 @@
             s->fused_running.view(a + o_fr, 2 * W * 8);
             s->fused_cent.view(a + o_fc, 2 * (uint64_t)K * 4);
         }
+        if (ps_may) s->ps_zero.view(a + o_ps, kPsZeroBytes);
     }
     s->dstate.view(s->resblk.p, sizeof(KmDevState));
     s->cent.view(static_cast<uint8_t *>(s->resblk.p) + s->res_cent, (uint64_t)K * 4);
@@ -1176,12 +1173,10 @@
         const uint32_t G = s->nblocks * (s->wide ? 1u : (uint32_t)kCellWaves) * nshards;
         KM_ALLOC(s->wfirst, ((uint64_t)G + 1) * 4);
         if (!s->big) KM_ALLOC(s->cell_rec, (uint64_t)kNumCells * cell_rec_words((K + 63) / 64) * 4);
-        DevBuf count, cursor, cell_tot;
+        DevBuf count, cursor;
         KM_ALLOC(count, (uint64_t)kNumCells * 4);
-        KM_ALLOC(cell_tot, (uint64_t)kCellGroups * 8 * 2);
         if (points_follow) {
-            hipLaunchKernelGGL(k_cell_totals, dim3(kCellGroups), dim3(64), 0, c->stream, cell_count_d, cell_tot.as<uint2>());
-            hipLaunchKernelGGL(k_cell_scan, dim3(kCellGroups), dim3(64), 0, c->stream, cell_count_d, (const uint2 *)cell_tot.as<uint2>(), s->cell_start.as<uint32_t>(),
+            hipLaunchKernelGGL(k_cell_scan, dim3(kNumCells / kCellScanThreads), dim3(kCellScanThreads), 0, c->stream, cell_count_d, s->cell_start.as<uint32_t>(),
                                (uint32_t *)nullptr, s->ne_cell.as<uint32_t>(), s->ne_start.as<uint32_t>(), s->ne_cost.as<uint32_t>(),
                                s->ne_count.as<uint32_t>(), kCellFixedCost, kCellSweepCost);
         } else if (rank_table_d) {
@@ -1190,8 +1185,7 @@
                 hipLaunchKernelGGL(k_cells_count_tbl, dim3(kNumCells), dim3(512), 0, c->stream, rank_table_d, count.as<uint32_t>());
                 cnt = count.as<uint32_t>();
             }
-            hipLaunchKernelGGL(k_cell_totals, dim3(kCellGroups), dim3(64), 0, c->stream, cnt, cell_tot.as<uint2>());
-            hipLaunchKernelGGL(k_cell_scan, dim3(kCellGroups), dim3(64), 0, c->stream, cnt, (const uint2 *)cell_tot.as<uint2>(), s->cell_start.as<uint32_t>(),
+            hipLaunchKernelGGL(k_cell_scan, dim3(kNumCells / kCellScanThreads), dim3(kCellScanThreads), 0, c->stream, cnt, s->cell_start.as<uint32_t>(),
                                (uint32_t *)nullptr, s->ne_cell.as<uint32_t>(), s->ne_start.as<uint32_t>(), s->ne_cost.as<uint32_t>(),
                                s->ne_count.as<uint32_t>(), kCellFixedCost, kCellSweepCost);
             if (s->wide)
@@ -1207,8 +1201,7 @@
             (void)hipMemsetAsync(count.p, 0, (uint64_t)kNumCells * 4, c->stream);
             const uint32_t g = grid_1d(U);
             hipLaunchKernelGGL(k_cell_count, dim3(g), dim3(256), 0, c->stream, keys_d, U, count.as<uint32_t>());
-            hipLaunchKernelGGL(k_cell_totals, dim3(kCellGroups), dim3(64), 0, c->stream, count.as<uint32_t>(), cell_tot.as<uint2>());
-            hipLaunchKernelGGL(k_cell_scan, dim3(kCellGroups), dim3(64), 0, c->stream, count.as<uint32_t>(), (const uint2 *)cell_tot.as<uint2>(), s->cell_start.as<uint32_t>(),
+            hipLaunchKernelGGL(k_cell_scan, dim3(kNumCells / kCellScanThreads), dim3(kCellScanThreads), 0, c->stream, count.as<uint32_t>(), s->cell_start.as<uint32_t>(),
                                cursor.as<uint32_t>(), s->ne_cell.as<uint32_t>(), s->ne_start.as<uint32_t>(), s->ne_cost.as<uint32_t>(),
                                s->ne_count.as<uint32_t>(), kCellFixedCost, kCellSweepCost);
             hipLaunchKernelGGL(k_cell_scatter, dim3(g), dim3(256), 0, c->stream, keys_d, weight_d, U, cursor.as<uint32_t>(),
diff --git a/cniic_amd/csrc/k_points.hip b/cniic_amd/csrc/k_points.hip
--- a/cniic_amd/csrc/k_points.hip
+++ b/cniic_amd/csrc/k_points.hip
@@ -71,16 +71,6 @@
     if (threadIdx.x == 255) total[b] = run;
 }
 
-__global__ __launch_bounds__(kSpBuckets) void k_sp_bstart(const uint32_t *__restrict__ total, uint32_t *__restrict__ bstart,
-                                                          uint32_t *__restrict__ sstart) {
-    __shared__ uint32_t wsum[kSpBuckets / 64];
-    const uint32_t t = total[threadIdx.x];
-    const uint32_t ex = block_exclusive_scan<kSpBuckets>(t, wsum);
-    bstart[threadIdx.x] = ex;
-    if (threadIdx.x == kSpBuckets - 1) bstart[kSpBuckets] = ex + t;
-    sstart[threadIdx.x] = block_exclusive_scan<kSpBuckets>(min(t, kSpBins), wsum);
-}
-
 template <int STEPS, typename F> __device__ __forceinline__ void sp_walk_sorted(const uint32_t *off, uint32_t n, F &&f) {
     const uint32_t lane = threadIdx.x & 63, wv = threadIdx.x >> 6;
     const uint32_t per = (n + kSpThreads - 1) / kSpThreads * 64;
@@ -109,15 +99,25 @@
 }
 
 __global__ __launch_bounds__(kSpThreads) void k_sp_scatter(const uint8_t *__restrict__ rgb, uint64_t npx, const uint32_t *__restrict__ cnt,
-                                                           const uint32_t *__restrict__ pre, const uint32_t *__restrict__ bstart,
+                                                           const uint32_t *__restrict__ pre, const uint32_t *__restrict__ total,
+                                                           uint32_t *__restrict__ bstart, uint32_t *__restrict__ sstart,
                                                            uint16_t *__restrict__ part, uint16_t *__restrict__ prank) {
     extern __shared__ __align__(16) uint8_t sp_lds[];
     uint16_t *stage = reinterpret_cast<uint16_t *>(sp_lds);
     uint32_t *off = reinterpret_cast<uint32_t *>(sp_lds + (size_t)kSpChunk * 2);
     uint32_t *cur = off + kSpBuckets + 1;
+    uint32_t *bst = cur + kSpBuckets;
     __shared__ uint32_t wsum[kSpWaves];
     const uint32_t *mycnt = cnt + (size_t)blockIdx.x * kSpBuckets;
     const uint32_t n_b = threadIdx.x < kSpBuckets ? mycnt[threadIdx.x] : 0u;
+    const uint32_t t_b = threadIdx.x < kSpBuckets ? total[threadIdx.x] : 0u;
+    const uint32_t bex = scan512(t_b, wsum);
+    if (threadIdx.x < kSpBuckets) bst[threadIdx.x] = bex;
+    if (blockIdx.x == 0) {
+        const uint32_t sex = scan512(min(t_b, kSpBins), wsum);
+        if (threadIdx.x < kSpBuckets) { bstart[threadIdx.x] = bex; sstart[threadIdx.x] = sex; }
+        if (threadIdx.x == kSpBuckets - 1) bstart[kSpBuckets] = bex + t_b;
+    }
     const uint32_t ex = scan512(n_b, wsum);
     if (threadIdx.x < kSpBuckets) { off[threadIdx.x] = ex; cur[threadIdx.x] = 0; }
     if (threadIdx.x == kSpBuckets - 1) off[kSpBuckets] = ex + n_b;
@@ -145,7 +145,7 @@
     const uint32_t lane = threadIdx.x & 63, wv = threadIdx.x >> 6;
     const uint32_t *mypre = pre + (size_t)blockIdx.x * kSpBuckets;
     const uint32_t mb = wv + kSpWaves * (lane & 31);
-    const uint32_t m_n = mycnt[mb], m_dst = bstart[mb] + mypre[mb], m_off = off[mb];
+    const uint32_t m_n = mycnt[mb], m_dst = bst[mb] + mypre[mb], m_off = off[mb];
     for (uint32_t k = 0; k < kSpBuckets / kSpWaves; k++) {
         const uint32_t n = __shfl(m_n, k, 64), d0 = __shfl(m_dst, k, 64), o = __shfl(m_off, k, 64);
         for (uint32_t i = lane; i < n; i += 64) part[(size_t)d0 + i] = stage[o + i];
@@ -416,19 +416,16 @@
     hipLaunchKernelGGL(k_sp_count, dim3(plan->nchunks), dim3(kSpThreads), 0, c->stream, rgb_d, npx, plan->cnt.as<uint32_t>());
     hipLaunchKernelGGL(k_sp_colscan, dim3(kSpBuckets), dim3(256), 0, c->stream, plan->cnt.as<uint32_t>(), plan->nchunks,
                        plan->pre.as<uint32_t>(), total.as<uint32_t>());
-    hipLaunchKernelGGL(k_sp_bstart, dim3(1), dim3(kSpBuckets), 0, c->stream, total.as<uint32_t>(), plan->bstart.as<uint32_t>(),
-                       plan->sstart.as<uint32_t>());
-    hipLaunchKernelGGL(k_sp_scatter, dim3(plan->nchunks), dim3(kSpThreads), (size_t)kSpChunk * 2 + kSpBuckets * 8 + 16, c->stream, rgb_d, npx,
-                       plan->cnt.as<uint32_t>(), plan->pre.as<uint32_t>(), plan->bstart.as<uint32_t>(), plan->part.as<uint16_t>(),
-                       plan->prank.as<uint16_t>());
+    hipLaunchKernelGGL(k_sp_scatter, dim3(plan->nchunks), dim3(kSpThreads), (size_t)kSpChunk * 2 + kSpBuckets * 12 + 16, c->stream, rgb_d, npx,
+                       plan->cnt.as<uint32_t>(), plan->pre.as<uint32_t>(), (const uint32_t *)total.as<uint32_t>(), plan->bstart.as<uint32_t>(),
+                       plan->sstart.as<uint32_t>(), plan->part.as<uint16_t>(), plan->prank.as<uint16_t>());
     hipLaunchKernelGGL(k_sp_hist, dim3(kSpBuckets), dim3(kSpThreads), (size_t)kSpBins * 4, c->stream, plan->part.as<uint16_t>(),
                        plan->bstart.as<uint32_t>(), plan->sstart.as<uint32_t>(), plan->cell_count.as<uint32_t>(), plan->bits.as<uint32_t>(),
                        plan->sbin.as<uint16_t>(), plan->scnt.as<uint32_t>());
     hipLaunchKernelGGL(k_bits_prefix, dim3(256), dim3(256), 0, c->stream, plan->bits.as<unsigned long long>(), plan->wprefix.as<uint32_t>(),
                        blocktot.as<uint32_t>());
-    CNIIC_TRY(gidx_finish(c, plan->wprefix.as<uint32_t>(), blocktot.as<uint32_t>(), plan->total.as<uint64_t>()));
+    CNIIC_TRY(gidx_finish(c, plan->wprefix.as<uint32_t>(), blocktot.as<uint32_t>(), plan->total.as<uint64_t>(), c->pinned_u + kPuSpCount.at));
     CNIIC_HIP_TRY(c, hipGetLastError());
-    CNIIC_HIP_TRY(c, hipMemcpyAsync(c->pinned_u + kPuSpCount.at, plan->total.p, 8, hipMemcpyDeviceToHost, c->stream));
     CNIIC_HIP_TRY(c, hipEventRecord(c->u_ev, c->stream));
     return CNIIC_OK;
 }
diff --git a/cniic_amd/csrc/kmeans_rgbw.hpp b/cniic_amd/csrc/kmeans_rgbw.hpp
--- a/cniic_amd/csrc/kmeans_rgbw.hpp
+++ b/cniic_amd/csrc/kmeans_rgbw.hpp
@@ -55,9 +55,9 @@
     bool ps_pending = false;
     std::shared_ptr<void> ps_hold;
     uint32_t ps_blocks = 0;
-    DevBuf ps_arena;
+    DevBuf ps_zero;
+    DevBuf ps_ranges;
     DevBuf ps_pk;
-    uint64_t ps_o_part = 0, ps_o_fail = 0, ps_o_rng = 0;
     uint32_t ps_budget = 0;
 };
 
@@ -72,6 +72,8 @@
 __host__ __device__ constexpr uint32_t ps_cell_bytes(uint32_t C) { return 16u + ((C + 3u) & ~3u) * (4u + 4u + kPsRecWords * 4u + 2u + 2u + 1u); }
 struct alignas(128) PsLine { uint32_t v; uint32_t pad[31]; };
 struct PsBar { PsLine xcount[8], xgen[8], xblocks[8], top, topgen, count, gen, abort_; };
+constexpr uint64_t kPsOffPart = (sizeof(PsBar) + 255) & ~255ull, kPsOffFail = kPsOffPart + ((3 * (uint64_t)kPsPartWords * 8 + 255) & ~255ull);
+constexpr uint64_t kPsZeroBytes = kPsOffFail + 256;
 constexpr uint32_t kPsStatusDone = 1, kPsStatusAborted = 2, kPsStatusRanges = 3;
 struct PsExit { uint32_t status, pad; uint64_t iter, moved_last, reseeds, active, pair_evals; };
 void launch_rgbw_assign_big(Ctx *c, const uint32_t *ckeys, const uint32_t *cweight, uint64_t U, uint32_t K, const uint32_t *cent, uint16_t *labels,
```

Result: faster. 10130 Mpixels/s, median of 5 (+1.0%).
